# LinXueyuanStdio/LaTeX_OCR

Hardware: AMD Instinct MI355X
Metric: formula-images/sec training step (batch 64, 128x512) (higher is better)
Workload: dtype bf16; 1 GPU; configs[2]: full encoder+attention+decoder training step, batch 64/GPU, 128x512, vocab 500, T=101 (lengths U{30..100}), Adam; global_batch=64, parallelism=dp1

## Files before the change

### include/lxo.h

```cpp
#ifndef LXO_H
#define LXO_H
#include <stddef.h>
#include <stdint.h>
#ifdef __cplusplus
extern "C" {
#endif
#pragma GCC visibility push(default)

#define LXO_F32 0
#define LXO_BF16 1

const char* lxo_last_error(void);
#define LXO_ABI_VERSION 6
int lxo_version(void);
int lxo_shape_size(void);


int lxo_gemm_nt(int dt, int a_f32, int c_f32, int small, const void* A, const void* Bp, void* C,
                int M, int N, int K, int lda, int ldb, int ldc, const float* bias, int act,
                float alpha, int accumulate, void* stream);

int lxo_gemm_tn(int dt, int a_f32, int b_f32, const void* A, const void* B, float* C,
                int M, int I, int J, int lda, int ldb, int ldc, int nsplit, int atomic, void* stream);

int lxo_gemm_slab(int dt, const void* A, const void* Bp, float* slab, int M, int N, int K, int lda, int ldb, int ldc,
                  long long slab_stride, void* stream);

int lxo_conv3x3(int dt, const void* in, const void* wpk, const float* bias, void* out, int B, int H, int W,
                int Cin, int Ho, int Wo, int Cout, int pad, int relu, void* stream);

int lxo_conv3x3_ex(int dt, const void* in, const void* wpk, const float* bias, void* out, int B, int H, int W,
                   int Cin, int Ho, int Wo, int Cout, int pad, int relu, const float* addend, int addend_rows,
                   void* out_pre, const void* relu_ref, float* colsum, void* stream);

int lxo_conv3x3_wgrad(int dt, const void* in, const void* dout, float* dw, int B, int H, int W,
                      int Cin, int Ho, int Wo, int Cout, int pad, void* stream);

int lxo_attention_fwd(int dt, const void* att_img, const void* img, const float* att_h, const float* beta,
                      float* alpha, float* part, float* ctx, int ldctx, int nv, int R, int E, int C, int beam,
                      void* stream);

int lxo_timing_enable(int on);
int lxo_timing_count(void);
int lxo_timing_get(int i, const char** family, const char** name, double* work, float* ms);


typedef struct lxo_shape {
    int B, H, W, T, V;
    int C, E, U, O, D;
    int dtype;
    int beam;
    int max_steps;
    float keep_prob;
    int dropout_seed;
    float div_gamma, div_prob;
    int div_seed;
    int encoder_cnn;
    int no_positional;
    int step_kernels;
    int encoder_rnn;
    int deterministic;
    int live_B;
} lxo_shape;

int lxo_param_num(void);
const char* lxo_param_name(int id);
const char* lxo_param_name_for(const lxo_shape* s, int id);
long long lxo_param_total(const lxo_shape* s);
int lxo_param_info(const lxo_shape* s, int id, long long* offset, long long* count);

size_t lxo_wpack_bytes(const lxo_shape* s);
size_t lxo_workspace_bytes(const lxo_shape* s);
int lxo_ws_region(const lxo_shape* s, const char* name, size_t* offset, size_t* bytes);
#define LXO_I32 2
#define LXO_U8 3
int lxo_ws_region_dtype(const lxo_shape* s, const char* name);

int lxo_pack_weights(const lxo_shape* s, const float* params, void* wpack, void* stream);

int lxo_encoder_fwd(const lxo_shape* s, const float* params, const void* wpack, void* ws,
                    const uint8_t* img, void* stream);
int lxo_encoder_bwd(const lxo_shape* s, const float* params, const void* wpack, void* ws,
                    const uint8_t* img, float* grads, int last_layer, int first_layer, void* stream);
int lxo_encoder_bwd_ready(const lxo_shape* s, const float* params, const void* wpack, void* ws, const uint8_t* img, float* grads,
                          int last_layer, int first_layer, void* const* ready_events, void* stream);
int lxo_train_bwd(const lxo_shape* s, const float* params, const void* wpack, void* ws, const int32_t* formula, const uint8_t* img,
                  float* grads, void* const* ready_events, void* stream);

int lxo_set_side_stream(void* stream);
int lxo_set_encoder_side_stream(void* stream);

int lxo_decoder_train_fwd(const lxo_shape* s, const float* params, const void* wpack, void* ws,
                          const int32_t* formula, void* stream);
int lxo_decoder_train_fwd_live(const lxo_shape* s, const float* params, const void* wpack, void* ws,
                               const int32_t* formula, const int32_t* lengths, void* stream);
int lxo_ce_loss_fwd_bwd(const lxo_shape* s, void* ws, const int32_t* formula,
                        const int32_t* lengths, float inv_ntok, void* stream);
int lxo_ce_loss_fwd_bwd_dev(const lxo_shape* s, void* ws, const int32_t* formula,
                            const int32_t* lengths, const float* ntok_dev, void* stream);
int lxo_ce_loss_weighted(const lxo_shape* s, void* ws, const int32_t* formula, const int32_t* lengths,
                         const float* w_tok, const float* w_row, float inv_norm, const float* norm_dev, void* stream);
int lxo_ce_loss_smoothed(const lxo_shape* s, void* ws, const int32_t* formula, const int32_t* lengths, float eps,
                         const float* w_tok, const float* w_row, float inv_norm, const float* norm_dev, void* stream);
int lxo_mrt_weights(const float* seq_logp, const float* cost, const int32_t* group_off, int G, int rows, float alpha,
                    float* w_out, float* q_out, float* risk_out, void* stream);
#define LXO_EDIT_MAX_REF 1024
int lxo_edit_distance(const int32_t* hyp, int hyp_block, long long hyp_block_stride, long long hyp_row_stride, long long hyp_tok_stride, int T,
                      const int32_t* hyp_len, const int32_t* ref, int G, int ref_ld, const int32_t* ref_len, const int32_t* ref_of, int per_ref,
                      int pairs, int id_end, int32_t* dist_out, float* cost_out, void* stream);
#define LXO_TEXT_STATS  12
#define LXO_TEXT_CORPUS 14
int lxo_text_stats(const int32_t* hyp, int hyp_block, long long hyp_block_stride, long long hyp_row_stride, long long hyp_tok_stride, int T,
                   const int32_t* hyp_len, const int32_t* ref, int G, int ref_ld, const int32_t* ref_len, const int32_t* ref_of, int per_ref,
                   int pairs, int id_end, int32_t* stats_out, long long* corpus_io, int accumulate, void* stream);
int lxo_mrt_candidates(const int32_t* ids, int B, int max_steps, int n, int steps, const int32_t* ref, int Tr, const int32_t* ref_len,
                       int id_end, int id_pad, int include_reference, int32_t* cand, int32_t* cand_len, float* cost, int32_t* group_off,
                       int32_t* row_image, void* stream);
#define LXO_CONSENSUS_MAX_N 64
int lxo_consensus(const int32_t* ids, long long image_stride, long long draw_stride, long long tok_stride, int B, int n, int T, int id_end,
                  const float* weights, int normalize, int32_t* dist_out, float* risk_out, int32_t* best_out, void* stream);
#define LXO_BLEU_COUNTS 10
int lxo_sentence_bleu(const int32_t* hyp, int hyp_block, long long hyp_block_stride, long long hyp_row_stride, long long hyp_tok_stride, int T,
                      const int32_t* hyp_len, const int32_t* ref, int G, int ref_ld, const int32_t* ref_len, const int32_t* ref_of, int per_ref,
                      int pairs, int id_end, int32_t* counts_out, float* bleu_out, float* cost_out, void* stream);
int lxo_consensus_bleu(const int32_t* ids, long long image_stride, long long draw_stride, long long tok_stride, int B, int n, int T, int id_end,
                       const float* weights, int32_t* match_out, float* cost_out, float* risk_out, int32_t* best_out, void* stream);
#define LXO_COST_EDIT 0
#define LXO_COST_BLEU 1
int lxo_mrt_candidates_cost(const int32_t* ids, int B, int max_steps, int n, int steps, const int32_t* ref, int Tr, const int32_t* ref_len,
                            int id_end, int id_pad, int include_reference, int32_t* cand, int32_t* cand_len, float* cost, int32_t* group_off,
                            int32_t* row_image, int cost_kind, void* stream);
int lxo_score_tokens(const lxo_shape* s, void* ws, const int32_t* formula, const int32_t* lengths,
                     float* logp_out, int32_t* top1_out, float* seq_out, void* stream);
int lxo_score_alternatives(const lxo_shape* s, void* ws, const int32_t* formula, const int32_t* lengths, int k,
                           const uint32_t* allow, int allow_ld, int32_t* ids_out, float* logp_out,
                           int32_t* rank_out, float* entropy_out, void* stream);
int lxo_decoder_train_bwd(const lxo_shape* s, const float* params, const void* wpack, void* ws,
                          const int32_t* formula, float* grads, void* stream);
int lxo_decoder_train_bwd_part(const lxo_shape* s, const float* params, const void* wpack, void* ws,
                               const int32_t* formula, float* grads, int parts, void* stream);

#define LXO_XDEC_BLOCK_BYTES (4096 + (384 << 10))
#define LXO_XDEC_ERR_WORD 512
int lxo_chain_guard(const lxo_shape* s, void* ws, const float* grads, float* scale_io, int have_scale, uint32_t* status_out, void* stream);

#define LXO_GNORM_FLOATS (2 + 1024)
int lxo_global_norm_scale(long long n, const float* grads, float clip, float* scale_out, void* stream);
int lxo_adam_step(long long n, float* params, const float* grads, float* m, float* v,
                  float lr_t, float beta1, float beta2, float eps, const float* scale_dev, void* stream);

int lxo_optimizer_step(int method, long long n, float* params, const float* grads, float* slot, float lr,
                       const float* scale_dev, void* stream);

int lxo_greedy_decode(const lxo_shape* s, const float* params, const void* wpack, void* ws,
                      int id_end, int max_iter, int32_t* ids_out, int* steps_out, void* stream);
int lxo_greedy_decode_attn(const lxo_shape* s, const float* params, const void* wpack, void* ws,
                           int id_end, int max_iter, int32_t* ids_out, float* alpha_out, int* steps_out, void* stream);
int lxo_greedy_decode_scores(const lxo_shape* s, const float* params, const void* wpack, void* ws, int id_end, int max_iter,
                             int32_t* ids_out, float* logp_out, float* alpha_out, int* steps_out, void* stream);
int lxo_greedy_decode_prefix(const lxo_shape* s, const float* params, const void* wpack, void* ws, int id_end, int max_iter,
                             const int32_t* prefix, int prefix_ld, const int32_t* prefix_len,
                             int32_t* ids_out, float* logp_out, float* alpha_out, int* steps_out, void* stream);
int lxo_greedy_decode_constrained(const lxo_shape* s, const float* params, const void* wpack, void* ws, int id_end, int max_iter,
                                  const uint32_t* allow, int allow_ld,
                                  const int32_t* prefix, int prefix_ld, const int32_t* prefix_len,
                                  int32_t* ids_out, float* logp_out, float* alpha_out, int* steps_out, void* stream);
typedef struct lxo_sample_opts { float temperature; int top_k; float top_p; unsigned seed; } lxo_sample_opts;
int lxo_sample_decode(const lxo_shape* s, const float* params, const void* wpack, void* ws, int id_end, int max_iter,
                      const lxo_sample_opts* opts, const uint32_t* allow, int allow_ld,
                      const int32_t* prefix, int prefix_ld, const int32_t* prefix_len,
                      int32_t* ids_out, float* logp_out, float* logq_out, float* alpha_out, int* steps_out, void* stream);
int lxo_sample_tokens(const float* logits, int ld, int rows, int n, int V, int time, const lxo_sample_opts* opts,
                      const uint32_t* allow, int allow_ld, int32_t* ids_out, float* logp_out, float* logq_out, void* stream);
int lxo_decode_begin(const lxo_shape* s, const float* params, const void* wpack, void* ws, void* stream);
int lxo_decode_step(const lxo_shape* s, const float* params, const void* wpack, void* ws, int id_end, int time,
                    int32_t* ids_out, int32_t* parents_out, int32_t* finished_host, int* unfinished_host, void* stream);
// ... 54 lines not shown
```

### latex_ocr_amd/_abi.py

```python
import ctypes
import os

c_int, c_ll, c_size, c_float, c_void = ctypes.c_int, ctypes.c_longlong, ctypes.c_size_t, ctypes.c_float, ctypes.c_void_p
P = ctypes.POINTER

LXO_F32, LXO_BF16 = 0, 1
LXO_GNORM_FLOATS = 2 + 1024
LIB_PATH = os.environ.get("LXO_LIB_PATH") or os.path.join(os.path.dirname(os.path.abspath(__file__)), "liblxo.so")


ABI_VERSION = 6
LXO_COMM_ID_BYTES = 128
LXO_I32, LXO_U8 = 2, 3
LXO_XDEC_BLOCK_BYTES, LXO_XDEC_ERR_WORD = 4096 + (384 << 10), 512
LXO_EDIT_MAX_REF = 1024
LXO_CONSENSUS_MAX_N = 64
LXO_TEXT_STATS, LXO_TEXT_CORPUS = 12, 14
LXO_BLEU_COUNTS = 10
LXO_COST_EDIT, LXO_COST_BLEU = 0, 1


class LxoShape(ctypes.Structure):
    _fields_ = [(n, c_int) for n in ("B", "H", "W", "T", "V", "C", "E", "U", "O", "D", "dtype", "beam", "max_steps")] + \
               [("keep_prob", c_float), ("dropout_seed", c_int), ("div_gamma", c_float), ("div_prob", c_float), ("div_seed", c_int),
                ("encoder_cnn", c_int), ("no_positional", c_int), ("step_kernels", c_int), ("encoder_rnn", c_int), ("deterministic", c_int), ("live_B", c_int)]


class LxoSampleOpts(ctypes.Structure):
    _fields_ = [("temperature", c_float), ("top_k", c_int), ("top_p", c_float), ("seed", ctypes.c_uint)]


class LxoGrammar(ctypes.Structure):
    _fields_ = [("cls", c_void), ("n_kinds", c_int), ("max_depth", c_int), ("budget", c_int)]


LXO_GRAMMAR_MAX_DEPTH = 32


def bind(lib):
    S = P(LxoShape)
    sig = {
        "lxo_last_error": (ctypes.c_char_p, []),
        "lxo_version": (c_int, []),
        "lxo_shape_size": (c_int, []),
        "lxo_ws_region_dtype": (c_int, [S, ctypes.c_char_p]),
        "lxo_gemm_nt": (c_int, [c_int] * 4 + [c_void] * 3 + [c_int] * 6 + [c_void, c_int, c_float, c_int, c_void]),
        "lxo_gemm_tn": (c_int, [c_int] * 3 + [c_void] * 3 + [c_int] * 8 + [c_void]),
        "lxo_conv3x3": (c_int, [c_int, c_void, c_void, c_void, c_void] + [c_int] * 9 + [c_void]),
        "lxo_conv3x3_ex": (c_int, [c_int, c_void, c_void, c_void, c_void] + [c_int] * 9 + [c_void, c_int, c_void, c_void, c_void, c_void]),
        "lxo_conv3x3_wgrad": (c_int, [c_int, c_void, c_void, c_void] + [c_int] * 8 + [c_void]),
        "lxo_gemm_slab": (c_int, [c_int, c_void, c_void, c_void] + [c_int] * 6 + [c_ll, c_void]),
        "lxo_attention_fwd": (c_int, [c_int] + [c_void] * 7 + [c_int] * 6 + [c_void]),
        "lxo_timing_enable": (c_int, [c_int]),
        "lxo_timing_count": (c_int, []),
        "lxo_timing_get": (c_int, [c_int, P(ctypes.c_char_p), P(ctypes.c_char_p), P(ctypes.c_double), P(c_float)]),
        "lxo_param_num": (c_int, []),
        "lxo_param_name": (ctypes.c_char_p, [c_int]),
        "lxo_param_name_for": (ctypes.c_char_p, [S, c_int]),
        "lxo_param_total": (c_ll, [S]),
        "lxo_param_info": (c_int, [S, c_int, P(c_ll), P(c_ll)]),
        "lxo_wpack_bytes": (c_size, [S]),
        "lxo_workspace_bytes": (c_size, [S]),
        "lxo_ws_region": (c_int, [S, ctypes.c_char_p, P(c_size), P(c_size)]),
        "lxo_pack_weights": (c_int, [S, c_void, c_void, c_void]),
        "lxo_encoder_fwd": (c_int, [S, c_void, c_void, c_void, c_void, c_void]),
        "lxo_encoder_bwd": (c_int, [S, c_void, c_void, c_void, c_void, c_void, c_int, c_int, c_void]),
        "lxo_encoder_bwd_ready": (c_int, [S, c_void, c_void, c_void, c_void, c_void, c_int, c_int, c_void, c_void]),
        "lxo_train_bwd": (c_int, [S, c_void, c_void, c_void, c_void, c_void, c_void, c_void, c_void]),
        "lxo_set_encoder_side_stream": (c_int, [c_void]),
        "lxo_set_side_stream": (c_int, [c_void]),
        "lxo_decoder_train_fwd": (c_int, [S, c_void, c_void, c_void, c_void, c_void]),
        "lxo_decoder_train_fwd_live": (c_int, [S, c_void, c_void, c_void, c_void, c_void, c_void]),
        "lxo_ce_loss_fwd_bwd": (c_int, [S, c_void, c_void, c_void, c_float, c_void]),
        "lxo_ce_loss_fwd_bwd_dev": (c_int, [S, c_void, c_void, c_void, c_void, c_void]),
        "lxo_ce_loss_weighted": (c_int, [S, c_void, c_void, c_void, c_void, c_void, c_float, c_void, c_void]),
        "lxo_ce_loss_smoothed": (c_int, [S, c_void, c_void, c_void, c_float, c_void, c_void, c_float, c_void, c_void]),
        "lxo_mrt_weights": (c_int, [c_void, c_void, c_void, c_int, c_int, c_float, c_void, c_void, c_void, c_void]),
        "lxo_edit_distance": (c_int, [c_void, c_int, c_ll, c_ll, c_ll, c_int, c_void, c_void, c_int, c_int, c_void, c_void, c_int, c_int, c_int, c_void, c_void, c_void]),
        "lxo_text_stats": (c_int, [c_void, c_int, c_ll, c_ll, c_ll, c_int, c_void, c_void, c_int, c_int, c_void, c_void, c_int, c_int, c_int, c_void, c_void, c_int, c_void]),
        "lxo_mrt_candidates": (c_int, [c_void, c_int, c_int, c_int, c_int, c_void, c_int, c_void, c_int, c_int, c_int, c_void, c_void, c_void, c_void, c_void, c_void]),
        "lxo_sentence_bleu": (c_int, [c_void, c_int, c_ll, c_ll, c_ll, c_int, c_void, c_void, c_int, c_int, c_void, c_void, c_int, c_int, c_int, c_void, c_void, c_void, c_void]),
        "lxo_mrt_candidates_cost": (c_int, [c_void, c_int, c_int, c_int, c_int, c_void, c_int, c_void, c_int, c_int, c_int, c_void, c_void, c_void, c_void, c_void, c_int, c_void]),
        "lxo_consensus_bleu": (c_int, [c_void, c_ll, c_ll, c_ll, c_int, c_int, c_int, c_int, c_void, c_void, c_void, c_void, c_void, c_void]),
        "lxo_consensus": (c_int, [c_void, c_ll, c_ll, c_ll, c_int, c_int, c_int, c_int, c_void, c_int, c_void, c_void, c_void, c_void]),
        "lxo_decoder_train_bwd_part": (c_int, [S, c_void, c_void, c_void, c_void, c_void, c_int, c_void]),
        "lxo_decoder_train_bwd": (c_int, [S, c_void, c_void, c_void, c_void, c_void, c_void]),
        "lxo_global_norm_scale": (c_int, [c_ll, c_void, c_float, c_void, c_void]),
        "lxo_adam_step": (c_int, [c_ll, c_void, c_void, c_void, c_void, c_float, c_float, c_float, c_float, c_void, c_void]),
        "lxo_optimizer_step": (c_int, [c_int, c_ll, c_void, c_void, c_void, c_float, c_void, c_void]),
        "lxo_greedy_decode": (c_int, [S, c_void, c_void, c_void, c_int, c_int, c_void, P(c_int), c_void]),
        "lxo_greedy_decode_attn": (c_int, [S, c_void, c_void, c_void, c_int, c_int, c_void, c_void, P(c_int), c_void]),
        "lxo_decode_begin": (c_int, [S, c_void, c_void, c_void, c_void]),
        "lxo_decode_step": (c_int, [S, c_void, c_void, c_void, c_int, c_int, c_void, c_void, c_void, P(c_int), c_void]),
        "lxo_beam_decode": (c_int, [S, c_void, c_void, c_void, c_int, c_int, c_void, c_void, P(c_int), c_void]),
        "lxo_beam_decode_attn": (c_int, [S, c_void, c_void, c_void, c_int, c_int, c_void, c_void, c_void, P(c_int), c_void]),
        "lxo_greedy_decode_scores": (c_int, [S, c_void, c_void, c_void, c_int, c_int, c_void, c_void, c_void, P(c_int), c_void]),
        "lxo_beam_decode_scores": (c_int, [S, c_void, c_void, c_void, c_int, c_int, c_void, c_void, c_void, c_void, P(c_int), c_void]),
        "lxo_score_tokens": (c_int, [S, c_void, c_void, c_void, c_void, c_void, c_void, c_void]),
        "lxo_score_alternatives": (c_int, [S, c_void, c_void, c_void, c_int, c_void, c_int, c_void, c_void, c_void, c_void, c_void]),
        "lxo_greedy_decode_prefix": (c_int, [S, c_void, c_void, c_void, c_int, c_int, c_void, c_int, c_void, c_void, c_void, c_void, P(c_int), c_void]),
        "lxo_beam_decode_prefix": (c_int, [S, c_void, c_void, c_void, c_int, c_int, c_void, c_int, c_void, c_void, c_void, c_void, c_void, P(c_int), c_void]),
        "lxo_greedy_decode_constrained": (c_int, [S, c_void, c_void, c_void, c_int, c_int, c_void, c_int, c_void, c_int, c_void, c_void, c_void, c_void, P(c_int), c_void]),
        "lxo_beam_decode_constrained": (c_int, [S, c_void, c_void, c_void, c_int, c_int, c_void, c_int, c_void, c_int, c_void, c_void, c_void, c_void, c_void, P(c_int), c_void]),
        "lxo_sample_decode": (c_int, [S, c_void, c_void, c_void, c_int, c_int, P(LxoSampleOpts), c_void, c_int, c_void, c_int, c_void, c_void, c_void, c_void, c_void, P(c_int), c_void]),
        "lxo_sample_tokens": (c_int, [c_void, c_int, c_int, c_int, c_int, c_int, P(LxoSampleOpts), c_void, c_int, c_void, c_void, c_void, c_void]),
        "lxo_grammar_scratch_bytes": (c_size, [c_int, c_int]),
        "lxo_greedy_decode_grammar": (c_int, [S, c_void, c_void, c_void, c_int, c_int, c_void, c_int, c_void, c_int, c_void, P(LxoGrammar), c_void, c_void, c_void, c_void, c_void, P(c_int), c_void]),
        "lxo_beam_decode_grammar": (c_int, [S, c_void, c_void, c_void, c_int, c_int, c_void, c_int, c_void, c_int, c_void, P(LxoGrammar), c_void, c_void, c_void, c_void, c_void, c_void, P(c_int), c_void]),
        "lxo_sample_decode_grammar": (c_int, [S, c_void, c_void, c_void, c_int, c_int, P(LxoSampleOpts), c_void, c_int, c_void, c_int, c_void, P(LxoGrammar), c_void, c_void, c_void, c_void, c_void, c_void, P(c_int), c_void]),
        "lxo_grammar_step": (c_int, [P(LxoGrammar), c_int, c_int, c_int, c_int, c_void, c_void, c_void, c_int, c_int, c_void, c_int, c_void, c_void, c_void, c_void]),
        "lxo_chain_guard": (c_int, [S, c_void, c_void, c_void, c_int, c_void, c_void]),
        "lxo_decode_state_get": (c_int, [S, c_void, c_int, c_void, c_void, c_void, c_void]),
        "lxo_decode_state_set": (c_int, [S, c_void, c_int, c_void, c_void, c_void, c_void, c_void]),
        "lxo_decode_cell_step": (c_int, [S, c_void, c_void, c_void, c_int, c_int, c_void]),
        "lxo_comm_unique_id": (c_int, [c_void]),
        "lxo_comm_init": (c_int, [c_void, c_int, c_int, P(c_void)]),
        "lxo_comm_info": (c_int, [c_void, P(c_int), P(c_int)]),
        "lxo_allreduce_bucket": (c_int, [c_void, c_void, c_ll, c_int, c_void, c_void]),
        "lxo_comm_destroy": (c_int, [c_void]),
        "lxo_comm_last_error": (ctypes.c_char_p, []),
    }
    missing = []
    for name, (res, args) in sig.items():
        try:
            fn = getattr(lib, name)
        except AttributeError:
            missing.append(name)
            continue
        fn.restype, fn.argtypes = res, args
    lib._lxo_missing = missing
    if not missing:
        if lib.lxo_version() != ABI_VERSION or lib.lxo_shape_size() != ctypes.sizeof(LxoShape):
            raise RuntimeError("liblxo ABI mismatch: library version %d / lxo_shape %d bytes, binding version %d / %d bytes"
                               % (lib.lxo_version(), lib.lxo_shape_size(), ABI_VERSION, ctypes.sizeof(LxoShape)))
    return lib


ENTRY_POINTS = ["lxo_last_error", "lxo_version", "lxo_shape_size", "lxo_ws_region_dtype", "lxo_timing_enable", "lxo_timing_count", "lxo_timing_get", "lxo_gemm_nt", "lxo_gemm_tn", "lxo_conv3x3", "lxo_conv3x3_ex", "lxo_conv3x3_wgrad", "lxo_gemm_slab", "lxo_attention_fwd", "lxo_param_num", "lxo_param_name", "lxo_param_name_for",
                "lxo_param_total", "lxo_param_info", "lxo_wpack_bytes", "lxo_workspace_bytes", "lxo_ws_region",
                "lxo_pack_weights", "lxo_encoder_fwd", "lxo_encoder_bwd", "lxo_encoder_bwd_ready", "lxo_train_bwd", "lxo_set_side_stream", "lxo_set_encoder_side_stream", "lxo_decoder_train_fwd", "lxo_decoder_train_fwd_live",
                "lxo_ce_loss_fwd_bwd", "lxo_ce_loss_fwd_bwd_dev", "lxo_ce_loss_weighted", "lxo_ce_loss_smoothed", "lxo_mrt_weights", "lxo_edit_distance", "lxo_text_stats", "lxo_mrt_candidates", "lxo_consensus", "lxo_sentence_bleu", "lxo_consensus_bleu", "lxo_mrt_candidates_cost", "lxo_decoder_train_bwd", "lxo_decoder_train_bwd_part", "lxo_global_norm_scale", "lxo_adam_step", "lxo_optimizer_step",
                "lxo_greedy_decode", "lxo_greedy_decode_attn", "lxo_beam_decode", "lxo_beam_decode_attn", "lxo_greedy_decode_scores", "lxo_beam_decode_scores", "lxo_score_tokens", "lxo_score_alternatives", "lxo_greedy_decode_prefix", "lxo_beam_decode_prefix", "lxo_greedy_decode_constrained", "lxo_beam_decode_constrained", "lxo_sample_decode", "lxo_sample_tokens",
                "lxo_grammar_scratch_bytes", "lxo_greedy_decode_grammar", "lxo_beam_decode_grammar", "lxo_sample_decode_grammar", "lxo_grammar_step", "lxo_decode_begin", "lxo_decode_step",
                "lxo_chain_guard", "lxo_decode_state_get", "lxo_decode_state_set", "lxo_decode_cell_step",
                "lxo_comm_unique_id", "lxo_comm_init", "lxo_comm_info", "lxo_allreduce_bucket", "lxo_comm_destroy", "lxo_comm_last_error"]

_lib = None


def load():
    global _lib
    if _lib is None:
        if not os.path.exists(LIB_PATH):
            raise RuntimeError(
                "latex_ocr_amd: %s is missing. Build it with `python -c 'import __graft_entry__ as g; g.build()'` "
                "(hipcc --offload-arch=gfx950). There is no CPU fallback." % LIB_PATH)
        try:
            import torch
        except ImportError:
            pass
        _lib = bind(ctypes.CDLL(LIB_PATH))
        if _lib._lxo_missing:
            raise RuntimeError("liblxo.so lacks entry points: %s" % _lib._lxo_missing)
    return _lib


def check(lib, rc, what=""):
    if rc != 0:
        raise RuntimeError("%s failed: rc=%d %s" % (what, rc, lib.lxo_last_error().decode()))
```

### latex_ocr_amd/csrc/api.hip

```cpp
#include "lxo.h"
#include "gemm.h"
#include "impl.h"
#include <stdio.h>
#include <string.h>

static thread_local char g_err[256] = "";
static int fail(int code, const char* what) {
    snprintf(g_err, sizeof(g_err), "%s (code %d)", what, code);
    return code < 0 ? code : -code;
}
#define CHECK_LAUNCH(expr, what) do { int rc_ = (expr); if (rc_ != 0) return fail(rc_, what); } while (0)

extern "C" const char* lxo_last_error(void) { return g_err; }
extern "C" int lxo_version(void) { return LXO_ABI_VERSION; }
extern "C" int lxo_shape_size(void) { return (int)sizeof(lxo_shape); }

extern "C" int lxo_gemm_nt(int dt, int a_f32, int c_f32, int small, const void* A, const void* Bp, void* C,
                           int M, int N, int K, int lda, int ldb, int ldc, const float* bias, int act,
                           float alpha, int accumulate, void* stream) {
    GemmNT p; memset(&p, 0, sizeof(p));
    p.A = A; p.Bp = Bp; p.C = C; p.M = M; p.N = N; p.K = K; p.lda = lda; p.ldb = ldb; p.ldc = ldc;
    p.bias = bias; p.act = act; p.alpha = alpha; p.accumulate = accumulate; p.addend_rows = 1;
    CHECK_LAUNCH(lxo_launch_gemm_nt(dt, a_f32, c_f32, small, p, (hipStream_t)stream), "lxo_gemm_nt");
    return 0;
}

extern "C" int lxo_gemm_tn(int dt, int a_f32, int b_f32, const void* A, const void* B, float* C,
                           int M, int I, int J, int lda, int ldb, int ldc, int nsplit, int atomic, void* stream) {
    GemmTN p; memset(&p, 0, sizeof(p));
    p.A = A; p.B = B; p.C = C; p.M = M; p.I = I; p.J = J; p.lda = lda; p.ldb = ldb; p.ldc = ldc;
    p.nsplit = nsplit; p.nbatch = 1; p.atomic = atomic;
    CHECK_LAUNCH(lxo_launch_gemm_tn(dt, a_f32, b_f32, p, (hipStream_t)stream), "lxo_gemm_tn");
    return 0;
}

#define MAKE_PLAN(P, s) if (!(s)) return fail(-1, "null shape"); Plan P(*(s)); \
    { char m_[200]; int v_ = P.validate(m_, sizeof(m_)); if (v_) { snprintf(g_err, sizeof(g_err), "%s", m_); return v_; } }

extern "C" int lxo_param_num(void) { return P_COUNT; }
extern "C" const char* lxo_param_name_for(const lxo_shape* s, int id) { return lxo_param_name_mode(id, s ? s->encoder_cnn : 0); }
extern "C" long long lxo_param_total(const lxo_shape* s) { if (!s) return -1; Plan P(*s); return P.ptotal; }
extern "C" int lxo_param_info(const lxo_shape* s, int id, long long* offset, long long* count) {
    if (!s || id < 0 || id >= P_COUNT) return fail(-1, "lxo_param_info");
    Plan P(*s);
    if (offset) *offset = P.poff[id];
    if (count) *count = P.pcount[id];
    return 0;
}
extern "C" size_t lxo_wpack_bytes(const lxo_shape* s) { if (!s) return 0; Plan P(*s); return P.ktotal; }
extern "C" size_t lxo_workspace_bytes(const lxo_shape* s) { if (!s) return 0; Plan P(*s); return P.wtotal; }
extern "C" int lxo_ws_region(const lxo_shape* s, const char* name, size_t* offset, size_t* bytes) {
    if (!s || !name) return fail(-1, "lxo_ws_region");
    Plan P(*s);
    for (int i = 0; i < W_COUNT; ++i)
        if (strcmp(name, lxo_ws_name(i)) == 0) {
            if (offset) *offset = P.woff[i];
            if (bytes) *bytes = P.wbytes[i];
            return 0;
        }
    return fail(-1, "unknown workspace region");
}
extern "C" int lxo_ws_region_dtype(const lxo_shape* s, const char* name) {
    if (!s || !name) return fail(-1, "lxo_ws_region_dtype");
    const bool bf = s->dtype == LXO_BF16;
    static const char* const kCompute[] = {"p1", "y2", "p2", "y3", "y4", "p4", "y5", "p5", "y6", "img", "att_img", "emb_in", "dlogits",
                                           "d_att_img", "g0", "g1", "g2", "cols", "dec_emb", "dec_txe", "rxt"};
    static const char* const kBf16[] = {"recb", "gb", "dzb", "rhb", "rdzb", "att_exp", "datth_b"};
    static const char* const kI32[] = {"dec_ids", "dec_flags", "beam_par"};
    static const char* const kU8[] = {"m2", "m4", "m5"};
    for (const char* n : kCompute) if (strcmp(name, n) == 0) return bf ? LXO_BF16 : LXO_F32;
    for (const char* n : kBf16) if (strcmp(name, n) == 0) return LXO_BF16;
    for (const char* n : kI32) if (strcmp(name, n) == 0) return LXO_I32;
    for (const char* n : kU8) if (strcmp(name, n) == 0) return LXO_U8;
    if (strcmp(name, "d_img") == 0) { Plan P(*s); return P.dimg_masked() ? LXO_BF16 : LXO_F32; }
    for (int i = 0; i < W_COUNT; ++i) if (strcmp(name, lxo_ws_name(i)) == 0) return LXO_F32;
    return fail(-1, "unknown workspace region");
}
extern "C" int lxo_pack_weights(const lxo_shape* s, const float* params, void* wpack, void* stream) {
    MAKE_PLAN(P, s);
    CHECK_LAUNCH(lxo_impl_pack_weights(P, params, wpack, (hipStream_t)stream), "lxo_pack_weights");
    return 0;
}
extern "C" int lxo_encoder_fwd(const lxo_shape* s, const float* params, const void* wpack, void* ws,
                               const uint8_t* img, void* stream) {
    MAKE_PLAN(P, s);
    CHECK_LAUNCH(lxo_impl_encoder_fwd(P, params, wpack, ws, img, (hipStream_t)stream), "lxo_encoder_fwd");
    return 0;
}
extern "C" int lxo_encoder_bwd(const lxo_shape* s, const float* params, const void* wpack, void* ws,
                               const uint8_t* img, float* grads, int last_layer, int first_layer, void* stream) {
    MAKE_PLAN(P, s);
    if (last_layer > 6 || first_layer < 1 || last_layer < first_layer) return fail(-1, "lxo_encoder_bwd: layer range");
    CHECK_LAUNCH(lxo_impl_encoder_bwd(P, params, wpack, ws, img, grads, last_layer, first_layer, (hipStream_t)stream), "lxo_encoder_bwd");
    return 0;
}
extern "C" int lxo_encoder_bwd_ready(const lxo_shape* s, const float* params, const void* wpack, void* ws, const uint8_t* img, float* grads,
                                     int last_layer, int first_layer, void* const* ready_events, void* stream) {
    MAKE_PLAN(P, s);
    if (last_layer > 6 || first_layer < 1 || last_layer < first_layer) return fail(-1, "lxo_encoder_bwd_ready: layer range");
    if (!ready_events) return fail(-1, "lxo_encoder_bwd_ready: null event table");
    CHECK_LAUNCH(lxo_impl_encoder_bwd(P, params, wpack, ws, img, grads, last_layer, first_layer, (hipStream_t)stream, ready_events), "lxo_encoder_bwd_ready");
    return 0;
}

#include "head_kernels.h"
extern "C" int lxo_decoder_train_fwd(const lxo_shape* s, const float* params, const void* wpack, void* ws,
                                     const int32_t* formula, void* stream) {
    MAKE_PLAN(P, s);
    if (s->T <= 0) return fail(-1, "T must be positive");
    CHECK_LAUNCH(lxo_impl_decoder_train_fwd(P, params, wpack, ws, formula, (hipStream_t)stream), "lxo_decoder_train_fwd");
    return 0;
}
extern "C" int lxo_decoder_train_fwd_live(const lxo_shape* s, const float* params, const void* wpack, void* ws,
                                          const int32_t* formula, const int32_t* lengths, void* stream) {
    MAKE_PLAN(P, s);
    if (s->T <= 0) return fail(-1, "T must be positive");
    CHECK_LAUNCH(lxo_impl_decoder_train_fwd(P, params, wpack, ws, formula, (hipStream_t)stream, lengths), "lxo_decoder_train_fwd_live");
    return 0;
}
extern "C" int lxo_ce_loss_fwd_bwd(const lxo_shape* s, void* ws, const int32_t* formula, const int32_t* lengths,
                                   float inv_ntok, void* stream) {
    MAKE_PLAN(P, s);
    CHECK_LAUNCH(lxo_impl_ce_loss(P, ws, formula, lengths, inv_ntok, nullptr, (hipStream_t)stream), "lxo_ce_loss_fwd_bwd");
    return 0;
}
extern "C" int lxo_ce_loss_fwd_bwd_dev(const lxo_shape* s, void* ws, const int32_t* formula, const int32_t* lengths,
                                       const float* ntok_dev, void* stream) {
    MAKE_PLAN(P, s);
    if (!ntok_dev) return fail(-1, "lxo_ce_loss_fwd_bwd_dev: null token count");
    CHECK_LAUNCH(lxo_impl_ce_loss(P, ws, formula, lengths, 0.f, ntok_dev, (hipStream_t)stream), "lxo_ce_loss_fwd_bwd_dev");
    return 0;
}
extern "C" int lxo_ce_loss_weighted(const lxo_shape* s, void* ws, const int32_t* formula, const int32_t* lengths, const float* w_tok, const float* w_row,
                                    float inv_norm, const float* norm_dev, void* stream) {
    MAKE_PLAN(P, s);
    if (!w_tok && !w_row) return fail(-1, "lxo_ce_loss_weighted: w_tok and w_row are both NULL (the unweighted loss is lxo_ce_loss_fwd_bwd)");
    CHECK_LAUNCH(lxo_impl_ce_loss(P, ws, formula, lengths, inv_norm, norm_dev, (hipStream_t)stream, w_tok, w_row), "lxo_ce_loss_weighted");
    return 0;
}
extern "C" int lxo_ce_loss_smoothed(const lxo_shape* s, void* ws, const int32_t* formula, const int32_t* lengths, float eps, const float* w_tok,
                                    const float* w_row, float inv_norm, const float* norm_dev, void* stream) {
    MAKE_PLAN(P, s);
    if (!ws || !formula || !lengths) return fail(-1, "lxo_ce_loss_smoothed: null ws, formula or lengths");
    if (!(eps - eps == 0.f) || !(eps >= 0.f && eps < 1.f)) return fail(-1, "lxo_ce_loss_smoothed: eps is not a finite number in [0, 1)");
    CHECK_LAUNCH(lxo_impl_ce_loss(P, ws, formula, lengths, inv_norm, norm_dev, (hipStream_t)stream, w_tok, w_row, &eps), "lxo_ce_loss_smoothed");
    return 0;
}
extern "C" int lxo_mrt_weights(const float* seq_logp, const float* cost, const int32_t* group_off, int G, int rows, float alpha,
                               float* w_out, float* q_out, float* risk_out, void* stream) {
    if (!w_out || !seq_logp || !cost || !group_off) return fail(-1, "lxo_mrt_weights: null w_out, seq_logp, cost or group_off");
    if (G < 0 || rows < 0) return fail(-1, "lxo_mrt_weights: G < 0 or rows < 0");
    if (!(alpha - alpha == 0.f)) return fail(-1, "lxo_mrt_weights: alpha is not finite");
    CHECK_LAUNCH(lxo_k_mrt_weights(seq_logp, cost, group_off, G, rows, alpha, w_out, q_out, risk_out, (hipStream_t)stream), "lxo_mrt_weights");
    return 0;
}
#include "seqcost.h"
static_assert(LXO_EDIT_MAX_REF == kEditMaxRef, "include/lxo.h and csrc/seqcost.h disagree on the reference limit");
extern "C" int lxo_edit_distance(const int32_t* hyp, int hyp_block, long long hyp_block_stride, long long hyp_row_stride, long long hyp_tok_stride, int T,
                                 const int32_t* hyp_len, const int32_t* ref, int G, int ref_ld, const int32_t* ref_len, const int32_t* ref_of,
                                 int per_ref, int pairs, int id_end, int32_t* dist_out, float* cost_out, void* stream) {
    if (!hyp || !ref || !dist_out) return fail(-1, "lxo_edit_distance: null hyp, ref or dist_out");
    if (pairs < 0 || T < 0 || G < 0 || hyp_block_stride < 0 || hyp_row_stride < 0 || hyp_tok_stride < 0)
        return fail(-1, "lxo_edit_distance: a negative count or stride");
    if (hyp_block < 1 || per_ref < 1 || (pairs > 0 && G < 1)) return fail(-1, "lxo_edit_distance: hyp_block < 1, per_ref < 1 or no reference row");
    if (ref_ld < 1 || ref_ld > LXO_EDIT_MAX_REF) return fail(-1, "lxo_edit_distance: ref_ld outside 1 .. LXO_EDIT_MAX_REF (a reference longer than the kernel's column limit)");
    const EditArgs a = {hyp, hyp_len, ref, ref_len, ref_of, nullptr, dist_out, cost_out, hyp_block_stride, hyp_row_stride, hyp_tok_stride,
                        hyp_block, T, G, ref_ld, per_ref, pairs, id_end};
    CHECK_LAUNCH(lxo_k_edit_distance(a, (hipStream_t)stream), "lxo_edit_distance");
    return 0;
}
static_assert(LXO_TEXT_STATS == kTextStats && LXO_TEXT_CORPUS == kTextCorpus, "include/lxo.h and csrc/seqcost.h disagree on the text-metric rows");
extern "C" int lxo_text_stats(const int32_t* hyp, int hyp_block, long long hyp_block_stride, long long hyp_row_stride, long long hyp_tok_stride, int T,
                              const int32_t* hyp_len, const int32_t* ref, int G, int ref_ld, const int32_t* ref_len, const int32_t* ref_of, int per_ref,
                              int pairs, int id_end, int32_t* stats_out, long long* corpus_io, int accumulate, void* stream) {
    if (!hyp || !ref) return fail(-1, "lxo_text_stats: null hyp or ref");
    if (!stats_out && !corpus_io) return fail(-1, "lxo_text_stats: stats_out and corpus_io are both NULL");
    if (pairs < 0 || T < 0 || G < 0 || hyp_block_stride < 0 || hyp_row_stride < 0 || hyp_tok_stride < 0)
        return fail(-1, "lxo_text_stats: a negative count or stride");
    if (hyp_block < 1 || per_ref < 1 || (pairs > 0 && G < 1)) return fail(-1, "lxo_text_stats: hyp_block < 1, per_ref < 1 or no reference row");
    if (T > LXO_EDIT_MAX_REF) return fail(-1, "lxo_text_stats: T outside 0 .. LXO_EDIT_MAX_REF (a hypothesis wider than the kernel's staging limit)");
    if (ref_ld < 1 || ref_ld > LXO_EDIT_MAX_REF) return fail(-1, "lxo_text_stats: ref_ld outside 1 .. LXO_EDIT_MAX_REF (a reference longer than the kernel's column limit)");
    if (accumulate != 0 && accumulate != 1) return fail(-1, "lxo_text_stats: accumulate must be 0 or 1");
    const TextArgs a = {hyp, hyp_len, ref, ref_len, ref_of, stats_out, corpus_io, hyp_block_stride, hyp_row_stride, hyp_tok_stride,
                        hyp_block, T, G, ref_ld, per_ref, pairs, id_end, accumulate};
    CHECK_LAUNCH(lxo_k_text_stats(a, (hipStream_t)stream), "lxo_text_stats");
// ... 443 lines not shown
```

### latex_ocr_amd/csrc/conv_wgrad.hip

```cpp
#include "gemm.h"
#include "api_util.h"
#include "lxo_debug.h"

namespace {

constexpr int WTH = 2, WTW = 64, WPW = WTW + 2, WPH = WTH + 2, WPROWS = WPH * WPW;
constexpr int WTHREADS = 512;
constexpr int WPATCH = 5 * WTHREADS * 16;
constexpr int WDY = WTH * WTW * 256;
constexpr int WSTAGE = WPATCH + WDY;
constexpr int WCI = 64, WCO = 128;

typedef __attribute__((address_space(1))) const void* gptr_t;
typedef __attribute__((address_space(3))) void* lptr_t;
typedef __attribute__((ext_vector_type(4))) short v4s_t;
typedef __attribute__((address_space(3))) v4s_t* ltr_t;
LXO_DEV void glds16(const void* g, void* l) {
    __builtin_amdgcn_global_load_lds((gptr_t)(uintptr_t)g, (lptr_t)(uintptr_t)l, 16, 0, 0);
}
LXO_DEV u32x2 tr_read(const char* p) {
    return __builtin_bit_cast(u32x2, __builtin_amdgcn_ds_read_tr16_b64_v4i16((ltr_t)(uintptr_t)p));
}

}
// ... 45 lines not shown
    const unsigned drel = (unsigned)(((tid >> 4) * Cout + dgch) * 2);
    const int dxq = (co0 + dgch) < Cout ? (tid >> 4) : 0x7FFF0000;
    int tx_i = pb_beg % tiles_x, ty_i = (pb_beg / tiles_x) % tiles_y, b_i = pb_beg / (tiles_x * tiles_y);
    auto issue = [&](int stage) {
        const int oy0 = ty_i * WTH, ox0 = tx_i * WTW;
        const unsigned sx = (unsigned)((((b_i * p.H + oy0) * p.W + ox0) * p.Cin + ci0) * 2);
        const int loy = max(0, p.pad - oy0), lox = max(0, p.pad - ox0);
        const int ny = min(WPH, p.H + p.pad - oy0) - loy, nx = min(WPW, p.W + p.pad - ox0) - lox;
        const unsigned lo = __builtin_amdgcn_readfirstlane(((unsigned)loy << 16) | (unsigned)lox);
        const unsigned lim = __builtin_amdgcn_readfirstlane(((unsigned)(ny - 1) << 16) | (unsigned)(nx - 1));
#pragma unroll
        for (int j = 0; j < 5; ++j) {
            if (j == 4 && wave != 0) break;
            const u16x2_t t = __builtin_bit_cast(u16x2_t, ppk[j]) - __builtin_bit_cast(u16x2_t, lo);
            const u16x2_t m = __builtin_elementwise_min(t, __builtin_bit_cast(u16x2_t, lim));
            const bool ok = __builtin_bit_cast(unsigned, m) == __builtin_bit_cast(unsigned, t) && (j < 4 || tid < 64);
            const unsigned voff = ok ? prel[j] : LXO_BLDS_OOB;
            LXO_BLDS16(voff, rx, sx, lxo_wgrad_lds, m0b, stage * WSTAGE + (wave * 64 + 512 * j) * 16);
        }
        const unsigned sd = (unsigned)((((b_i * p.Ho + oy0) * p.Wo + ox0) * Cout + co0) * 2);
#pragma unroll
        for (int j = 0; j < 4; ++j) {
            const int hx = (oy0 + (j >> 1) < p.Ho) ? p.Wo - ox0 - 32 * (j & 1) : 0;
            const unsigned voff = dxq < hx ? drel : LXO_BLDS_OOB;
            const unsigned sdj = __builtin_amdgcn_readfirstlane(sd + (unsigned)((((j >> 1) * p.Wo + 32 * (j & 1)) * Cout) * 2));
            LXO_BLDS16(voff, rdy, sdj, lxo_wgrad_lds, m0b, stage * WSTAGE + WPATCH + (wave * 64 + 512 * j) * 16);
        }
        if (++tx_i == tiles_x) { tx_i = 0; if (++ty_i == tiles_y) { ty_i = 0; ++b_i; } }
    };

    f32x16 acc[9];
#pragma unroll
    for (int t = 0; t < 9; ++t)
#pragma unroll
        for (int e = 0; e < 16; ++e) acc[t][e] = 0.f;

    const int h = lane >> 5, g = (lane >> 4) & 1, qj = (lane & 15) >> 2, qc = lane & 3;
    const int a_ch = wci * 32 + 16 * g + 4 * qc;
    const int a_chunk = a_ch >> 3, a_sub = (a_ch & 7) * 2;
    const int b_ch = wco * 32 + 16 * g + 4 * qc;
    const int b_chunk = b_ch >> 3, b_sub = (b_ch & 7) * 2;
    const int bl = 8 * h + qj;
    int poff[8];
#pragma unroll
    for (int k = 0; k < 8; ++k) poff[k] = bl * 128 + ((a_chunk ^ ((k + (bl >> 1)) & 7)) << 4) + a_sub;
    const int doff_a = WPATCH + bl * 256 + ((b_chunk ^ (bl & 15)) << 4) + b_sub;
    const int doff_b = WPATCH + (bl + 4) * 256 + ((b_chunk ^ ((bl + 4) & 15)) << 4) + b_sub;

#define WSTAMP(i) do { if (p.dbg && tid == 0 && (i) < 64) p.dbg[(long long)blockIdx.x * 64 + (i)] = __builtin_readcyclecounter(); } while (0)
    WSTAMP(0);
    issue(0);
    for (int pb = pb_beg; pb < pb_end; ++pb) {
        const int stage = (pb - pb_beg) & 1;
        WSTAMP(1 + 3 * (pb - pb_beg));
        __builtin_amdgcn_s_waitcnt(0x0F70);
        WSTAMP(2 + 3 * (pb - pb_beg));
        __builtin_amdgcn_s_barrier();
        WSTAMP(3 + 3 * (pb - pb_beg));
#ifndef LXO_WG_DIAG
#define LXO_WG_DIAG 0
#endif
        const char* sb = lxo_wgrad_lds + stage * WSTAGE;
        const char* pk[8];
#pragma unroll
        for (int k = 0; k < 8; ++k) pk[k] = sb + poff[k];
        const char* da = sb + doff_a;
        const char* db = sb + doff_b;
        u32x2 ra[2][4], rb[2][4];
        auto read_b = [&](int xg, u32x2 (&b4)[4]) {
#pragma unroll
            for (int ty = 0; ty < 2; ++ty) {
                const int cd = (ty * 64 + xg * 16) * 256;
                b4[2 * ty] = tr_read(da + cd);
                b4[2 * ty + 1] = tr_read(db + cd);
            }
        };
        auto read_a = [&](int s, u32x2 (&r)[4]) {
            const int cc = (s & 3) * WPW + (s >> 2) * 16;
            r[0] = tr_read(pk[(cc >> 1) & 7] + cc * 128);
            r[1] = tr_read(pk[((cc + 4) >> 1) & 7] + (cc + 4) * 128);
            r[2] = tr_read(pk[((cc + 2) >> 1) & 7] + (cc + 2) * 128);
            r[3] = tr_read(pk[((cc + 6) >> 1) & 7] + (cc + 6) * 128);
        };
        read_b(0, rb[0]);
        read_a(0, ra[0]);
        __builtin_amdgcn_sched_barrier(0);
        if (pb + 1 < pb_end && !((LXO_WG_DIAG & 1) && pb > pb_beg)) issue(stage ^ 1);
        __builtin_amdgcn_sched_barrier(0);
#pragma unroll
        for (int s = 0; s < 16; ++s) {
            const int xg = s >> 2, row = s & 3, cur = s & 1, bcur = xg & 1;
            if (s == 0) __builtin_amdgcn_s_setprio(3);
            else if (s == 4) __builtin_amdgcn_s_setprio(2);
            else if (s == 8) __builtin_amdgcn_s_setprio(1);
            else if (s == 12) __builtin_amdgcn_s_setprio(0);
            if (!(LXO_WG_DIAG & 2)) {
                if (s + 1 < 16) read_a(s + 1, ra[cur ^ 1]);
                if (row == 1 && xg + 1 < 4) read_b(xg + 1, rb[bcur ^ 1]);
            } else if (s == 0) { read_a(1, ra[1]); read_b(1, rb[1]); }
            __builtin_amdgcn_sched_barrier(0);
            const u32x2* r = ra[cur];
            const u32x4 a0 = {r[0][0], r[0][1], r[1][0], r[1][1]};
            const u32x4 a2 = {r[2][0], r[2][1], r[3][0], r[3][1]};
            const u32x4 b0 = {rb[bcur][0][0], rb[bcur][0][1], rb[bcur][1][0], rb[bcur][1][1]};
            const u32x4 b1 = {rb[bcur][2][0], rb[bcur][2][1], rb[bcur][3][0], rb[bcur][3][1]};
#define WG_MFMA(A, B, T) acc[T] = __builtin_amdgcn_mfma_f32_32x32x16_bf16(__builtin_bit_cast(bf16x8_t, A), __builtin_bit_cast(bf16x8_t, B), acc[T], 0, 0, 0)
            if (row <= 2) WG_MFMA(a0, b0, row * 3 + 0); else WG_MFMA(a0, b1, (row - 1) * 3 + 0);
            __builtin_amdgcn_sched_barrier(0);
            const u32x4 a1 = (LXO_WG_DIAG & 4) ? u32x4{r[0][1], r[1][0], r[1][1], r[3][1]} :
                             u32x4{__builtin_amdgcn_alignbit(r[0][1], r[0][0], 16), __builtin_amdgcn_alignbit(r[1][0], r[0][1], 16),
                                   __builtin_amdgcn_alignbit(r[1][1], r[1][0], 16), __builtin_amdgcn_alignbit(r[3][1], r[1][1], 16)};
            __builtin_amdgcn_sched_barrier(0);
            if (row <= 2) {
                WG_MFMA(a2, b0, row * 3 + 2);
                WG_MFMA(a1, b0, row * 3 + 1);
                if (row >= 1) WG_MFMA(a0, b1, (row - 1) * 3 + 0);
            }
            if (row >= 1) {
                WG_MFMA(a2, b1, (row - 1) * 3 + 2);
                WG_MFMA(a1, b1, (row - 1) * 3 + 1);
            }
#undef WG_MFMA
            __builtin_amdgcn_sched_barrier(0);
        }
    }
    WSTAMP(61);
    if (p.det_slab) {
        float* const sb = p.det_slab + ((long long)split * ntiles + tile) * (9 * WCI * WCO) + (wci * 32 + 4 * (lane >> 5)) * WCO + wco * 32 + (lane & 31);
#pragma unroll
        for (int t = 0; t < 9; ++t)
#pragma unroll
            for (int e = 0; e < 16; ++e) sb[(t * WCI + (e & 3) + 8 * (e >> 2)) * WCO] = acc[t][e];
        return;
    }
    const int co = co0 + wco * 32 + (lane & 31);
    if (co < Cout) {
        const int rot = (int)(blockIdx.x % 9u);
        float* const cbase = p.C + (long long)(ci0 + wci * 32 + 4 * (lane >> 5)) * p.ldc + co;
        auto emit = [&](const f32x16& a, int t) {
#pragma unroll
            for (int e = 0; e < 16; ++e) atomicAdd(cbase + (t * p.Cin + (e & 3) + 8 * (e >> 2)) * p.ldc, a[e]);
        };
#pragma unroll
        for (int t = 0; t < 9; ++t) if (t >= rot) emit(acc[t], t);
#pragma unroll
        for (int t = 0; t < 9; ++t) if (t < rot) emit(acc[t], t);
    }
    WSTAMP(62);
}

__global__ __launch_bounds__(256) void wgrad_slab_reduce_kernel(const float* __restrict__ slab, int nsplit, int ntiles, int tiles_co, int Cin, int Cout,
                                                               float* __restrict__ dw, int ldc) {
    const int tile = blockIdx.y;
    const int i = blockIdx.x * 256 + threadIdx.x;
    if (i >= 9 * WCI * WCO) return;
    const int co = i % WCO, ci = (i / WCO) % WCI, tap = i / (WCO * WCI);
    const int ci0 = (tile / tiles_co) * WCI, co0 = (tile % tiles_co) * WCO;
    float s = 0.f;
    for (int q = 0; q < nsplit; ++q) s += slab[((long long)q * ntiles + tile) * (9 * WCI * WCO) + i];
    if (co0 + co < Cout) dw[(long long)(tap * Cin + ci0 + ci) * ldc + co0 + co] += s;
}

}

static thread_local unsigned long long* g_wgrad_dbg = nullptr;
extern "C" int lxo_wgrad_debug(unsigned long long* buf) { g_wgrad_dbg = buf; return 0; }
int lxo_launch_conv_wgrad(const GemmTN& p, hipStream_t s) {
    if (!p.conv || p.Cin % 64 || p.J % 8) return -2;
    {
        const long long nb = p.M / (p.Ho * p.Wo);
        if (nb * p.H * p.W * p.Cin * 2 + 2LL * (p.W + 1) * p.Cin >= (1LL << 31) || nb * p.Ho * p.Wo * p.J * 2 >= (1LL << 31)) return -2;
    }
    {
        static bool done[64] = {};
        int dev = 0;
        const bool known = hipGetDevice(&dev) == hipSuccess && dev >= 0 && dev < 64;
        if (!known || !done[dev]) {
            HIPRC(hipFuncSetAttribute(reinterpret_cast<const void*>(conv_wgrad_kernel), hipFuncAttributeMaxDynamicSharedMemorySize, 2 * WSTAGE));
            if (known) done[dev] = true;
        }
    }
    const int B = p.M / (p.Ho * p.Wo);
    const int tiles_ci = p.Cin / WCI, tiles_co = cdiv(p.J, WCO);
    const int tiles_x = cdiv(p.Wo, WTW), tiles_y = cdiv(p.Ho, WTH);
    const int nblocks = B * tiles_x * tiles_y;
    const int tiles = tiles_ci * tiles_co;
    int nsplit = cdiv(256, tiles);
    if (nsplit > nblocks) nsplit = nblocks;
    constexpr int min_blk = 8;
    if (nsplit > cdiv(nblocks, min_blk)) nsplit = cdiv(nblocks, min_blk);
    if (nsplit < 1) nsplit = 1;
    const int per_split = cdiv(nblocks, nsplit);
    nsplit = cdiv(nblocks, per_split);
    constexpr float stag_scale = 10.f;
    float stagger = stag_scale / (float)per_split;
    if (stagger > 0.5f) stagger = 0.5f;
    if (nsplit < 2) stagger = 0.f;
    GemmTN q = p;
    q.nbatch = tiles;
    q.dbg = g_wgrad_dbg;
    const int nsplit8 = (nsplit + 7) / 8 * 8;
    if (q.det_slab) {
        const size_t need = (size_t)nsplit * tiles * 9 * WCI * WCO;
        if (need > q.det_floats) return -6;
    }
    hipLaunchKernelGGL(conv_wgrad_kernel, dim3(tiles * nsplit8), dim3(WTHREADS), 2 * WSTAGE, s, q, tiles_co, tiles_x, tiles_y, nblocks, nsplit, stagger);
    if (q.det_slab)
        hipLaunchKernelGGL(wgrad_slab_reduce_kernel, dim3(9 * WCI * WCO / 256, tiles), dim3(256), 0, s, q.det_slab, nsplit, tiles, tiles_co, p.Cin, p.J, p.C, p.ldc);
    return (int)hipGetLastError();
}
```

### latex_ocr_amd/csrc/decoder_kernels.hip

```cpp
#include "decoder_kernels.h"
#include "api_util.h"
#include "drop.h"

namespace {


LXO_DEV void load4(const float* p, float (&v)[4]) {
    f32x4 a = *reinterpret_cast<const f32x4*>(p);
    v[0] = a[0]; v[1] = a[1]; v[2] = a[2]; v[3] = a[3];
}
LXO_DEV void load4(const bf16_t* p, float (&v)[4]) {
    u32x2 a = *reinterpret_cast<const u32x2*>(p);
    v[0] = __uint_as_float(a[0] << 16); v[1] = __uint_as_float(a[0] & 0xffff0000u);
    v[2] = __uint_as_float(a[1] << 16); v[3] = __uint_as_float(a[1] & 0xffff0000u);
}
LXO_DEV void store4(float* p, const float (&v)[4]) { f32x4 a = {v[0], v[1], v[2], v[3]}; *reinterpret_cast<f32x4*>(p) = a; }
LXO_DEV void store4(bf16_t* p, const float (&v)[4]) { u32x2 a = {pack_bf2(v[0], v[1]), pack_bf2(v[2], v[3])}; *reinterpret_cast<u32x2*>(p) = a; }

LXO_DEV float slab_sum(const Slabs& sl, long long row, int col) {
    float v = 0.f;
    const float* q = sl.p + row * sl.ld + col;
    for (int s = 0; s < sl.n; ++s) v += q[(long long)s * sl.stride];
    return v;
}
// ... 902 lines not shown
            const long long pitch = (long long)B * E;
            int t0 = 0;
            for (; t0 + TU <= n; t0 += TU) {
                f32x4 a[TU], d[TU][Q];
#pragma unroll
                for (int tt = 0; tt < TU; ++tt) {
                    a[tt] = *reinterpret_cast<const f32x4*>(ap + (t0 + tt) * pitch);
#pragma unroll
                    for (int c = 0; c < Q; ++c) d[tt][c] = sd[t0 + tt][wave * Q + c];
                }
#pragma unroll
                for (int tt = 0; tt < TU; ++tt) datt_live_step<RW>(x, a[tt], d[tt], acc, db, sumd);
            }
            for (; t0 < n; ++t0) {
                const f32x4 a = *reinterpret_cast<const f32x4*>(ap + t0 * pitch);
                f32x4 d[Q];
#pragma unroll
                for (int c = 0; c < Q; ++c) d[c] = sd[t0][wave * Q + c];
                datt_live_step<RW>(x, a, d, acc, db, sumd);
            }
        }
    }
    if (kon) {
        float bt[4];
        load4(beta + k0, bt);
#pragma unroll
        for (int rr = 0; rr < RW; ++rr)
            if (rbase + rr < R) {
                float o[4];
#pragma unroll
                for (int j = 0; j < 4; ++j) o[j] = (acc[rr][j] * 4.f) * bt[j];
                store4(dout + ((long long)b * R + rbase + rr) * E + k0, o);
            }
#pragma unroll
        for (int j = 0; j < 4; ++j) redb[wave][k0 + j] = sumd - 2.f * db[j];
    }
    __syncthreads();
    if (tid < E) {
        const float s = redb[0][tid] + redb[1][tid] + redb[2][tid] + redb[3][tid];
        if (dbeta_part) dbeta_part[((long long)blockIdx.y * gridDim.x + blockIdx.x) * E + tid] = s;
        else atomicAdd(&dbeta[tid], s);
    }
}

__global__ __launch_bounds__(256) void add_mean_grad_kernel(float* __restrict__ dimg, const float* __restrict__ dmean, int B, int R, int C) {
    const long long total = (long long)B * R * C;
    const float inv = 1.0f / (float)R;
    for (long long i = (long long)blockIdx.x * 256 + threadIdx.x; i < total; i += (long long)gridDim.x * 256) {
        const int c = (int)(i % C);
        const int b = (int)(i / ((long long)R * C));
        dimg[i] += dmean[(long long)b * C + c] * inv;
    }
}

__global__ __launch_bounds__(256) void colsum_kernel(const float* __restrict__ a, int lda, float* __restrict__ out, int M, int N, int rows_per_block) {
    const int n = blockIdx.x * 256 + threadIdx.x;
    const int m0 = blockIdx.y * rows_per_block, m1 = min(M, m0 + rows_per_block);
    if (n >= N) return;
    float s = 0.f;
    for (int m = m0; m < m1; ++m) s += a[(long long)m * lda + n];
    atomicAdd(&out[n], s);
}

__global__ __launch_bounds__(256) void colsum4_kernel(const float* __restrict__ a, int lda, float* __restrict__ out, int M, int N, int rows_per_block) {
    __shared__ f32x4 red[4][64];
    const int cq = threadIdx.x & 63, ry = threadIdx.x >> 6;
    const int n = (blockIdx.x * 64 + cq) * 4;
    const int m0 = blockIdx.y * rows_per_block, m1 = min(M, m0 + rows_per_block);
    const int nl = n < N ? n : 0;
    f32x4 s = {0.f, 0.f, 0.f, 0.f};
    for (int mb = m0 + ry; mb < m1; mb += 32) {
        f32x4 v[8];
#pragma unroll
        for (int u = 0; u < 8; ++u) { const int m = min(mb + 4 * u, m1 - 1); v[u] = *reinterpret_cast<const f32x4*>(a + (long long)m * lda + nl); }
#pragma unroll
        for (int u = 0; u < 8; ++u) if (mb + 4 * u < m1) s += v[u];
    }
    red[ry][cq] = s;
    __syncthreads();
    if (ry == 0 && n < N) {
        const f32x4 t = red[0][cq] + red[1][cq] + red[2][cq] + red[3][cq];
#pragma unroll
        for (int e = 0; e < 4; ++e) atomicAdd(&out[n + e], t[e]);
    }
}


template <typename AT>
__global__ __launch_bounds__(256) void colsum_part_kernel(const AT* __restrict__ a, long long lda, float* __restrict__ part, long long M, int N, int rows_per) {
    const int n = blockIdx.x * 256 + threadIdx.x;
    const long long m0 = (long long)blockIdx.y * rows_per, m1 = m0 + rows_per < M ? m0 + rows_per : M;
    if (n >= N) return;
    float s = 0.f;
    for (long long mb = m0; mb < m1; mb += 8) {
        float v[8];
#pragma unroll
        for (int u = 0; u < 8; ++u) { const long long m = mb + u < m1 ? mb + u : m1 - 1; v[u] = to_f32(a[m * lda + n]); }
#pragma unroll
        for (int u = 0; u < 8; ++u) if (mb + u < m1) s += v[u];
    }
    part[(long long)blockIdx.y * N + n] = s;
}
__global__ __launch_bounds__(256) void det_reduce_kernel(const float* __restrict__ part, int nslot, long long stride, int N, float* __restrict__ out) {
    __shared__ float gs[16][16];
    const int c = threadIdx.x & 15, g = threadIdx.x >> 4;
    const int n = blockIdx.x * 16 + c;
    const int per = (nslot + 15) / 16;
    const int q0 = g * per, q1 = min(nslot, q0 + per);
    float s = 0.f;
    if (n < N) {
        for (int q = q0; q < q1; q += 8) {
            float v[8];
#pragma unroll
            for (int u = 0; u < 8; ++u) v[u] = part[(long long)min(q + u, q1 - 1) * stride + n];
#pragma unroll
            for (int u = 0; u < 8; ++u) if (q + u < q1) s += v[u];
        }
    }
    gs[g][c] = s;
    __syncthreads();
    if (g == 0 && n < N) {
        float tsum = gs[0][c];
#pragma unroll
        for (int k = 1; k < 16; ++k) tsum += gs[k][c];
        out[n] += tsum;
    }
}

__global__ __launch_bounds__(256) void embed_scatter_kernel(const float* __restrict__ demb, const int* __restrict__ formula,
                                                           float* __restrict__ dtable, float* __restrict__ dstart,
                                                           int B, int T, int D, int V) {
    const long long total = (long long)T * B * D;
    for (long long i = (long long)blockIdx.x * 256 + threadIdx.x; i < total; i += (long long)gridDim.x * 256) {
        const int d = (int)(i % D);
        const long long row = i / D;
        const int b = (int)(row % B), t = (int)(row / B);
        const float g = demb[i];
        if (t == 0) atomicAdd(&dstart[d], g);
        else {
            int id = formula[(long long)b * T + t - 1];
            id = id < 0 ? 0 : (id >= V ? V - 1 : id);
            atomicAdd(&dtable[(long long)id * D + d], g);
        }
    }
}

__global__ __launch_bounds__(256) void embed_scatter_rows_kernel(const float* __restrict__ demb, const int* __restrict__ formula,
                                                                float* __restrict__ dtable, float* __restrict__ dstart,
                                                                int B, int T, int D, int V, int det) {
    constexpr int CH = 2048;
    __shared__ int list[CH];
    __shared__ float part[256];
    __shared__ int cnt;
    __shared__ int wcnt[4];
    const int id = blockIdx.x;
    const int tid = threadIdx.x;
    const int rpw = 256 / D, r = tid / D, c = tid - r * D;
    float sum = 0.f;
    const int total = T * B;
    const int per = (total + (int)gridDim.y - 1) / (int)gridDim.y;
    const int s0 = blockIdx.y * per, s1 = min(total, s0 + per);
    for (int base = s0; base < s1; base += CH) {
        if (tid == 0) cnt = 0;
        __syncthreads();
        if (det) {
            for (int jb = base; jb < min(s1, base + CH); jb += 256) {
                const int j = jb + tid;
                int row = -1;
                if (j < min(s1, base + CH)) {
                    const int b = j / T, tt = j - b * T;
                    if (id == V) { if (j < B) row = j; }
                    else if (tt + 1 < T) { int tok = formula[j]; tok = tok < 0 ? 0 : (tok >= V ? V - 1 : tok); if (tok == id) row = (tt + 1) * B + b; }
                }
                const unsigned long long m = __ballot(row >= 0);
                const int lane = tid & 63, wv = tid >> 6;
                if (lane == 0) wcnt[wv] = __builtin_popcountll(m);
                __syncthreads();
                int off = cnt;
                for (int w = 0; w < wv; ++w) off += wcnt[w];
                if (row >= 0) list[off + __builtin_popcountll(m & ((1ull << lane) - 1ull))] = row;
                __syncthreads();
                if (tid == 0) cnt += wcnt[0] + wcnt[1] + wcnt[2] + wcnt[3];
                __syncthreads();
            }
        } else
        for (int j = base + tid; j < min(s1, base + CH); j += 256) {
            const int b = j / T, tt = j - b * T;
            if (id == V) { if (j < B) list[atomicAdd(&cnt, 1)] = j; continue; }
            if (tt + 1 >= T) continue;
            int tok = formula[j]; tok = tok < 0 ? 0 : (tok >= V ? V - 1 : tok);
            if (tok == id) list[atomicAdd(&cnt, 1)] = (tt + 1) * B + b;
        }
        __syncthreads();
        const int n = cnt;
        if (r < rpw) {
            for (int k = r; k < n; k += 4 * rpw) {
                float v[4];
#pragma unroll
                for (int u = 0; u < 4; ++u) { const int kk = min(k + u * rpw, n - 1); v[u] = demb[(long long)list[kk] * D + c]; }
#pragma unroll
                for (int u = 0; u < 4; ++u) if (k + u * rpw < n) sum += v[u];
            }
        }
        __syncthreads();
    }
    part[tid] = (r < rpw) ? sum : 0.f;
    __syncthreads();
    if (tid < D) {
        float t = 0.f;
        for (int q = 0; q < rpw; ++q) t += part[q * D + tid];
        float* dst = id == V ? dstart : dtable + (long long)id * D;
        if (t != 0.f) atomicAdd(&dst[tid], t);
    }
}

__global__ __launch_bounds__(256) void init_bwd_kernel(const float* __restrict__ dcc, Slabs dxh,
                                                      const float* __restrict__ c0, const float* __restrict__ rec0, int ldr,
                                                      float* __restrict__ dpre, int B, int U, int O) {
    const int W = 2 * U + O;
    const int total = B * W;
    for (int i = blockIdx.x * 256 + threadIdx.x; i < total; i += gridDim.x * 256) {
        const int b = i / W, k = i - b * W;
        float d, s;
        if (k < U) { d = dcc[(long long)b * U + k]; s = c0[(long long)b * U + k]; }
        else if (k < 2 * U) { d = slab_sum(dxh, b, O + (k - U)); s = rec0[(long long)b * ldr + O + (k - U)]; }
        else { d = slab_sum(dxh, b, k - 2 * U); s = rec0[(long long)b * ldr + (k - 2 * U)]; }
        dpre[i] = d * (1.f - s * s);
    }
}

__global__ __launch_bounds__(256) void beam_gather_kernel(const float* __restrict__ rec, int ldr, int XH, const float* __restrict__ cs, int U,
                                                         const int* __restrict__ parents, int k, float* __restrict__ tmp_rec, float* __restrict__ tmp_cs, int n) {
    const int W = XH + U;
    const long long total = (long long)n * W;
    for (long long i = (long long)blockIdx.x * 256 + threadIdx.x; i < total; i += (long long)gridDim.x * 256) {
        const int v = (int)(i / W), c = (int)(i - (long long)v * W);
        const int src = (v / k) * k + parents[v];
        if (c < XH) tmp_rec[(long long)v * XH + c] = rec[(long long)src * ldr + c];
        else tmp_cs[(long long)v * U + (c - XH)] = cs[(long long)src * U + (c - XH)];
    }
}
__global__ __launch_bounds__(256) void beam_scatter_kernel(float* __restrict__ rec, int ldr, int XH, float* __restrict__ cs, int U,
                                                          const float* __restrict__ tmp_rec, const float* __restrict__ tmp_cs, int n,
                                                          bf16_t* __restrict__ recb, int ldrb) {
    const int W = XH + U;
    const long long total = (long long)n * W;
    for (long long i = (long long)blockIdx.x * 256 + threadIdx.x; i < total; i += (long long)gridDim.x * 256) {
        const int v = (int)(i / W), c = (int)(i - (long long)v * W);
        if (c < XH) {
            const float x = tmp_rec[(long long)v * XH + c];
            rec[(long long)v * ldr + c] = x;
            if (recb) recb[(long long)v * ldrb + c] = f2bf(x);
        }
        else cs[(long long)v * U + (c - XH)] = tmp_cs[(long long)v * U + (c - XH)];
    }
}
constexpr int BP_KMAX = 16;
__global__ __launch_bounds__(256) void beam_permute_kernel(float* __restrict__ rec, int ldr, int XH, float* __restrict__ cs, int U,
                                                          const int* __restrict__ parents, int k, bf16_t* __restrict__ recb, int ldrb) {
    const int b = blockIdx.x, c = blockIdx.y * 256 + threadIdx.x;
    if (c >= XH + U) return;
    float v[BP_KMAX];
#pragma unroll
    for (int r = 0; r < BP_KMAX; ++r) {
        v[r] = 0.f;
        if (r < k) {
            const int src = b * k + parents[b * k + r];
            v[r] = c < XH ? rec[(long long)src * ldr + c] : cs[(long long)src * U + (c - XH)];
        }
    }
#pragma unroll
    for (int r = 0; r < BP_KMAX; ++r) {
        if (r < k) {
            const int dst = b * k + r;
            if (c < XH) { rec[(long long)dst * ldr + c] = v[r]; if (recb) recb[(long long)dst * ldrb + c] = f2bf(v[r]); }
            else cs[(long long)dst * U + (c - XH)] = v[r];
        }
    }
}
__global__ __launch_bounds__(256) void tile_rows_kernel(const float* __restrict__ src, int lds, float* __restrict__ dst, int ldd, int n, int k, int cols) {
    const long long total = (long long)n * cols;
    for (long long i = (long long)blockIdx.x * 256 + threadIdx.x; i < total; i += (long long)gridDim.x * 256) {
        const int v = (int)(i / cols), c = (int)(i - (long long)v * cols);
        dst[(long long)v * ldd + c] = src[(long long)(v / k) * lds + c];
    }
}

__global__ __launch_bounds__(256) void sumsq_kernel(const float* __restrict__ g, long long n, float* __restrict__ out) {
    __shared__ float red[4];
    float s = 0.f;
    for (long long i = (long long)blockIdx.x * 256 + threadIdx.x; i < n; i += (long long)gridDim.x * 256) s = fmaf(g[i], g[i], s);
    s = wave_sum(s);
    if ((threadIdx.x & 63) == 0) red[threadIdx.x >> 6] = s;
    __syncthreads();
    if (threadIdx.x == 0) out[blockIdx.x] = red[0] + red[1] + red[2] + red[3];
}
__global__ void clip_scale_kernel(const float* __restrict__ sumsq, int nparts, float clip, float* __restrict__ out) {
    float ss = 0.f;
    for (int i = 0; i < nparts; ++i) ss += sumsq[i];
    const float gn = sqrtf(ss);
    out[1] = gn;
    out[0] = clip > 0.f ? clip / fmaxf(gn, clip) : 1.0f;
}
__global__ void chain_guard_kernel(const unsigned* __restrict__ err_fwd, const unsigned* __restrict__ err_bwd, const float* __restrict__ probe,
                                   float* __restrict__ scale, int have_scale, unsigned* __restrict__ status) {
    const unsigned ef = err_fwd ? err_fwd[0] : 0u, eb = err_bwd ? err_bwd[0] : 0u;
    const float pv = probe ? probe[0] : 0.f;
    const bool drop = (ef | eb) != 0u || pv != pv;
    if (status) { status[0] = ef; status[1] = eb; status[2] = drop ? 1u : 0u; }
    scale[0] = drop ? __uint_as_float(0x7fc00000u) : (have_scale ? scale[0] : 1.0f);
}
__global__ void chain_poison_kernel(const unsigned* __restrict__ err_fwd, const unsigned* __restrict__ err_bwd, float* __restrict__ probe) {
    if ((err_fwd && err_fwd[0]) || (err_bwd && err_bwd[0])) probe[0] = __uint_as_float(0x7fc00000u);
}
__global__ __launch_bounds__(256) void adam_kernel(float* __restrict__ p, const float* __restrict__ g, float* __restrict__ m, float* __restrict__ v,
                                                  long long n, float lr_t, float b1, float b2, float eps, const float* __restrict__ scale) {
    const float sc = scale ? scale[0] : 1.0f;
    if (sc != sc) return;
    for (long long i = (long long)blockIdx.x * 256 + threadIdx.x; i < n; i += (long long)gridDim.x * 256) {
        const float gi = g[i] * sc;
        const float mi = b1 * m[i] + (1.f - b1) * gi;
        const float vi = b2 * v[i] + (1.f - b2) * gi * gi;
        m[i] = mi; v[i] = vi;
        p[i] -= lr_t * mi / (sqrtf(vi) + eps);
    }
}

__global__ __launch_bounds__(256) void simple_opt_kernel(float* __restrict__ p, const float* __restrict__ g, float* __restrict__ slot,
                                                        long long n, float lr, int mode, const float* __restrict__ scale) {
    const float sc = scale ? scale[0] : 1.0f;
    if (sc != sc) return;
    for (long long i = (long long)blockIdx.x * 256 + threadIdx.x; i < n; i += (long long)gridDim.x * 256) {
        const float gi = g[i] * sc;
        if (mode == 1) p[i] -= lr * gi;
        else if (mode == 2) { const float a = slot[i] + gi * gi; slot[i] = a; p[i] -= lr * gi / sqrtf(a); }
        else { const float ms = 0.9f * slot[i] + 0.1f * gi * gi; slot[i] = ms; p[i] -= lr * gi / sqrtf(ms + 1e-10f); }
    }
}

inline int grid1(long long items, int per_block = 256, int cap = 2048) {
    long long g = (items + per_block - 1) / per_block;
    return (int)(g < 1 ? 1 : (g > cap ? cap : g));
}
}

#define LAUNCH(kern, grid, ...) hipLaunchKernelGGL(kern, dim3(grid), dim3(256), 0, st, __VA_ARGS__)
#define BYCT(dt, kern, grid, ...) do { if ((dt) == LXO_BF16) LAUNCH((kern<bf16_t>), grid, __VA_ARGS__); else LAUNCH((kern<float>), grid, __VA_ARGS__); } while (0)
#define DONE return (int)hipGetLastError()

int lxo_k_rowmean(int dt, const void* img, float* mean, int B, int R, int C, hipStream_t st) {
    if (C % 64) return -2;
    if (dt == LXO_BF16) LAUNCH((rowmean_kernel<bf16_t>), dim3(C / 64, B), (const bf16_t*)img, mean, R, C);
    else LAUNCH((rowmean_kernel<float>), dim3(C / 64, B), (const float*)img, mean, R, C);
    DONE;
// ... 206 lines not shown
```

### latex_ocr_amd/csrc/gemm.h

```cpp
#pragma once
#include "lxo_common.h"

struct GemmNT {
    const void* A; const void* Bp; void* C;
    int M, N, K;
    int lda, ldb, ldc;
    int conv, H, W, Cin, Ho, Wo, pad;
    const float* bias;
    const float* addend; int addend_rows;
    int act;
    const void* relu_ref; int ldr;
    void* out_pre;
    int accumulate;
    float* colsum;
    float* colsum_part; size_t colsum_part_floats;
    float alpha;
    unsigned long long* dbg;
    void* pool_out; unsigned char* pool_mask; int pool_h, pool_w;
    int diag;
};

struct GemmTN {
    const void* A; const void* B; float* C;
    int M, I, J;
    int lda, ldb, ldc;
    int conv, H, W, Cin, Ho, Wo, pad;
    int nsplit, nbatch;
    long long strideA, strideB, strideC;
    int atomic;
    unsigned long long* dbg;
    float* det_slab; size_t det_floats;
};

int lxo_launch_gemm_nt(int dt, int a_f32, int c_f32, int small, const GemmNT& p, hipStream_t s);
int lxo_launch_gemm_tn(int dt, int a_f32, int b_f32, const GemmTN& p, hipStream_t s);

int lxo_launch_gemm_slab(int dt, const GemmNT& p, float* slab, long long slab_stride, hipStream_t s);

int lxo_launch_conv_igemm(const GemmNT& p, hipStream_t s);

int lxo_launch_gemm_nt_dma(const GemmNT& p, int c_f32, hipStream_t s);

int lxo_launch_gemm_tn_tr(const GemmTN& p, hipStream_t s);

int lxo_launch_conv_wgrad(const GemmTN& p, hipStream_t s);
```

### latex_ocr_amd/csrc/gemm_tn_tr.hip

```cpp
#include "gemm.h"
#include "api_util.h"

namespace {

constexpr int TBR = 64;
constexpr int TTILE = TBR * 256;
constexpr int TSTAGE = 2 * TTILE;

typedef __attribute__((ext_vector_type(4))) short v4s_t;
typedef __attribute__((address_space(3))) v4s_t* ltr_t;
LXO_DEV u32x2 tr_read(const char* p) {
    return __builtin_bit_cast(u32x2, __builtin_amdgcn_ds_read_tr16_b64_v4i16((ltr_t)(uintptr_t)p));
}

}

HIP_DYNAMIC_SHARED(char, lxo_tntr_lds)

namespace {

__global__ __launch_bounds__(256) void gemm_tn_tr_kernel(GemmTN p) {
    const int tid = threadIdx.x, lane = tid & 63, wave = tid >> 6;
    const int wi = wave >> 1, wj = wave & 1;
    const int tj_n = (p.J + 127) / 128, ti_n = (p.I + 127) / 128, tiles = tj_n * ti_n;
    const int units = tiles * p.nsplit, per_xcd = (units + 7) / 8;
    const int unit = (int)(blockIdx.x & 7) * per_xcd + (int)(blockIdx.x >> 3);
    if ((int)(blockIdx.x >> 3) >= per_xcd || unit >= units) return;
    const int split = unit / tiles, tile = unit - split * tiles;
    const int i0 = (tile / tj_n) * 128, j0 = (tile % tj_n) * 128;
    const int per = ((p.M + p.nsplit - 1) / p.nsplit + TBR - 1) / TBR * TBR;
    const int mbeg = split * per, mend = min(p.M, mbeg + per);
    float* const slab = p.det_slab ? p.det_slab + ((long long)split * tiles + tile) * (128 * 128) : nullptr;
    if (mbeg >= mend) {
        if (slab) for (int i = tid; i < 128 * 128 / 4; i += 256) reinterpret_cast<f32x4*>(slab)[i] = f32x4{0.f, 0.f, 0.f, 0.f};
        return;
    }
    const bf16_t* __restrict__ A = reinterpret_cast<const bf16_t*>(p.A);
    const bf16_t* __restrict__ B = reinterpret_cast<const bf16_t*>(p.B);

    const int dch = tid & 15, drow = tid >> 4;
    const unsigned m0b = __builtin_amdgcn_readfirstlane((unsigned)(uintptr_t)lxo_tntr_lds);
    const lxo_rsrc_t ra = lxo_make_rsrc(A, (unsigned)((long long)mend * p.lda * 2));
    const lxo_rsrc_t rb = lxo_make_rsrc(B, (unsigned)((long long)mend * p.ldb * 2));
    unsigned voa[4], vob[4];
#pragma unroll
    for (int j = 0; j < 4; ++j) {
        const int r = drow + 16 * j;
        const int gch = (dch ^ (r & 15)) << 3;
        voa[j] = i0 + gch < p.I ? (unsigned)((r * p.lda + i0 + gch) * 2) : LXO_BLDS_OOB;
        vob[j] = j0 + gch < p.J ? (unsigned)((r * p.ldb + j0 + gch) * 2) : LXO_BLDS_OOB;
    }
    const int wave_u = __builtin_amdgcn_readfirstlane(wave);
    auto issue = [&](int m0, int stage) {
        const unsigned sa = __builtin_amdgcn_readfirstlane((unsigned)(m0 * p.lda * 2)), sb = __builtin_amdgcn_readfirstlane((unsigned)(m0 * p.ldb * 2));
#pragma unroll
        for (int j = 0; j < 4; ++j) {
            LXO_BLDS16(voa[j], ra, sa, lxo_tntr_lds, m0b, stage * TSTAGE + (wave_u * 64 + 256 * j) * 16);
            LXO_BLDS16(vob[j], rb, sb, lxo_tntr_lds, m0b, stage * TSTAGE + TTILE + (wave_u * 64 + 256 * j) * 16);
        }
    };

    f32x16 acc[2][2];
#pragma unroll
    for (int a = 0; a < 2; ++a)
#pragma unroll
        for (int b = 0; b < 2; ++b)
#pragma unroll
            for (int e = 0; e < 16; ++e) acc[a][b][e] = 0.f;

    const int h = lane >> 5, g = (lane >> 4) & 1, qj = (lane & 15) >> 2, qc = lane & 3;
    const int bl = 8 * h + qj;
    int offa[2][2], offb[2][2];
#pragma unroll
    for (int t = 0; t < 2; ++t) {
        const int ca = wi * 64 + t * 32 + 16 * g + 4 * qc, cb = wj * 64 + t * 32 + 16 * g + 4 * qc;
#pragma unroll
        for (int u = 0; u < 2; ++u) {
            const int r = bl + 4 * u;
            offa[t][u] = r * 256 + (((ca >> 3) ^ (r & 15)) << 4) + (ca & 7) * 2;
            offb[t][u] = TTILE + r * 256 + (((cb >> 3) ^ (r & 15)) << 4) + (cb & 7) * 2;
        }
    }

    issue(mbeg, 0);
    for (int m0 = mbeg, it = 0; m0 < mend; m0 += TBR, ++it) {
        const int stage = it & 1;
        __builtin_amdgcn_s_waitcnt(0x0070);
        __builtin_amdgcn_s_barrier();
        if (m0 + TBR < mend) issue(m0 + TBR, stage ^ 1);
        const char* sb = lxo_tntr_lds + stage * TSTAGE;
#pragma unroll
        for (int ks = 0; ks < TBR / 16; ++ks) {
            const int cd = ks * 16 * 256;
            u32x4 af[2], bf[2];
#pragma unroll
            for (int t = 0; t < 2; ++t) {
                const u32x2 a0 = tr_read(sb + offa[t][0] + cd), a1 = tr_read(sb + offa[t][1] + cd);
                const u32x2 b0 = tr_read(sb + offb[t][0] + cd), b1 = tr_read(sb + offb[t][1] + cd);
                af[t] = u32x4{a0[0], a0[1], a1[0], a1[1]};
                bf[t] = u32x4{b0[0], b0[1], b1[0], b1[1]};
            }
#pragma unroll
            for (int a = 0; a < 2; ++a)
#pragma unroll
                for (int b = 0; b < 2; ++b)
                    acc[a][b] = __builtin_amdgcn_mfma_f32_32x32x16_bf16(__builtin_bit_cast(bf16x8_t, af[a]), __builtin_bit_cast(bf16x8_t, bf[b]), acc[a][b], 0, 0, 0);
        }
    }
    if (slab) {
#pragma unroll
        for (int b = 0; b < 2; ++b)
#pragma unroll
            for (int a = 0; a < 2; ++a)
#pragma unroll
                for (int e = 0; e < 16; ++e)
                    slab[(wi * 64 + a * 32 + (e & 3) + 8 * (e >> 2) + 4 * (lane >> 5)) * 128 + wj * 64 + b * 32 + (lane & 31)] = acc[a][b][e];
        return;
    }
#pragma unroll
    for (int b = 0; b < 2; ++b) {
        const int jj = j0 + wj * 64 + b * 32 + (lane & 31);
#pragma unroll
        for (int a = 0; a < 2; ++a)
#pragma unroll
            for (int e = 0; e < 16; ++e) {
                const int ii = i0 + wi * 64 + a * 32 + (e & 3) + 8 * (e >> 2) + 4 * (lane >> 5);
                if (ii < p.I && jj < p.J) atomicAdd(&p.C[(long long)ii * p.ldc + jj], acc[a][b][e]);
            }
    }
}

__global__ __launch_bounds__(256) void tn_slab_reduce_kernel(const float* __restrict__ slab, int nsplit, int tiles, int tj_n, int I, int J, float* __restrict__ C, int ldc) {
    const int tile = blockIdx.y;
    const int i = blockIdx.x * 256 + threadIdx.x;
    const int r = i >> 7, c = i & 127;
    const int ii = (tile / tj_n) * 128 + r, jj = (tile % tj_n) * 128 + c;
    float s = 0.f;
    for (int q = 0; q < nsplit; ++q) s += slab[((long long)q * tiles + tile) * (128 * 128) + i];
    if (ii < I && jj < J) C[(long long)ii * ldc + jj] += s;
}

}

int lxo_launch_gemm_tn_tr(const GemmTN& p, hipStream_t s) {
    if (p.conv || !p.atomic || p.nbatch != 1 || p.lda % 8 || p.ldb % 8 || (p.I + 7) / 8 * 8 > p.lda || (p.J + 7) / 8 * 8 > p.ldb) return -2;
    if (((uintptr_t)p.A | (uintptr_t)p.B) & 15) return -2;
    if ((long long)p.M * p.lda * 2 >= (1LL << 31) || (long long)p.M * p.ldb * 2 >= (1LL << 31)) return -2;
    {
        static bool done[64] = {};
        int dev = 0;
        const bool known = hipGetDevice(&dev) == hipSuccess && dev >= 0 && dev < 64;
        if (!known || !done[dev]) {
            HIPRC(hipFuncSetAttribute(reinterpret_cast<const void*>(gemm_tn_tr_kernel), hipFuncAttributeMaxDynamicSharedMemorySize, 2 * TSTAGE));
            if (known) done[dev] = true;
        }
    }
    const int tiles = ((p.J + 127) / 128) * ((p.I + 127) / 128);
    const int units = tiles * p.nsplit;
    if (p.det_slab && (size_t)units * 128 * 128 > p.det_floats) return -2;
    dim3 grid(8 * ((units + 7) / 8));
    hipLaunchKernelGGL(gemm_tn_tr_kernel, grid, dim3(256), 2 * TSTAGE, s, p);
    if (p.det_slab)
        hipLaunchKernelGGL(tn_slab_reduce_kernel, dim3(128 * 128 / 256, tiles), dim3(256), 0, s, p.det_slab, p.nsplit, tiles, (p.J + 127) / 128, p.I, p.J, p.C, p.ldc);
    return (int)hipGetLastError();
}
```

### latex_ocr_amd/csrc/model_decoder.hip

```cpp
#include "plan.h"
#include "impl.h"
#include "gemm.h"
#include "head_kernels.h"
#include "grammar.h"
#include "rstep.h"
#include "xdec.h"
#include "dimg.h"
#include "api_util.h"
#include "switches.h"
#include "timing.h"

namespace {
int nt(const Plan& P, bool a_f32, bool c_f32, bool small, const void* A, int lda, const void* Bp, int ldb, void* C, int ldc,
       int M, int N, int K, const float* bias, int act, bool accumulate, hipStream_t st) {
    GemmNT g; memset(&g, 0, sizeof(g));
    g.A = A; g.Bp = Bp; g.C = C; g.M = M; g.N = N; g.K = K; g.lda = lda; g.ldb = ldb; g.ldc = ldc;
    g.bias = bias; g.act = act; g.alpha = 1.f; g.accumulate = accumulate ? 1 : 0; g.addend_rows = 1;
    if (P.s.dtype == LXO_F32) { a_f32 = true; c_f32 = true; }
    return lxo_launch_gemm_nt(P.s.dtype, a_f32, c_f32, small, g, st);
}
int tn(const Plan& P, bool a_f32, bool b_f32, const void* A, int lda, const void* B, int ldb, float* C, int ldc,
       int M, int I, int J, hipStream_t st, DetScratch det = DetScratch{nullptr, 0}) {
    GemmTN g; memset(&g, 0, sizeof(g));
    g.A = A; g.B = B; g.C = C; g.M = M; g.I = I; g.J = J; g.lda = lda; g.ldb = ldb; g.ldc = ldc;
    const int tiles = cdiv(I, 128) * cdiv(J, 128);
    int ns = cdiv(512, tiles);
    const int maxs = M / 64 > 0 ? M / 64 : 1;
    if (ns > maxs) ns = maxs;
    g.nsplit = ns < 1 ? 1 : ns; g.nbatch = 1; g.atomic = 1;
    if (P.bf && P.det()) { if (det.p) { g.det_slab = det.p; g.det_floats = det.floats; } else g.nsplit = 1; }
    if (P.s.dtype == LXO_F32) { a_f32 = true; b_f32 = true; }
    return lxo_launch_gemm_tn(P.s.dtype, a_f32, b_f32, g, st);
}
int slab(const Plan& P, const float* A, int lda, const void* Bp, int ldb, float* out, int M, int N, int K, hipStream_t st) {
    GemmNT g; memset(&g, 0, sizeof(g));
    g.A = A; g.Bp = Bp; g.M = M; g.N = N; g.K = K; g.lda = lda; g.ldb = ldb; g.ldc = N; g.alpha = 1.f; g.addend_rows = 1;
    return lxo_launch_gemm_slab(P.s.dtype, g, out, (long long)M * N, st);
}
Slabs view(const float* p, int K, int M, int N) { Slabs s = {p, K / 128, (long long)M * N, N}; return s; }
const Slabs kNoSlabs = {nullptr, 0, 0, 0};
}

static bool att_alternate() { return lxo_switch(SW_ATT_ALT) != 0; }
static int rs_dense(const Plan& P, const float* A, int lda, const void* W, int ldw, float* out, int ldo, int M, int N, int K,
                    const float* bias, bool tanh_act, bool accumulate, hipStream_t st) {
    RStep a; memset(&a, 0, sizeof(a));
    a.M = M; a.N = N; a.K = K; a.U = P.s.U; a.O = P.s.O; a.zx_row = -1;
    a.A = A; a.lda = lda; a.W = W; a.ldw = ldw; a.out = out; a.ldo = ldo; a.bias = bias; a.accumulate = accumulate ? 1 : 0;
    a.epi = tanh_act ? RS_TANH_O : RS_PLAIN;
    a.dr.inv_keep = 1.f;
    return lxo_launch_rstep(P.s.dtype, 0, a, st);
}

static thread_local hipStream_t g_side = nullptr;
static thread_local hipEvent_t g_ev_fork = nullptr, g_ev_join = nullptr;
int lxo_impl_set_side_stream(hipStream_t s) {
    g_side = s;
    if (s && !g_ev_fork) {
        HIPRC(hipEventCreateWithFlags(&g_ev_fork, hipEventDisableTiming));
        HIPRC(hipEventCreateWithFlags(&g_ev_join, hipEventDisableTiming));
    }
    return 0;
}
static int fork_side(hipStream_t st) { HIPRC(hipEventRecord(g_ev_fork, st)); HIPRC(hipStreamWaitEvent(g_side, g_ev_fork, 0)); return 0; }
static int join_side(hipStream_t st) { HIPRC(hipEventRecord(g_ev_join, g_side)); HIPRC(hipStreamWaitEvent(st, g_ev_join, 0)); return 0; }

static bool rstep_k_ok(int K, bool bf) {
    if (K % 128) return false;
    const int kq = K / 4;
    auto pow2_16 = [](int n) { return n >= 1 && n <= 16 && (n & (n - 1)) == 0; };
    if (bf && kq % 64 == 0 && pow2_16(kq / 64)) return true;
    return kq % 32 == 0 && pow2_16(kq / 32);
}
struct StepPath {
    enum Kernels { SplitK, Fused };
    Kernels shape, loop;
    bool dual, mirrors, try_chain;
};
static StepPath step_path(const Plan& P, bool training) {
    StepPath p;
    p.shape = P.s.step_kernels == 1 ? StepPath::SplitK : StepPath::Fused;
    const int ks[7] = {P.XH, P.s.U, P.HC, P.s.O, P.s.E, 4 * P.s.U, P.s.C};
    for (int k : ks) if (!rstep_k_ok(k, P.bf) || !rstep_k_ok(k, false)) p.shape = StepPath::SplitK;
    p.dual = training && g_side != nullptr && P.s.B >= 2 && (P.s.B % 2) == 0;
    p.loop = p.dual ? StepPath::SplitK : p.shape;
    p.mirrors = P.bf && p.loop == StepPath::Fused;
    p.try_chain = p.mirrors && P.s.step_kernels == 0;
    return p;
}
static int attn_bwd_chunks(const Plan& P, int nr) { return P.det() ? 1 : P.attn_chunks(nr); }

enum { kChainFwd = 0, kChainBwd = 1 };
static unsigned* chain_block(const Plan& P, void* ws, int which) { return P.ws<unsigned>(ws, W_XSYNC) + which * kXDecBlockWords; }
static unsigned* chain_err(const Plan& P, void* ws, int which) { return P.bf ? chain_block(P, ws, which) + kXDecErrWord : nullptr; }

struct InitProj { size_t woff; int n; ParamId bias, weight; float* x; int ldx; };
struct InitProjs { InitProj p[3]; const InitProj* begin() const { return p; } const InitProj* end() const { return p + 3; } };
static InitProjs init_projs(const Plan& P, float* c, int ldc, float* h, int ldh, float* o, int ldo) {
    const size_t blk = (size_t)P.s.U * P.s.C * P.esz;
    return {{{0, P.s.U, P_BC0, P_WC0, c, ldc}, {blk, P.s.U, P_BH0, P_WH0, h, ldh}, {2 * blk, P.s.O, P_BO0, P_WO0, o, ldo}}};
}

static int attention_prepare(const Plan& P, const StepPath& sp, const float* prm, const void* wp, void* ws, int beam, hipStream_t st) {
    const int B = P.s.B, C = P.s.C, E = P.s.E, U = P.s.U, O = P.s.O;
    RC(nt(P, false, false, false, P.ws<void>(ws, W_IMG), C, P.pk(wp, K_ATT_IMG_T), C, P.ws<void>(ws, W_ATT_IMG), E,
          B * P.R, E, C, nullptr, 0, false, st));
    RC(lxo_k_rowmean(P.s.dtype, P.ws<void>(ws, W_IMG), P.ws<float>(ws, W_MEAN), B, P.R, C, st));
    float* rec0 = P.ws<float>(ws, W_REC);
    const char* wt = (const char*)P.pk(wp, K_INIT_T);
    float* mean = P.ws<float>(ws, W_MEAN);
    const InitProjs state = init_projs(P, P.ws<float>(ws, W_CS), U, rec0 + O, P.REC, rec0, P.REC);
    float* tmp = P.ws<float>(ws, W_BEAM_TMP);
    const InitProjs out = beam <= 1 ? state : init_projs(P, tmp, U, tmp + (size_t)B * U, U, tmp + (size_t)2 * B * U, O);
    for (const InitProj& p : out) {
        if (beam <= 1 && sp.shape == StepPath::Fused) RC(rs_dense(P, mean, C, wt + p.woff, C, p.x, p.ldx, B, p.n, C, prm + P.poff[p.bias], true, false, st));
        else RC(nt(P, true, true, true, mean, C, wt + p.woff, C, p.x, p.ldx, B, p.n, C, prm + P.poff[p.bias], 2, false, st));
    }
    for (int i = 0; i < 3 && beam > 1; ++i)
        RC(lxo_k_tile_rows(out.p[i].x, out.p[i].ldx, state.p[i].x, state.p[i].ldx, B * beam, beam, out.p[i].n, st));
    return 0;
}

struct Step {
    const float *zx, *rec_prev, *cs_prev; float *rec_cur, *cs_cur; const bf16_t* recb_prev; bf16_t* recb_cur;
    float *gates, *atth, *alpha;
    const float* dolog; float *g, *dhc, *de, *datth, *dz; bf16_t *gb, *dzb;
};

static int cell_step(const Plan& P, const float* prm, const void* wp, void* ws, int r0, int nr, int beam, const Step& s, Drop dr, hipStream_t st) {
    const int C = P.s.C, E = P.s.E, U = P.s.U, O = P.s.O;
    const size_t r = (size_t)r0;
    float* s1 = P.ws<float>(ws, W_S_K1) + r * (P.XH / 128) * 4 * U;
    float* s2 = P.ws<float>(ws, W_S_K2) + r * (U / 128) * E;
    float* s4 = P.ws<float>(ws, W_S_K4) + r * (P.HC / 128) * O;
    const char* att_img = (const char*)P.ws<void>(ws, W_ATT_IMG) + (r / beam) * P.R * E * P.esz;
    const char* img = (const char*)P.ws<void>(ws, W_IMG) + (r / beam) * P.R * C * P.esz;
    float* part = P.ws<float>(ws, W_APART) + r * 32 * (C + 2);
    RC(slab(P, s.rec_prev, P.REC, P.pk(wp, K_LSTM_RT), P.ldRT, s1, nr, 4 * U, P.XH, st));
    RC(lxo_k_lstm_fwd(s.zx, view(s1, P.XH, nr, 4 * U), s.cs_prev, s.gates, s.cs_cur, s.rec_cur + O, s.rec_cur + P.OFF_HT, P.REC, dr, nr, U, st));
    RC(slab(P, s.rec_cur + P.OFF_HT, P.REC, P.pk(wp, K_ATT_H_T), P.ldAHT, s2, nr, E, U, st));
    RC(lxo_k_attn_fwd(P.s.dtype, att_img, img, nullptr, view(s2, U, nr, E), s.atth,
                      prm + P.poff[P_BETA], s.alpha, part, s.rec_cur + P.OFF_CTX, P.REC, nullptr, 0, nr, P.R, P.Rp, E, C, beam,
                      P.attn_chunks(nr), 0, st));
    RC(slab(P, s.rec_cur + P.OFF_HT, P.REC, P.pk(wp, K_OW_T), P.ldOWT, s4, nr, O, P.HC, st));
    RC(lxo_k_tanh_finalize(view(s4, P.HC, nr, O), s.rec_cur, P.REC, dr, nr, O, st));
    return 0;
}

static int cell_step_fused(const Plan& P, const float* prm, const void* wp, void* ws, int nr, int beam, const Step& s, Drop dr, hipStream_t st,
                           const int* zx_idx = nullptr, int zx_row = -1, const int* a_par = nullptr) {
    const int C = P.s.C, E = P.s.E, U = P.s.U, O = P.s.O;
    const bool bf = P.bf;
    const char* att_img = (const char*)P.ws<void>(ws, W_ATT_IMG);
    const char* img = (const char*)P.ws<void>(ws, W_IMG);
    float* part = P.ws<float>(ws, W_APART);
    RStep a; memset(&a, 0, sizeof(a));
    a.M = nr; a.U = U; a.O = O; a.dr = dr; a.zx_row = -1;
    RStep k1 = a;
    k1.A = bf ? (const void*)s.recb_prev : (const void*)s.rec_prev; k1.lda = bf ? P.RECB : P.REC;
    k1.W = P.pk(wp, K_LSTM_RT); k1.ldw = P.ldRT; k1.N = 4 * U; k1.K = P.XH; k1.epi = RS_LSTM_FWD;
    k1.zx = s.zx; k1.c_prev = s.cs_prev; k1.gates = s.gates; k1.c_out = s.cs_cur;
    k1.zx_idx = zx_idx; k1.zx_vocab = P.s.V; k1.zx_row = zx_row;
    k1.a_par = a_par; k1.a_k = beam;
    k1.out = s.rec_cur + O; k1.out2 = s.rec_cur + P.OFF_HT; k1.ldo = P.REC;
    if (bf) { k1.outb = s.recb_cur + O; k1.out2b = s.recb_cur + P.OFF_HT; k1.ldob = P.RECB; }
    RC(lxo_launch_rstep(P.s.dtype, bf, k1, st));
    RStep k2 = a;
    k2.A = bf ? (const void*)(s.recb_cur + P.OFF_HT) : (const void*)(s.rec_cur + P.OFF_HT); k2.lda = bf ? P.RECB : P.REC;
    k2.W = P.pk(wp, K_ATT_H_T); k2.ldw = P.ldAHT; k2.N = E; k2.K = U; k2.epi = RS_PLAIN;
    k2.out = s.atth; k2.ldo = E;
    RC(lxo_launch_rstep(P.s.dtype, bf, k2, st));
    {
    LxoTimed tm("attn_fwd", "part+combine", (double)nr * P.R * (E + C) * P.esz, st);
    RC(lxo_k_attn_fwd(P.s.dtype, att_img, img, s.atth, kNoSlabs, nullptr,
                      prm + P.poff[P_BETA], s.alpha, part, s.rec_cur + P.OFF_CTX, P.REC, bf ? s.recb_cur + P.OFF_CTX : nullptr, P.RECB, nr, P.R, P.Rp, E, C, beam,
                      P.attn_chunks(nr), att_alternate() ? (dr.t & 1) : 0, st,
                      (!s.gates && P.att_exp()) ? P.ws<void>(ws, W_ATT_EXP) : nullptr));
    }
    RStep k4 = a;
    k4.A = bf ? (const void*)(s.recb_cur + P.OFF_HT) : (const void*)(s.rec_cur + P.OFF_HT); k4.lda = bf ? P.RECB : P.REC;
    k4.W = P.pk(wp, K_OW_T); k4.ldw = P.ldOWT; k4.N = O; k4.K = P.HC; k4.epi = RS_TANH_O;
    k4.out = s.rec_cur; k4.ldo = P.REC;
// ... 7 lines not shown
}
template <class X>
static void xdec_common(X& x, const Plan& P, const float* prm, const void* wp, void* ws) {
    x.Wrt = (const bf16_t*)P.pk(wp, K_LSTM_RT); x.ldrt = P.ldRT;
    x.Wah = (const bf16_t*)P.pk(wp, K_ATT_H_T); x.ldah = P.ldAHT;
    x.Wow = (const bf16_t*)P.pk(wp, K_OW_T); x.ldow = P.ldOWT;
    x.beta = prm + P.poff[P_BETA];
    x.img = P.ws<bf16_t>(ws, W_IMG);
    x.att_exp = P.att_exp() ? P.ws<bf16_t>(ws, W_ATT_EXP) : nullptr;
    x.rec = P.ws<float>(ws, W_REC); x.recb = P.ws<bf16_t>(ws, W_RECB); x.cs = P.ws<float>(ws, W_CS);
    x.part = P.ws<float>(ws, W_APART); x.sync = chain_block(P, ws, kChainFwd);
    x.B = P.s.B; x.R = P.R; x.REC = P.REC; x.RECB = P.RECB;
}

struct Train {
    const Plan& P; const float* prm; const void* wp; void* ws; hipStream_t st;
    StepPath sp;
    float *zx, *rec, *cs, *gates, *atth, *alpha; bf16_t* recb;
    float *dolog, *g, *dhc, *de, *datth, *dz, *dcc, *dxh; bf16_t *gb, *dzb;
    Step step(int t, int r0 = 0) const {
        const int B = P.s.B, U = P.s.U, O = P.s.O, E = P.s.E;
        const size_t p = (size_t)t * B + r0, c = p + B;
        Step s;
        s.zx = zx + p * 4 * U; s.rec_prev = rec + p * P.REC; s.cs_prev = cs + p * U; s.rec_cur = rec + c * P.REC; s.cs_cur = cs + c * U;
        s.recb_prev = recb ? recb + p * P.RECB : nullptr; s.recb_cur = recb ? recb + c * P.RECB : nullptr;
        s.gates = gates + p * 4 * U; s.atth = atth + p * E; s.alpha = alpha + p * P.Rp;
        s.dolog = dolog + p * O; s.g = g + p * O; s.dhc = dhc + p * P.HC; s.de = de + p * P.Rp; s.datth = datth + p * E; s.dz = dz + p * 4 * U;
        s.gb = gb ? gb + p * P.GBP : nullptr; s.dzb = dzb ? dzb + p * P.DZBP : nullptr;
        return s;
    }
};
static Train train_of(const Plan& P, const float* prm, const void* wp, void* ws, hipStream_t st) {
    Train w = {P, prm, wp, ws, st, step_path(P, true),
               P.ws<float>(ws, W_ZX), P.ws<float>(ws, W_REC), P.ws<float>(ws, W_CS), P.ws<float>(ws, W_GATES), P.ws<float>(ws, W_ATTH),
               P.ws<float>(ws, W_ALPHA), P.bf ? P.ws<bf16_t>(ws, W_RECB) : nullptr,
               P.ws<float>(ws, W_DOLOG), P.ws<float>(ws, W_G), P.ws<float>(ws, W_DHC), P.ws<float>(ws, W_DE), P.ws<float>(ws, W_DATTH),
               P.ws<float>(ws, W_DZ), P.ws<float>(ws, W_DCC), P.ws<float>(ws, W_DXH),
               P.bf ? P.ws<bf16_t>(ws, W_GB) : nullptr, P.bf ? P.ws<bf16_t>(ws, W_DZB) : nullptr};
    return w;
}

static int fwd_setup(const Train& w, const int* formula) {
    const Plan& P = w.P; void* ws = w.ws; hipStream_t st = w.st;
    const int B = P.s.B, T = P.s.T, U = P.s.U, D = P.s.D, V = P.s.V;
    RC(attention_prepare(P, w.sp, w.prm, w.wp, ws, 1, st));
    if (P.att_exp()) RC(lxo_k_att_exp(P.ws<void>(ws, W_ATT_IMG), P.ws<void>(ws, W_ATT_EXP), (long long)B * P.R * P.s.E, st));
    RC(lxo_k_embed_gather(P.s.dtype, w.prm + P.poff[P_EMB], w.prm + P.poff[P_START], formula, P.ws<void>(ws, W_EMB_IN), B, T, D, P.Dp, V, st));
    return nt(P, false, true, false, P.ws<void>(ws, W_EMB_IN), P.Dp, P.pk(w.wp, K_LSTM_XT), P.Dp, w.zx, 4 * U, T * B, 4 * U, P.Dp,
              w.prm + P.poff[P_LSTM_B], 0, false, st);
}
static int fwd_chain(const Train& w, const int* lengths, bool* ran) {
    const Plan& P = w.P; void* ws = w.ws;
    RC(mirror_oh(P, ws, 0, P.s.B, w.st));
    XDecFwd x; memset(&x, 0, sizeof(x));
    xdec_common(x, P, w.prm, w.wp, ws);
    x.att_img = P.ws<bf16_t>(ws, W_ATT_IMG);
    x.zx = w.zx; x.gates = w.gates; x.atth = w.atth; x.alpha = w.alpha;
    x.T = P.s.T; x.Rp = P.Rp;
    x.dr = P.drop(0, 0);
    x.lengths = lengths;
    LxoTimed tm("xdec_fwd", "chain", (double)P.s.T * P.s.B * P.R * (P.s.E + P.s.C) * P.esz, w.st);
    const int rc = lxo_launch_xdec_fwd(x, P.s.U, P.s.O, P.s.C, P.s.E, w.st);
    if (rc == 0) *ran = true;
    else if (rc != -2) return rc < 0 ? rc : -rc;
    return 0;
}
static int fwd_fused_loop(const Train& w) {
    const Plan& P = w.P;
    RC(mirror_oh(P, w.ws, 0, P.s.B, w.st));
    for (int t = 0; t < P.s.T; ++t) RC(cell_step_fused(P, w.prm, w.wp, w.ws, P.s.B, 1, w.step(t), P.drop(t, 0), w.st));
    return 0;
}
static int fwd_splitk_loop(const Train& w) {
    const Plan& P = w.P;
    const int nh = w.sp.dual ? 2 : 1, hb = P.s.B / nh;
    if (w.sp.dual) RC(fork_side(w.st));
    for (int t = 0; t < P.s.T; ++t)
        for (int h = 0; h < nh; ++h)
            RC(cell_step(P, w.prm, w.wp, w.ws, h * hb, hb, 1, w.step(t, h * hb), P.drop(t, h * hb), h ? g_side : w.st));
    if (w.sp.dual) RC(join_side(w.st));
    return 0;
}
static int fwd_logits(const Train& w) {
    const Plan& P = w.P;
    const bool m = w.sp.mirrors;
    return nt(P, !m, true, false, m ? (const void*)w.step(0).recb_cur : (const void*)w.step(0).rec_cur, m ? P.RECB : P.REC, P.pk(w.wp, K_YWO_T), P.s.O,
              P.ws<float>(w.ws, W_LOGITS), P.Vp, P.s.T * P.s.B, P.s.V, P.s.O, nullptr, 0, false, w.st);
}

int lxo_impl_decoder_train_fwd(const Plan& P, const float* prm, const void* wp, void* ws, const int* formula, hipStream_t st, const int* lengths) {
    const Train w = train_of(P, prm, wp, ws, st);
    RC(fwd_setup(w, formula));
    bool chain = false;
    if (w.sp.try_chain) RC(fwd_chain(w, lengths, &chain));
    if (P.bf && !chain) HIPRC(hipMemsetAsync(chain_block(P, ws, kChainFwd), 0, kXDecSyncBytes, st));
    if (w.sp.loop == StepPath::SplitK) RC(fwd_splitk_loop(w));
    else if (!chain) RC(fwd_fused_loop(w));
    return fwd_logits(w);
}

int lxo_impl_ce_loss(const Plan& P, void* ws, const int* formula, const int* lengths, float inv_ntok, const float* ntok_dev, hipStream_t st,
                     const float* w_tok, const float* w_row, const float* smooth_eps) {
    HIPRC(hipMemsetAsync(P.ws<float>(ws, W_LOSS), 0, 64, st));
    const CeWeights wt = {w_tok, w_row};
    const CeSmooth sm = {smooth_eps ? *smooth_eps : 0.f, smooth_eps ? *smooth_eps / (float)P.s.V : 0.f};
    RC(lxo_k_ce_loss(P.s.dtype, P.ws<float>(ws, W_LOGITS), formula, lengths, P.ws<void>(ws, W_DLOGITS), P.ws<float>(ws, W_LOSS),
                     inv_ntok, ntok_dev, chain_err(P, ws, kChainFwd), P.s.B, P.s.T, P.s.V, P.Vp,
                     DetScratch{P.ws<float>(ws, W_DET), P.wbytes[W_DET] / 4}, st,
                     (w_tok || w_row) ? &wt : nullptr, smooth_eps ? &sm : nullptr));
    return 0;
}

int lxo_impl_score_tokens(const Plan& P, void* ws, const int* formula, const int* lengths, float* logp_out, int* top1_out, float* seq_out, hipStream_t st) {
    return lxo_k_score(P.s.dtype, P.ws<float>(ws, W_LOGITS), formula, lengths, logp_out, top1_out, seq_out,
                       chain_err(P, ws, kChainFwd), P.s.B, P.s.T, P.s.V, P.Vp, st);
}

int lxo_impl_score_alternatives(const Plan& P, void* ws, const int* formula, const int* lengths, int k, const DecAllow* allow, int* ids_out, float* logp_out,
                                int* rank_out, float* ent_out, hipStream_t st) {
    return lxo_k_score_alt(P.s.dtype, P.ws<float>(ws, W_LOGITS), formula, lengths, k, allow, ids_out, logp_out, rank_out, ent_out,
                           chain_err(P, ws, kChainFwd), P.s.B, P.s.T, P.s.V, P.Vp, st);
}

hipStream_t lxo_impl_encoder_side_stream();
static thread_local hipEvent_t g_dbw_fork = nullptr, g_dbw_fork2 = nullptr, g_dbw_join = nullptr, g_dbw_init = nullptr;
struct BwdStreams {
    hipStream_t main, side;
    hipStream_t deferred() const { return side ? side : main; }
    int fork() const {
        if (!side) return 0;
        if (!g_dbw_fork) for (hipEvent_t* e : {&g_dbw_fork, &g_dbw_fork2, &g_dbw_join, &g_dbw_init}) HIPRC(hipEventCreateWithFlags(e, hipEventDisableTiming));
        HIPRC(hipEventRecord(g_dbw_fork, main));
        HIPRC(hipStreamWaitEvent(side, g_dbw_fork, 0));
        return 0;
    }
    int dmean_ready() const { if (side) HIPRC(hipEventRecord(g_dbw_init, side)); return 0; }
    int wait_dmean() const { if (side) HIPRC(hipStreamWaitEvent(main, g_dbw_init, 0)); return 0; }
    int datt_img_ready() const { if (side) HIPRC(hipEventRecord(g_dbw_fork2, main)); return 0; }
    int wait_datt_img() const { if (side) HIPRC(hipStreamWaitEvent(side, g_dbw_fork2, 0)); return 0; }
    int join(bool defer) const {
        if (!side || defer) return 0;
        HIPRC(hipEventRecord(g_dbw_join, side));
        HIPRC(hipStreamWaitEvent(main, g_dbw_join, 0));
        return 0;
    }
    int record_ready(void* ready) const {
        if (!ready) return 0;
        if (side) { HIPRC(hipEventRecord(g_dbw_fork, main)); HIPRC(hipStreamWaitEvent(side, g_dbw_fork, 0)); }
        HIPRC(hipEventRecord((hipEvent_t)ready, deferred()));
        return 0;
    }
};

static int bwd_logits(const Train& w, float* grads) {
    const Plan& P = w.P; hipStream_t st = w.st;
    const int B = P.s.B, TB = P.s.T * B, O = P.s.O, V = P.s.V;
    const void* dlog = P.ws<void>(w.ws, W_DLOGITS);
    RC(nt(P, false, true, false, dlog, P.Vp, P.pk(w.wp, K_YWO), P.Vp, w.dolog, O, TB, O, P.Vp, nullptr, 0, false, st));
    if (w.sp.mirrors) RC(tn(P, false, false, w.step(0).recb_cur, P.RECB, dlog, P.Vp, grads + P.poff[P_YWO], V, TB, O, V, st, P.det_scratch(w.ws)));
    else RC(tn(P, true, false, w.step(0).rec_cur, P.REC, dlog, P.Vp, grads + P.poff[P_YWO], V, TB, O, V, st));
    if (P.bf) RC(lxo_k_chain_poison(chain_err(P, w.ws, kChainFwd), nullptr, grads + P.ptotal - 1, st));
    return 0;
}
static int bwd_zero_acc(const Train& w) {
    HIPRC(hipMemsetAsync(w.dcc, 0, (size_t)w.P.s.B * w.P.s.U * 4, w.st));
    HIPRC(hipMemsetAsync(w.datth, 0, (size_t)w.P.s.T * w.P.s.B * w.P.s.E * 4, w.st));
    return 0;
}
static int bwd_last_g(const Train& w) {
    const Plan& P = w.P;
    const Step l = w.step(P.s.T - 1);
    return lxo_k_tanh_bwd(l.dolog, P.s.O, kNoSlabs, l.rec_cur, P.REC, l.g, P.s.O, l.gb, P.GBP, P.drop(P.s.T - 1, 0), 0, P.s.B, P.s.O, w.st);
}
static int bwd_chain(const Train& w, bool* ran) {
    const Plan& P = w.P; void* ws = w.ws; const void* wp = w.wp;
    XDecBwd x; memset(&x, 0, sizeof(x));
    x.Wow = (const bf16_t*)P.pk(wp, K_OW); x.ldow = P.ldOW;
    x.Wah = (const bf16_t*)P.pk(wp, K_ATT_H); x.ldah = P.ldAH;
    x.Wk = (const bf16_t*)P.pk(wp, K_LSTM) + (size_t)P.s.D * P.ldK; x.ldk = P.ldK;
    x.beta = w.prm + P.poff[P_BETA];
    x.att_img = P.ws<bf16_t>(ws, W_ATT_IMG); x.img = P.ws<bf16_t>(ws, W_IMG);
    x.att_exp = P.att_exp() ? P.ws<bf16_t>(ws, W_ATT_EXP) : nullptr;
    x.rec = w.rec; x.REC = P.REC; x.cs = w.cs; x.gates = w.gates; x.atth = w.atth; x.alpha = w.alpha; x.Rp = P.Rp;
    x.dolog = w.dolog; x.gall = w.g; x.gb = w.gb; x.GBP = P.GBP; x.dhc = w.dhc; x.de = w.de; x.datth = w.datth; x.datthb = P.ws<bf16_t>(ws, W_DATTHB);
    x.dz = w.dz; x.dzb = w.dzb; x.DZBP = P.DZBP; x.carry_h = P.ws<float>(ws, W_CARRYH); x.dcc = w.dcc; x.dxh = w.dxh;
    x.part = P.ws<float>(ws, W_APART);
    x.sync = chain_block(P, ws, kChainBwd);
    x.T = P.s.T; x.B = P.s.B; x.R = P.R;
    x.dr = P.drop(0, 0);
    LxoTimed tm("xdec_bwd", "chain", (double)P.s.T * P.s.B * P.R * (P.s.E + P.s.C) * P.esz, w.st);
    const int rc = lxo_launch_xdec_bwd(x, P.s.U, P.s.O, P.s.C, P.s.E, w.st);
    if (rc == 0) *ran = true;
    else if (rc != -2) return rc < 0 ? rc : -rc;
    else { RC(bwd_zero_acc(w)); HIPRC(hipMemsetAsync(x.sync, 0, kXDecSyncBytes, w.st)); }
    return 0;
}
static int bwd_fused_loop(const Train& w) {
    const Plan& P = w.P; void* ws = w.ws; const void* wp = w.wp; hipStream_t st = w.st;
    const int B = P.s.B, T = P.s.T, C = P.s.C, E = P.s.E, U = P.s.U, O = P.s.O;
    const bool bf = P.bf;
    float* carry_h = P.ws<float>(ws, W_CARRYH);
    const int nchb = attn_bwd_chunks(P, B);
    RStep a; memset(&a, 0, sizeof(a));
    a.U = U; a.O = O; a.zx_row = -1; a.M = B;
    for (int t = T - 1; t >= 0; --t) {
        const Step s = w.step(t);
        RStep b1 = a;
        b1.A = bf ? (const void*)s.gb : (const void*)s.g; b1.lda = bf ? P.GBP : O;
        b1.W = P.pk(wp, K_OW); b1.ldw = P.ldOW; b1.N = P.HC; b1.K = O; b1.epi = RS_PLAIN;
        b1.out = s.dhc; b1.ldo = P.HC;
        RC(lxo_launch_rstep(P.s.dtype, bf, b1, st));
        const Slabs dc1 = {s.dhc, 1, 0, P.HC};
        {
        LxoTimed tm("attn_bwd", "part", (double)B * P.R * (E + C) * P.esz, st);
        RC(lxo_k_attn_bwd(P.s.dtype, P.ws<void>(ws, W_ATT_IMG), P.att_exp() ? P.ws<void>(ws, W_ATT_EXP) : nullptr, P.ws<void>(ws, W_IMG), s.atth, w.prm + P.poff[P_BETA],
                          s.alpha, dc1, U, nullptr, P.HC, s.rec_cur + P.OFF_CTX, P.REC,
                          s.de, s.datth, B, P.R, P.Rp, E, C, nchb, att_alternate() ? (t & 1) : 0, st));
        }
        RStep b3 = a;
        b3.A = s.datth; b3.lda = E;
        b3.W = P.pk(wp, K_ATT_H); b3.ldw = P.ldAH; b3.N = U; b3.K = E; b3.epi = RS_LSTM_BWD;
        b3.dhm = s.dhc; b3.lddhm = P.HC; b3.carry_h = carry_h; b3.carry_rows = (t == T - 1) ? 0 : B;
        b3.gates_in = s.gates; b3.c_prev = s.cs_prev; b3.c_cur = s.cs_cur;
        b3.dcc = w.dcc; b3.out = s.dz; b3.outb = s.dzb; b3.ldob = P.DZBP; b3.dr = P.drop(t, 0);
        RC(lxo_launch_rstep(P.s.dtype, 0, b3, st));
        RStep b4 = a;
        b4.A = bf ? (const void*)s.dzb : (const void*)s.dz; b4.lda = bf ? P.DZBP : 4 * U;
        b4.W = (const char*)P.pk(wp, K_LSTM) + (size_t)P.s.D * P.ldK * P.esz; b4.ldw = P.ldK; b4.N = P.XH; b4.K = 4 * U; b4.epi = RS_CARRY;
        if (t == 0) { b4.first = 1; b4.out = w.dxh; b4.ldo = P.XH; }
        else {
            const Step q = w.step(t - 1);
            b4.out = q.g; b4.outb = q.gb; b4.ldob = P.GBP; b4.out2 = carry_h;
            b4.dolog = q.dolog; b4.o_prev = s.rec_prev; b4.ldoprev = P.REC;
            b4.dr = P.drop(t - 1, 0);
        }
        RC(lxo_launch_rstep(P.s.dtype, bf, b4, st));
    }
    return 0;
}
static int bwd_splitk_loop(const Train& w) {
    const Plan& P = w.P; void* ws = w.ws; const void* wp = w.wp;
    const int T = P.s.T, C = P.s.C, E = P.s.E, U = P.s.U, O = P.s.O;
    const int nh = w.sp.dual ? 2 : 1, hb = P.s.B / nh;
    const int nchb = attn_bwd_chunks(P, hb);
    auto sb4_of = [&](size_t r0) { return P.ws<float>(ws, W_S_B4) + r0 * (4 * U / 128) * P.XH; };
    if (w.sp.dual) RC(fork_side(w.st));
    for (int t = T - 1; t >= 0; --t) {
        for (int h = 0; h < nh; ++h) {
            const int crows = (t == T - 1) ? 0 : hb;
            hipStream_t sh = h ? g_side : w.st;
            const size_t r0 = (size_t)h * hb;
            const Step s = w.step(t, (int)r0);
            float* sb1 = P.ws<float>(ws, W_S_B1) + r0 * (O / 128) * P.HC;
            float* sb3 = P.ws<float>(ws, W_S_B3) + r0 * (E / 128) * U;
            float* sb4 = sb4_of(r0);
            const char* att_img = (const char*)P.ws<void>(ws, W_ATT_IMG) + r0 * P.R * E * P.esz;
            const char* img = (const char*)P.ws<void>(ws, W_IMG) + r0 * P.R * C * P.esz;
            const Slabs carry = (crows <= 0) ? kNoSlabs : view(sb4, 4 * U, crows, P.XH);
            const Drop dr = P.drop(t, (int)r0);
            RC(lxo_k_tanh_bwd(s.dolog, O, carry, s.rec_cur, P.REC, s.g, O, nullptr, 0, dr, crows, hb, O, sh));
            RC(slab(P, s.g, O, P.pk(wp, K_OW), P.ldOW, sb1, hb, P.HC, O, sh));
            RC(lxo_k_attn_bwd(P.s.dtype, att_img, P.att_exp() ? (const char*)P.ws<void>(ws, W_ATT_EXP) + r0 * P.R * E * P.esz : nullptr, img, s.atth, w.prm + P.poff[P_BETA],
                              s.alpha, view(sb1, O, hb, P.HC), U, s.dhc + U, P.HC, s.rec_cur + P.OFF_CTX, P.REC,
                              s.de, s.datth, hb, P.R, P.Rp, E, C, nchb, 0, sh));
            RC(slab(P, s.datth, E, P.pk(wp, K_ATT_H), P.ldAH, sb3, hb, U, E, sh));
            RC(lxo_k_lstm_bwd(s.gates, s.cs_prev, s.cs_cur, view(sb1, O, hb, P.HC), view(sb3, E, hb, U), carry, O, w.dcc + r0 * U, s.dz, dr, crows, hb, U, sh));
            RC(slab(P, s.dz, 4 * U, (const char*)P.pk(wp, K_LSTM) + (size_t)P.s.D * P.ldK * P.esz, P.ldK, sb4, hb, P.XH, 4 * U, sh));
        }
    }
    if (w.sp.dual) RC(join_side(w.st));
    for (int h = 0; h < nh; ++h) {
        const size_t r0 = (size_t)h * hb;
        RC(lxo_k_slab_reduce(view(sb4_of(r0), 4 * U, hb, P.XH), w.dxh + r0 * P.XH, P.XH, hb, P.XH, w.st));
    }
    return 0;
}
static int bwd_init_states(const Train& w, float* grads, const BwdStreams& s, DetScratch det_s) {
    const Plan& P = w.P; void* ws = w.ws;
    const int B = P.s.B, C = P.s.C, U = P.s.U, O = P.s.O, W3 = 2 * U + O;
    hipStream_t sd = s.deferred();
    float* dpre = P.ws<float>(ws, W_DPRE0); float* mean = P.ws<float>(ws, W_MEAN); float* dmean = P.ws<float>(ws, W_DMEAN);
    { const Slabs one = {w.dxh, 1, 0, P.XH}; RC(lxo_k_init_bwd(w.dcc, one, w.cs, w.rec, P.REC, dpre, B, U, O, sd)); }
    const char* wi = (const char*)P.pk(w.wp, K_INIT);
    const InitProjs pr = init_projs(P, dpre, W3, dpre + U, W3, dpre + 2 * U, W3);
    for (const InitProj& p : pr) {
        const bool acc = &p != pr.p;
        if (w.sp.shape == StepPath::Fused) RC(rs_dense(P, p.x, W3, wi + p.woff, p.n, dmean, C, B, C, p.n, nullptr, false, acc, sd));
        else RC(nt(P, true, true, true, p.x, W3, wi + p.woff, p.n, dmean, C, B, C, p.n, nullptr, 0, acc, sd));
    }
    RC(s.dmean_ready());
    for (const InitProj& p : pr) RC(tn(P, true, true, mean, C, p.x, W3, grads + P.poff[p.weight], p.n, B, C, p.n, sd));
    for (const InitProj& p : pr) RC(lxo_k_colsum(p.x, W3, grads + P.poff[p.bias], B, p.n, det_s, sd));
    return 0;
}
static int bwd_weight_grads(const Train& w, float* grads, bool bwd_chain_ran, const BwdStreams& s, DetScratch det_s) {
    const Plan& P = w.P; void* ws = w.ws; hipStream_t st = w.st, sd = s.deferred();
    const int TB = P.s.T * P.s.B, E = P.s.E, U = P.s.U, O = P.s.O, D = P.s.D;
    auto gw = [&](int pid) { return grads + P.poff[pid]; };
    const bool m = w.sp.mirrors, f = !m;
    const Step s0 = w.step(0);
    const void* rec = m ? (const void*)w.recb : (const void*)w.rec; const int ldr = m ? P.RECB : P.REC;
    const void* hc = m ? (const void*)(s0.recb_cur + P.OFF_HT) : (const void*)(s0.rec_cur + P.OFF_HT);
    const void* g = m ? (const void*)w.gb : (const void*)w.g; const int ldg = m ? P.GBP : O;
    const void* dz = m ? (const void*)w.dzb : (const void*)w.dz; const int ldz = m ? P.DZBP : 4 * U;
    hipStream_t sx = m ? sd : st;
    const DetScratch dx = m ? det_s : DetScratch{nullptr, 0};
    RC(tn(P, f, f, hc, ldr, g, ldg, gw(P_OWH), O, TB, P.HC, O, sx, dx));
    if (bwd_chain_ran) RC(tn(P, f, false, hc, ldr, P.ws<bf16_t>(ws, W_DATTHB), E, gw(P_ATT_H), E, TB, U, E, sx, dx));
    else RC(tn(P, f, true, hc, ldr, w.datth, E, gw(P_ATT_H), E, TB, U, E, sx));
    RC(tn(P, false, f, P.ws<void>(ws, W_EMB_IN), P.Dp, dz, ldz, gw(P_LSTM_K), 4 * U, TB, D, 4 * U, sx, dx));
    RC(tn(P, f, f, rec, ldr, dz, ldz, gw(P_LSTM_K) + (size_t)D * 4 * U, 4 * U, TB, P.XH, 4 * U, sx, dx));
    return lxo_k_colsum(w.dz, 4 * U, gw(P_LSTM_B), TB, 4 * U, det_s, sd);
}
static int bwd_embedding(const Train& w, const int* formula, float* grads, const BwdStreams& s) {
    const Plan& P = w.P; hipStream_t sd = s.deferred();
    const int B = P.s.B, T = P.s.T, TB = T * B, U = P.s.U, D = P.s.D;
    float* demb = P.ws<float>(w.ws, W_DEMB);
    if (w.sp.loop == StepPath::Fused) {
        RStep e; memset(&e, 0, sizeof(e));
        e.M = TB; e.N = D; e.K = 4 * U; e.U = U; e.O = P.s.O; e.zx_row = -1; e.epi = RS_PLAIN; e.dr.inv_keep = 1.f;
        e.A = P.bf ? (const void*)w.dzb : (const void*)w.dz; e.lda = P.bf ? P.DZBP : 4 * U;
        e.W = P.pk(w.wp, K_LSTM); e.ldw = P.ldK; e.out = demb; e.ldo = D;
        RC(lxo_launch_rstep(P.s.dtype, P.bf, e, sd));
    } else
        RC(nt(P, true, true, true, w.dz, 4 * U, P.pk(w.wp, K_LSTM), P.ldK, demb, D, TB, D, 4 * U, nullptr, 0, false, w.st));
    return lxo_k_embed_scatter(demb, formula, grads + P.poff[P_EMB], grads + P.poff[P_START], B, T, D, P.s.V, P.det() ? 1 : 0, sd);
}
static int bwd_datt_img(const Train& w, float* grads) {
    const Plan& P = w.P;
    return lxo_k_datt_img(P.s.dtype, P.ws<void>(w.ws, W_ATT_IMG), w.atth, w.prm + P.poff[P_BETA], w.de, P.ws<void>(w.ws, W_DATTIMG), grads + P.poff[P_BETA],
                          P.s.T, P.s.B, P.R, P.Rp, P.s.E, P.wbytes[W_ATTH_EXP] ? P.ws<float>(w.ws, W_ATTH_EXP) : nullptr, P.det_scratch(w.ws), w.st);
}
static int bwd_dimg_masked(const Train& w, float* grads, const BwdStreams& s) {
    const Plan& P = w.P; void* ws = w.ws;
    const int B = P.s.B;
    const DetScratch det = P.det_scratch(ws);
    RC(bwd_datt_img(w, grads));
    RC(s.datt_img_ready());
    RC(s.wait_dmean());
    DimgArgs a; memset(&a, 0, sizeof(a));
    a.alpha = w.alpha; a.ld_alpha = (long long)B * P.Rp; a.Rp = P.Rp;
    a.dctx = w.dhc + P.s.U; a.ld_dctx = (long long)B * P.HC; a.HC = P.HC;
    a.datt = P.ws<bf16_t>(ws, W_DATTIMG); a.W = (const bf16_t*)P.pk(w.wp, K_ATT_IMG); a.ldw = P.s.E;
    a.dmean = P.ws<float>(ws, W_DMEAN); a.T = P.s.T; a.B = B; a.R = P.R; a.C = P.s.C; a.E = P.s.E;
    a.y6 = P.ws<bf16_t>(ws, W_Y6); a.dy6 = P.ws<bf16_t>(ws, W_DIMG); a.db = grads + P.poff[P_CONV6_B];
    if (P.det()) { a.db_part = det.p; a.db_part_floats = det.floats; }
    return lxo_launch_dimg_fused(a, w.st);
}
static int bwd_dimg_plain(const Train& w, float* grads, const BwdStreams& s) {
    const Plan& P = w.P; void* ws = w.ws; hipStream_t st = w.st;
    const int B = P.s.B, C = P.s.C, E = P.s.E;
    float* dimg = P.ws<float>(ws, W_DIMG);
    GemmTN g; memset(&g, 0, sizeof(g));
    g.A = w.alpha; g.B = w.dhc + P.s.U; g.C = dimg; g.M = P.s.T; g.I = P.R; g.J = C;
    g.lda = B * P.Rp; g.ldb = B * P.HC; g.ldc = C;
    g.nsplit = 1; g.nbatch = B; g.strideA = P.Rp; g.strideB = P.HC; g.strideC = (long long)P.R * C; g.atomic = 0;
    RC(lxo_launch_gemm_tn(P.s.dtype, 1, 1, g, st));
    RC(s.wait_dmean());
    RC(lxo_k_add_mean_grad(dimg, P.ws<float>(ws, W_DMEAN), B, P.R, C, st));
    RC(bwd_datt_img(w, grads));
    RC(s.datt_img_ready());
    return nt(P, false, true, false, P.ws<void>(ws, W_DATTIMG), E, P.pk(w.wp, K_ATT_IMG), E, dimg, C, B * P.R, C, E, nullptr, 0, true, st);
}

int lxo_impl_decoder_train_bwd(const Plan& P, const float* prm, const void* wp, void* ws, const int* formula, float* grads,
                               int parts, hipStream_t st, bool defer_join, void* ready) {
    const Train w = train_of(P, prm, wp, ws, st);
    if (parts & 1) RC(bwd_logits(w, grads));
    if (!(parts & 2)) return 0;
    bool chain = false;
    if (!w.sp.try_chain) {
        RC(bwd_zero_acc(w));
        if (P.bf) HIPRC(hipMemsetAsync(chain_block(P, ws, kChainBwd), 0, kXDecSyncBytes, st));
    }
    if (w.sp.loop == StepPath::SplitK) RC(bwd_splitk_loop(w));
    else {
        RC(bwd_last_g(w));
        if (w.sp.try_chain) RC(bwd_chain(w, &chain));
        if (!chain) RC(bwd_fused_loop(w));
    }
    const BwdStreams s = {st, (w.sp.mirrors && !lxo_timer_on()) ? lxo_impl_encoder_side_stream() : nullptr};
    const DetScratch det_s = s.side ? P.det_scratch_side(ws) : P.det_scratch(ws);
    RC(s.fork());
    RC(bwd_init_states(w, grads, s, det_s));
    RC(bwd_weight_grads(w, grads, chain, s, det_s));
    RC(P.dimg_masked() ? bwd_dimg_masked(w, grads, s) : bwd_dimg_plain(w, grads, s));
    RC(bwd_embedding(w, formula, grads, BwdStreams{st, nullptr}));
    RC(s.wait_datt_img());
    RC(tn(P, false, false, P.ws<void>(ws, W_IMG), P.s.C, P.ws<void>(ws, W_DATTIMG), P.s.E, grads + P.poff[P_ATT_IMG], P.s.E, P.s.B * P.R, P.s.C, P.s.E,
          s.deferred(), det_s));
    RC(s.join(defer_join));
    if (chain) RC(lxo_k_chain_poison(nullptr, chain_err(P, ws, kChainBwd), grads + P.ptotal - 1, st));
    return s.record_ready(ready);
}

struct Dec {
    int k, nv;
    bool beam;
    int *flags, *finished;
    int *ids_step, *par_step;
    float *logp, *tmp;
    float *rec, *cs; bf16_t* recb;
    float *logits, *alpha;
    StepPath path;
    bool fused() const { return path.shape == StepPath::Fused; }
};
static Dec dec_of(const Plan& P, void* ws, int k, bool beam) {
    Dec d;
    d.k = k; d.nv = P.s.B * k; d.beam = beam;
    d.flags = P.ws<int>(ws, W_DEC_FLAGS); d.finished = d.flags + 64;
    d.ids_step = P.ws<int>(ws, W_DEC_IDS); d.par_step = P.ws<int>(ws, W_BEAM_PAR);
    d.logp = P.ws<float>(ws, W_BEAM_LP); d.tmp = P.ws<float>(ws, W_BEAM_TMP);
    d.rec = P.ws<float>(ws, W_REC); d.cs = P.ws<float>(ws, W_CS);
    d.logits = P.ws<float>(ws, W_DEC_LOGITS); d.alpha = P.ws<float>(ws, W_ALPHA);
    d.path = step_path(P, false);
    d.recb = d.path.mirrors ? P.ws<bf16_t>(ws, W_RECB) : nullptr;
    return d;
}
static int decode_token_table(const Plan& P, const float* prm, const void* wp, void* ws, hipStream_t st) {
    const int U = P.s.U, D = P.s.D, V = P.s.V;
    RC(lxo_k_embed_table(P.s.dtype, prm + P.poff[P_EMB], prm + P.poff[P_START], P.ws<void>(ws, W_DEC_TXE), V, D, P.Dp, st));
    RC(nt(P, false, true, false, P.ws<void>(ws, W_DEC_TXE), P.Dp, P.pk(wp, K_LSTM_XT), P.Dp, P.ws<float>(ws, W_DEC_TX), 4 * U, V + 1, 4 * U, P.Dp,
          prm + P.poff[P_LSTM_B], 0, false, st));
    return 0;
}
static int decode_common_step(const Plan& P, const float* prm, const void* wp, void* ws, const Dec& d, int time, const int* ids_prev, hipStream_t st, const int* a_par = nullptr) {
    const int U = P.s.U, O = P.s.O, D = P.s.D, V = P.s.V, nv = d.nv;
    const size_t cur = (size_t)((time + 1) & 1) * nv, prev = (size_t)(time & 1) * nv;
    Step s; memset(&s, 0, sizeof(s));
    s.rec_prev = d.rec + prev * P.REC; s.cs_prev = d.cs + prev * U; s.rec_cur = d.rec + cur * P.REC; s.cs_cur = d.cs + cur * U;
    if (d.recb) { s.recb_prev = d.recb + prev * P.RECB; s.recb_cur = d.recb + cur * P.RECB; }
    s.atth = P.ws<float>(ws, W_ATTH); s.alpha = d.alpha;
    if (d.fused()) {
        s.zx = P.ws<float>(ws, W_DEC_TX);
        RC(cell_step_fused(P, prm, wp, ws, nv, d.k, s, Drop{0u, 1.f, 0u, (time + 1) & 1, 0, 0}, st,
                           ids_prev, ids_prev ? -1 : V, ids_prev ? a_par : nullptr));
    } else {
        float* zx = P.ws<float>(ws, W_DEC_ZX);
        RC(lxo_k_embed_rows(P.s.dtype, prm + P.poff[P_EMB], prm + P.poff[P_START], ids_prev, P.ws<void>(ws, W_DEC_EMB), nv, D, P.Dp, V, st));
        RC(nt(P, false, true, false, P.ws<void>(ws, W_DEC_EMB), P.Dp, P.pk(wp, K_LSTM_XT), P.Dp, zx, 4 * U, nv, 4 * U, P.Dp,
              prm + P.poff[P_LSTM_B], 0, false, st));
        s.zx = zx;
        RC(cell_step(P, prm, wp, ws, 0, nv, d.k, s, Drop{0u, 1.f, 0u, 0, 0, 0}, st));
    }
    if (d.fused() && V % 4 == 0) {
        RStep e; memset(&e, 0, sizeof(e));
        e.M = nv; e.N = V; e.K = O; e.U = U; e.O = O; e.zx_row = -1; e.epi = RS_PLAIN; e.dr.inv_keep = 1.f;
        e.A = P.bf ? (const void*)s.recb_cur : (const void*)s.rec_cur;
        e.lda = P.bf ? P.RECB : P.REC;
        e.W = P.pk(wp, K_YWO_T); e.ldw = O; e.out = d.logits; e.ldo = P.Vp;
        const int rc = lxo_launch_rstep(P.s.dtype, P.bf, e, st);
        if (rc != -2) return rc < 0 ? rc : -rc;
    }
    return nt(P, true, true, nv <= 64, s.rec_cur, P.REC, P.pk(wp, K_YWO_T), O, d.logits, P.Vp, nv, V, O, nullptr, 0, false, st);
}

namespace {
struct DecodePoll { int* host; hipEvent_t ev[2]; bool ok; };
thread_local DecodePoll g_poll = {nullptr, {nullptr, nullptr}, false};
int poll_init() {
    if (g_poll.ok) return 0;
    HIPRC(hipHostMalloc((void**)&g_poll.host, 2 * 64 * sizeof(int), 0));
    HIPRC(hipEventCreateWithFlags(&g_poll.ev[0], hipEventDisableTiming));
    HIPRC(hipEventCreateWithFlags(&g_poll.ev[1], hipEventDisableTiming));
    g_poll.ok = true;
    return 0;
}
}
template <typename EnqueueFn>
static int decode_loop(int max_iter, int steps_per_enqueue, int counter_words, int* flags, hipStream_t st, int* steps_out, EnqueueFn enqueue) {
    RC(poll_init());
    if (steps_per_enqueue > counter_words) steps_per_enqueue = counter_words;
    int enq = 0;
    int nchunks = 0;
    int steps = -1;
    auto enqueue_chunk = [&]() -> int {
        const int slot = nchunks & 1;
        int* dflags = flags + slot * 32;
        HIPRC(hipMemsetAsync(dflags, 0, counter_words * sizeof(int), st));
        int n = max_iter + 1 - enq; if (n > steps_per_enqueue) n = steps_per_enqueue;
        RC(enqueue(enq, n, dflags));
        enq += n;
        HIPRC(hipMemcpyAsync(g_poll.host + slot * 64, dflags, counter_words * sizeof(int), hipMemcpyDeviceToHost, st));
        HIPRC(hipEventRecord(g_poll.ev[slot], st));
        g_poll.host[slot * 64 + 32] = n;
        g_poll.host[slot * 64 + 33] = enq - n;
        ++nchunks;
        return 0;
    };
    RC(enqueue_chunk());
    int checked = 0;
    while (steps < 0) {
        if (enq <= max_iter) RC(enqueue_chunk());
        const int slot = checked & 1;
        HIPRC(hipEventSynchronize(g_poll.ev[slot]));
        const int n = g_poll.host[slot * 64 + 32], first = g_poll.host[slot * 64 + 33];
        for (int c = 0; c < n; ++c) {
            if ((g_poll.host[slot * 64 + c] & 0xffff) == 0 || first + c >= max_iter) { steps = first + c + 1; break; }
        }
        ++checked;
        if (steps < 0 && checked == nchunks && enq > max_iter) steps = enq;
    }
    if (nchunks > checked) HIPRC(hipEventSynchronize(g_poll.ev[(nchunks - 1) & 1]));
    if (steps_out) *steps_out = steps;
    return 0;
}
template <typename StepFn>
static int decode_loop_steps(int max_iter, int* flags, hipStream_t st, int* steps_out, StepFn step) {
    return decode_loop(max_iter, 8, 8, flags, st, steps_out, [&](int first, int n, int* unfinished) -> int {
        for (int c = 0; c < n; ++c) RC(step(first + c, unfinished + c));
        return 0;
    });
}

static int decode_check(const Plan& P, int k, int steps_needed, const DecPrefix* prefix, const DecAllow* allow = nullptr) {
    if (P.s.max_steps < steps_needed || k < 1 || k > 16 || k > P.s.V) return -5;
    if (prefix && (!prefix->ids || !prefix->len || prefix->ld < 1)) return -5;
    if (allow && (!allow->bits || (allow->ld != 0 && allow->ld < (P.s.V + 31) / 32))) return -5;
    return 0;
}
static int decode_setup(const Plan& P, const float* prm, const void* wp, void* ws, const Dec& d, bool again, hipStream_t st) {
    RC(attention_prepare(P, d.path, prm, wp, ws, d.k, st));
    if (!again && P.att_exp())
        RC(lxo_k_att_exp(P.ws<void>(ws, W_ATT_IMG), P.ws<void>(ws, W_ATT_EXP), (long long)P.s.B * P.R * P.s.E, st));
    if (d.fused()) RC(mirror_oh(P, ws, 0, d.nv, st));
    HIPRC(hipMemsetAsync(d.flags, 0, 256 + (size_t)d.nv * 4, st));
    if (again) return 0;
    if (d.beam) HIPRC(hipMemsetAsync(d.logp, 0, (size_t)d.nv * 4, st));
    if (d.fused()) RC(decode_token_table(P, prm, wp, ws, st));
    return 0;
}
static int decode_keep_alpha(const Plan& P, const Dec& d, int time, const DecodeOuts& o, hipStream_t st) {
    if (o.alpha) HIPRC(hipMemcpyAsync(o.alpha + (size_t)time * d.nv * P.Rp, d.alpha, (size_t)d.nv * P.Rp * 4, hipMemcpyDeviceToDevice, st));
    return 0;
}
struct DecGram { bool on; GrammarArgs a; DecAllow rows; int* depth; };
static DecGram decode_grammar(const Plan& P, const Dec& d, int id_end, int max_iter, const DecodeOuts& o) {
    DecGram g; memset(&g, 0, sizeof(g));
    if (!o.grammar) return g;
    g.on = true;
    g.a = GrammarArgs{o.grammar->cls, o.grammar->n_kinds, o.grammar->max_depth, o.grammar->budget, o.allow ? o.allow->bits : nullptr,
                      o.allow ? o.allow->ld : 0, o.grammar->scratch, d.nv, d.k, P.s.V, id_end, max_iter};
    g.rows = DecAllow{lxo_k_grammar_sets(g.a), (P.s.V + 31) / 32, 1};
    g.depth = o.grammar->depth;
    return g;
// ... 166 lines not shown
```

### latex_ocr_amd/csrc/plan.hip

```cpp
#include "plan.h"
#include <stdio.h>
#include <string.h>
#include "switches.h"

static const char* kParamNames[P_COUNT] = {
    "Encoder/convolutional_encoder/conv2d/kernel", "Encoder/convolutional_encoder/conv2d/bias",
    "Encoder/convolutional_encoder/conv2d_1/kernel", "Encoder/convolutional_encoder/conv2d_1/bias",
    "Encoder/convolutional_encoder/conv2d_2/kernel", "Encoder/convolutional_encoder/conv2d_2/bias",
    "Encoder/convolutional_encoder/conv2d_3/kernel", "Encoder/convolutional_encoder/conv2d_3/bias",
    "Encoder/convolutional_encoder/conv2d_4/kernel", "Encoder/convolutional_encoder/conv2d_4/bias",
    "Encoder/convolutional_encoder/conv2d_strided/kernel", "Encoder/convolutional_encoder/conv2d_strided/bias",
    "Encoder/convolutional_encoder/conv2d_5/kernel", "Encoder/convolutional_encoder/conv2d_5/bias",
    "Encoder/row_encoder/bidirectional_rnn/fw/lstm_cell/kernel", "Encoder/row_encoder/bidirectional_rnn/fw/lstm_cell/bias",
    "Encoder/row_encoder/bidirectional_rnn/bw/lstm_cell/kernel", "Encoder/row_encoder/bidirectional_rnn/bw/lstm_cell/bias",
    "Decoder/embedding_table", "Decoder/start_token",
    "Decoder/AttentionCell/att_img/kernel",
    "Decoder/AttentionCell/att_mechanism/W_c_0", "Decoder/AttentionCell/att_mechanism/b_c_0",
    "Decoder/AttentionCell/att_mechanism/W_h_0", "Decoder/AttentionCell/att_mechanism/b_h_0",
    "Decoder/AttentionCell/att_mechanism/W_o_0", "Decoder/AttentionCell/att_mechanism/b_o_0",
    "Decoder/AttentionCell/rnn/lstm_cell/kernel", "Decoder/AttentionCell/rnn/lstm_cell/bias",
    "Decoder/AttentionCell/rnn/att_mechanism/dense/kernel", "Decoder/AttentionCell/rnn/att_mechanism/att_beta",
    "Decoder/AttentionCell/rnn/o_W_h", "Decoder/AttentionCell/rnn/o_W_c", "Decoder/AttentionCell/rnn/y_W_o",
};
const char* lxo_param_name(int id) { return (id >= 0 && id < P_COUNT) ? kParamNames[id] : ""; }
const char* lxo_param_name_mode(int id, int encoder_cnn) {
    if (encoder_cnn) {
        switch (id) {
        case P_CONVS_W: return "Encoder/convolutional_encoder/conv2d_5/kernel";
        case P_CONVS_B: return "Encoder/convolutional_encoder/conv2d_5/bias";
        case P_CONV6_W: return "Encoder/convolutional_encoder/conv2d_6/kernel";
        case P_CONV6_B: return "Encoder/convolutional_encoder/conv2d_6/bias";
        default: break;
        }
    }
    return lxo_param_name(id);
}

static const char* kWsNames[W_COUNT] = {
    "p1", "y2", "p2", "y3", "y4", "p4", "y5", "p5", "y6", "img", "pos",
    "att_img", "att_part", "mean", "emb_in", "zx", "rec", "cs", "gates", "att_h", "alpha", "logits",
    "dlogits", "loss", "do_log", "g", "dhc", "de", "datth", "dz", "dxh", "dcc", "d_img", "d_att_img",
    "d_emb", "dpre0", "dmean", "g0", "g1", "g2", "gnorm",
    "s_k1", "s_k2", "s_k4", "s_b1", "s_b3", "s_b4",
    "recb", "gb", "dzb", "carry_h", "dec_tx", "dec_txe",
    "dec_ids", "dec_flags", "dec_emb", "dec_zx", "dec_logits", "beam_lp", "beam_par", "beam_tmp",
    "cols",
    "rxt", "rzx", "rg", "rc", "rh", "rhb", "rdz", "rdzb", "rdh", "rdcc", "rzero",
    "m2", "m4", "m5",
    "att_exp", "xdec_sync", "det_part", "datth_b", "atth_exp",
};
const char* lxo_ws_name(int id) { return (id >= 0 && id < W_COUNT) ? kWsNames[id] : ""; }

static inline int cd2(int n) { return (n + 1) / 2; }
static inline size_t al256(size_t n) { return (n + 255) / 256 * 256; }

Plan::Plan(const lxo_shape& sh, int ) : s(sh) {
    bf = s.dtype == LXO_BF16;
    esz = bf ? 2 : 4;
    const int B = s.B, C = s.C, E = s.E, U = s.U, O = s.O, D = s.D, V = s.V, T = s.T > 0 ? s.T : 1;
    H1 = cd2(s.H); W1 = cd2(s.W);
    H2 = cd2(H1); W2 = cd2(W1);
    cnn = s.encoder_cnn != 0;
    rnn = s.encoder_rnn != 0;
    Be = (s.live_B > 0 && s.live_B < s.B && !rnn) ? s.live_B : s.B;
    Ur = C / 2;
    H4 = cnn ? H2 : cd2(H2);
    W5 = cd2(W2);
    H6 = cnn ? cd2(H2) : H4;
    Hp = H6 - 2; Wp = W5 - 2;
    R = Hp > 0 && Wp > 0 ? Hp * Wp : 0;
    const int ci[6] = {1, 64, 128, 256, 256, C}, co[6] = {64, 128, 256, 256, C, C};
    const int wid[6] = {P_CONV1_W, P_CONV2_W, P_CONV3_W, P_CONV4_W, P_CONV5_W, P_CONV6_W};
    for (int i = 0; i < 6; ++i) { convCin[i] = ci[i]; convCout[i] = co[i]; convW[i] = wid[i]; convB[i] = wid[i] + 1; }
    Vp = (V + 31) / 32 * 32;
    Dp = (D + 63) / 64 * 64;
    Rp = (R + 7) / 8 * 8;
    XH = O + U; HC = U + C; OFF_HT = O + U; OFF_CTX = O + 2 * U; REC = O + 2 * U + C;
    const int WPAD = 128;
    ldRT = XH + WPAD; ldAHT = U + WPAD; ldOWT = HC + WPAD; ldOW = O + WPAD; ldAH = E + WPAD; ldK = 4 * U + WPAD;
    RECB = REC + WPAD; GBP = O + WPAD; DZBP = 4 * U + WPAD;

    long long cnt[P_COUNT];
    for (int i = 0; i < 6; ++i) { cnt[convW[i]] = 9LL * ci[i] * co[i]; cnt[convB[i]] = co[i]; }
    cnt[P_CONVS_W] = cnn ? 8LL * C * C : 0; cnt[P_CONVS_B] = cnn ? C : 0;
    cnt[P_ROWF_K] = cnt[P_ROWB_K] = rnn ? (long long)(C + Ur) * 4 * Ur : 0; cnt[P_ROWF_B] = cnt[P_ROWB_B] = rnn ? 4LL * Ur : 0;
    cnt[P_EMB] = (long long)V * D; cnt[P_START] = D; cnt[P_ATT_IMG] = (long long)C * E;
    cnt[P_WC0] = (long long)C * U; cnt[P_BC0] = U; cnt[P_WH0] = (long long)C * U; cnt[P_BH0] = U;
    cnt[P_WO0] = (long long)C * O; cnt[P_BO0] = O;
    cnt[P_LSTM_K] = (long long)(D + O + U) * 4 * U; cnt[P_LSTM_B] = 4LL * U;
    cnt[P_ATT_H] = (long long)U * E; cnt[P_BETA] = E;
    cnt[P_OWH] = (long long)U * O; cnt[P_OWC] = (long long)C * O; cnt[P_YWO] = (long long)O * V;
    ptotal = 0;
    for (int i = 0; i < P_COUNT; ++i) { poff[i] = ptotal; pcount[i] = cnt[i]; ptotal += cnt[i]; }

    size_t kb[K_COUNT];
    for (int l = 1; l < 6; ++l) {
        kb[K_CONV2_F + l - 1] = (size_t)co[l] * 9 * ci[l] * esz;
        kb[K_CONV2_D + l - 1] = (size_t)ci[l] * 9 * co[l] * esz;
    }
    kb[K_ATT_IMG_T] = (size_t)E * C * esz; kb[K_ATT_IMG] = (size_t)C * E * esz;
    kb[K_INIT_T] = (size_t)(2 * U + O) * C * esz; kb[K_INIT] = (size_t)C * (2 * U + O) * esz;
    kb[K_LSTM_XT] = (size_t)4 * U * Dp * esz; kb[K_LSTM_RT] = (size_t)4 * U * ldRT * esz;
    kb[K_LSTM] = (size_t)(D + O + U) * ldK * esz;
    kb[K_ATT_H_T] = (size_t)E * ldAHT * esz; kb[K_ATT_H] = (size_t)U * ldAH * esz;
    kb[K_OW_T] = (size_t)O * ldOWT * esz; kb[K_OW] = (size_t)HC * ldOW * esz;
    kb[K_YWO_T] = (size_t)V * O * esz; kb[K_YWO] = (size_t)O * Vp * esz;
    kb[K_CONVS_F] = cnn ? (size_t)8 * C * C * esz : 0; kb[K_CONVS_D] = kb[K_CONVS_F];
    for (int d = 0; d < 2; ++d) {
        kb[K_ROWX_T + d] = rnn ? (size_t)4 * Ur * C * esz : 0; kb[K_ROWX + d] = kb[K_ROWX_T + d];
        kb[K_ROWH_T + d] = rnn ? (size_t)4 * Ur * Ur * esz : 0; kb[K_ROWH + d] = kb[K_ROWH_T + d];
    }
    ktotal = 0;
    for (int i = 0; i < K_COUNT; ++i) { koff[i] = ktotal; ktotal += al256(kb[i] + 64); }

    const size_t f4 = 4;
    size_t wb[W_COUNT];
    memset(wb, 0, sizeof(wb));
    const size_t BL = (size_t)B;
    wb[W_P1] = BL * H1 * W1 * 64 * esz;
    wb[W_Y2] = BL * H1 * W1 * 128 * esz;  wb[W_P2] = BL * H2 * W2 * 128 * esz;
    wb[W_Y3] = BL * H2 * W2 * 256 * esz;  wb[W_Y4] = BL * H2 * W2 * 256 * esz;
    wb[W_P4] = cnn ? 0 : BL * H4 * W2 * 256 * esz;
    wb[W_Y5] = BL * H4 * W2 * C * esz;    wb[W_P5] = BL * H6 * W5 * C * esz;
    wb[W_COLS] = cnn ? BL * H6 * W5 * 8 * C * esz : 0;
    wb[W_Y6] = BL * R * C * esz;          wb[W_IMG] = BL * R * C * esz;
    wb[W_POS] = (size_t)R * C * f4;
    if (rnn) {
        const size_t TM = (size_t)B * (Hp > 0 ? Hp : 0) * (Wp > 0 ? Wp : 0), Mr = (size_t)B * (Hp > 0 ? Hp : 0);
        wb[W_RXT] = TM * C * esz;
        wb[W_RZX] = 2 * TM * 4 * Ur * f4;
        wb[W_RG] = 2 * TM * 4 * Ur * f4; wb[W_RC] = 2 * TM * Ur * f4; wb[W_RH] = 2 * TM * Ur * f4;
        wb[W_RHB] = bf ? 2 * TM * Ur * 2 : 0;
        wb[W_RDZ] = 2 * TM * 4 * Ur * f4; wb[W_RDZB] = bf ? 2 * TM * 4 * Ur * 2 : 0;
        wb[W_RDH] = TM * C * f4; wb[W_RDCC] = 2 * Mr * Ur * f4; wb[W_RZERO] = Mr * 4 * Ur * f4;
    }
    wb[W_M2] = bf ? BL * H2 * W2 * 128 : 0;
    wb[W_M4] = (bf && !cnn) ? BL * H4 * W2 * 256 : 0;
    wb[W_M5] = (bf && !cnn) ? BL * H6 * W5 * C : 0;
    wb[W_ATT_EXP] = bf ? BL * R * E * esz : 0;
    wb[W_XSYNC] = bf ? 2 * ((size_t)4096 + (384u << 10)) : 8192;
    wb[W_DET] = 8192;
    if (!bf || s.deterministic) {
        size_t need = BL * (size_t)((R + 15) / 16) * E * f4;
        const size_t floor_ = (size_t)1024 * (4 * U > 2048 ? 4 * U : 2048) * f4;
        wb[W_DET] = need > floor_ ? need : floor_;
        const size_t wg = (size_t)264 * 9 * 64 * 128 * f4;
        if (bf && wb[W_DET] < wg) wb[W_DET] = wg;
        if (bf) wb[W_DET] = 2 * ((wb[W_DET] + 255) / 256 * 256);
    }
    const int nb = s.beam > 1 ? s.beam : 1;
    const size_t BK_ = BL * nb;
    const size_t TB = (size_t)T * B;
    wb[W_DATTHB] = bf ? TB * E * 2 : 0;
    wb[W_ATTH_EXP] = (bf && E <= 256) ? TB * E * f4 : 0;
    wb[W_ATT_IMG] = BL * R * E * esz;
    wb[W_APART] = BK_ * 32 * (C + 16) * f4;
    wb[W_MEAN] = BL * C * f4;
    wb[W_EMB_IN] = TB * Dp * esz;
    wb[W_ZX] = TB * 4 * U * f4;
    wb[W_REC] = (size_t)(T + 1) * B * REC * f4;
    wb[W_CS] = (size_t)(T + 1) * B * U * f4;
    wb[W_GATES] = TB * 4 * U * f4;
    wb[W_ATTH] = TB * E * f4;
    wb[W_ALPHA] = TB * Rp * f4;
    wb[W_LOGITS] = TB * Vp * f4;
    wb[W_DLOGITS] = TB * Vp * esz;
    wb[W_LOSS] = 64;
    wb[W_DOLOG] = TB * O * f4;
    wb[W_G] = TB * O * f4;
    wb[W_DHC] = TB * HC * f4;
    wb[W_DE] = TB * Rp * f4;
    wb[W_DATTH] = TB * E * f4;
    wb[W_DZ] = TB * 4 * U * f4;
    wb[W_DXH] = BL * XH * f4;
    wb[W_DCC] = BL * U * f4;
    wb[W_DIMG] = BL * R * C * f4;
    wb[W_DATTIMG] = BL * R * E * esz;
    wb[W_DEMB] = TB * D * f4;
    wb[W_DPRE0] = BL * (2 * U + O) * f4;
    wb[W_DMEAN] = BL * C * f4;
    size_t gmax = wb[W_Y2];
    const size_t cand[] = {wb[W_P1], wb[W_P2], wb[W_Y3], wb[W_Y4], wb[W_P4], wb[W_Y5], wb[W_P5], wb[W_Y6]};
    for (size_t c : cand) if (c > gmax) gmax = c;
    wb[W_G0] = gmax; wb[W_G1] = gmax; wb[W_G2] = gmax;
    wb[W_GNORM] = 64;
    wb[W_S_K1] = (size_t)(XH / 128) * BK_ * 4 * U * f4;
    wb[W_S_K2] = (size_t)(U / 128) * BK_ * E * f4;
    wb[W_S_K4] = (size_t)(HC / 128) * BK_ * O * f4;
    wb[W_S_B1] = (size_t)(O / 128) * BL * HC * f4;
    wb[W_S_B3] = (size_t)(E / 128) * BL * U * f4;
    wb[W_S_B4] = (size_t)(4 * U / 128) * BL * XH * f4;
    wb[W_RECB] = bf ? (size_t)(T + 1) * B * RECB * 2 : 0;
    wb[W_GB] = bf ? TB * GBP * 2 : 0;
    wb[W_DZB] = bf ? TB * DZBP * 2 : 0;
    wb[W_CARRYH] = BL * U * f4;
    const int ms = s.max_steps > 0 ? s.max_steps : 0;
    if (ms > 0) {
        wb[W_DEC_IDS] = BK_ * ms * 4 + 64;
        wb[W_DEC_FLAGS] = 256 + BK_ * 4;
        wb[W_DEC_EMB] = BK_ * Dp * esz;
        wb[W_DEC_TX] = (size_t)(V + 1) * 4 * U * f4;
        wb[W_DEC_TXE] = (size_t)(V + 1) * Dp * esz;
        wb[W_DEC_ZX] = BK_ * 4 * U * f4;
        wb[W_DEC_LOGITS] = BK_ * Vp * f4;
        wb[W_BEAM_LP] = BK_ * 2 * f4;
        wb[W_BEAM_PAR] = BK_ * ms * 4;
        wb[W_BEAM_TMP] = 3 * (BK_ * REC + BK_ * U) * f4 / 3 + BK_ * 64;
        if (wb[W_BEAM_TMP] < BK_ * Vp * f4) wb[W_BEAM_TMP] = BK_ * Vp * f4;
        const size_t recd = 2 * BK_ * REC * f4, csd = 2 * BK_ * U * f4;
        if (wb[W_REC] < recd) wb[W_REC] = recd;
        if (bf && wb[W_RECB] < 2 * BK_ * RECB * 2) wb[W_RECB] = 2 * BK_ * RECB * 2;
        if (wb[W_CS] < csd) wb[W_CS] = csd;
        if (wb[W_GATES] < BK_ * 4 * U * f4) wb[W_GATES] = BK_ * 4 * U * f4;
        if (wb[W_ATTH] < BK_ * E * f4) wb[W_ATTH] = BK_ * E * f4;
        if (wb[W_ALPHA] < BK_ * Rp * f4) wb[W_ALPHA] = BK_ * Rp * f4;
        if (wb[W_ZX] < BK_ * 4 * U * f4) wb[W_ZX] = BK_ * 4 * U * f4;
    }
    wtotal = 0;
    for (int i = 0; i < W_COUNT; ++i) { wbytes[i] = wb[i]; woff[i] = wtotal; wtotal += al256(wb[i] + 256); }
}

int Plan::attn_chunks(int nv) const {
    constexpr int target = 512;
    int nch = (target + nv - 1) / nv;
    if (nch > 16) nch = 16;
    const int by_rows = R / 32 > 0 ? R / 32 : 1;
    if (nch > by_rows) nch = by_rows;
    const int need = (R + 1023) / 1024;
    if (nch < need) nch = need;
    return nch < 1 ? 1 : nch;
}

int Plan::validate(char* msg, size_t n) const {
#define BAD(cond, text) if (cond) { snprintf(msg, n, "lxo_shape invalid: %s", text); return -10; }
    BAD(s.B <= 0 || s.H <= 0 || s.W <= 0, "B/H/W must be positive");
    BAD(Hp <= 0 || Wp <= 0, "image too small: need ceil(H/8) >= 3 and ceil(W/8) >= 3");
    BAD(s.V < 4, "V < 4");
    BAD(s.C != 512 && s.C != 256 && s.C != 128, "C must be 128/256/512");
    BAD(s.E % 128 || s.U % 128 || s.O % 128 || s.E <= 0 || s.U <= 0 || s.O <= 0, "E, U, O must be positive multiples of 128");
    BAD(s.D % 8 || s.D <= 0, "D must be a positive multiple of 8");
    BAD(s.dtype != LXO_F32 && s.dtype != LXO_BF16, "dtype");
    BAD(s.E > 1024 || s.C > 512, "E <= 1024, C <= 512");
    BAD(R > 16384, "more than 16384 regions");
    BAD(s.encoder_rnn && s.C != 512 && s.C != 256, "encoder_rnn needs C in {256, 512} (C/2 units per direction, multiples of 128)");
#undef BAD
    return 0;
}

bool Plan::att_exp() const {
    return bf && lxo_switch(SW_ATT_EXP) && s.E <= 256 && (long long)s.B * R * s.E % 8 == 0;
}
bool Plan::pool_fused() const {
    return bf && lxo_switch(SW_POOL_FUSED) && lxo_switch(SW_CONV_2WG) && s.C % 128 == 0;
}
Drop Plan::drop(int t, int row0) const {
    Drop d = {0u, 1.f, (unsigned)s.dropout_seed, t, row0, s.B};
    if (s.keep_prob > 0.f && s.keep_prob < 1.f) {
        d.thr = (unsigned)(s.keep_prob * 16777216.0f);
        if (d.thr == 0u) d.thr = 1u;
        d.inv_keep = 1.f / s.keep_prob;
    }
    return d;
}
```

### latex_ocr_amd/csrc/switches.h

```cpp
#pragma once

enum LxoSwitch {
    SW_ATT_ALT, SW_ATT_EXP, SW_BEAM_FAST, SW_BEAM_INDIRECT, SW_RSTEP_MT16, SW_GEMM_NT_DMA, SW_GEMM_TN_TR, SW_WGRAD_HALO,
    SW_POOL_FUSED, SW_CONV1_MFMA, SW_CONV_2WG, SW_CONV_SMALL, SW_XDEC, SW_XDEC_DEC, SW_XDEC_BWD, SW_XDEC_DEC_CHUNK,
    SW_COUNT
};
int lxo_switch(LxoSwitch s);
#ifdef LXO_DIAG
int lxo_conv_diag();
#endif
```

### latex_ocr_amd/csrc/switches.hip

```cpp
#include "switches.h"
#include <stdlib.h>

namespace {
enum Kind { arm, value, live };
struct Row { const char* name; Kind kind; int def; };
const Row kSwitches[SW_COUNT] = {
    {"LXO_ATT_ALT", arm, 1},
    {"LXO_ATT_EXP", arm, 1},
    {"LXO_BEAM_FAST", arm, 1},
    {"LXO_BEAM_INDIRECT", arm, 1},
    {"LXO_RSTEP_MT16", arm, 1},
    {"LXO_GEMM_NT_DMA", arm, 1},
    {"LXO_GEMM_TN_TR", arm, 1},
    {"LXO_WGRAD_HALO", arm, 1},
    {"LXO_POOL_FUSED", arm, 1},
    {"LXO_CONV1_MFMA", arm, 1},
    {"LXO_CONV_2WG", arm, 1},
    {"LXO_CONV_SMALL", value, 256},
    {"LXO_XDEC", arm, 1},
    {"LXO_XDEC_DEC", arm, 1},
    {"LXO_XDEC_BWD", arm, 1},
    {"LXO_XDEC_DEC_CHUNK", live, 0},
};
int read(const Row& r) {
    const char* e = getenv(r.name);
    if (!e) return r.def;
    return r.kind == arm ? e[0] != '0' : atoi(e);
}
struct Cache {
    int v[SW_COUNT];
    Cache() { for (int i = 0; i < SW_COUNT; ++i) v[i] = read(kSwitches[i]); }
};
}

int lxo_switch(LxoSwitch s) {
    static const Cache cache;
    return kSwitches[s].kind == live ? read(kSwitches[s]) : cache.v[s];
}
#ifdef LXO_DIAG
int lxo_conv_diag() {
    static const int diag = [] { const char* e = getenv("LXO_CONV_DIAG"); return e ? atoi(e) : 0; }();
    return diag;
}
#endif
```

Baseline: 9043 img/s.

## Group decoder weight-gradient TN GEMMs into one launch and vectorize slab reductions

Adds a grouped TN GEMM launcher that runs up to eight weight-gradient products (O_W_h, att_h, LSTM kernel halves, and the deferred y_W_o gradient) in a single kernel plus a single slab-reduce kernel. The y_W_o gradient moves off the main stream into the deferred side stream. The slab reductions in both the TN and conv wgrad paths now read float4 with unrolled loads, and the embedding-gradient compaction drops two barriers per chunk and unrolls its gather deeper. This is meant to cut launch count and under-filled grids and to improve reduction bandwidth. In exchange the deterministic scratch grows, and the switch is read from the environment on every call.

```diff
diff --git a/include/lxo.h b/include/lxo.h
--- a/include/lxo.h
+++ b/include/lxo.h
@@ -22,6 +22,9 @@
 
 int lxo_gemm_tn(int dt, int a_f32, int b_f32, const void* A, const void* B, float* C,
                 int M, int I, int J, int lda, int ldb, int ldc, int nsplit, int atomic, void* stream);
+
+int lxo_gemm_tn_group(int n, const void* const* A, const void* const* B, float* const* C, const int* dims, float* slab, size_t slab_floats,
+                      void* stream);
 
 int lxo_gemm_slab(int dt, const void* A, const void* Bp, float* slab, int M, int N, int K, int lda, int ldb, int ldc,
                   long long slab_stride, void* stream);
diff --git a/latex_ocr_amd/_abi.py b/latex_ocr_amd/_abi.py
--- a/latex_ocr_amd/_abi.py
+++ b/latex_ocr_amd/_abi.py
@@ -46,6 +46,7 @@
         "lxo_ws_region_dtype": (c_int, [S, ctypes.c_char_p]),
         "lxo_gemm_nt": (c_int, [c_int] * 4 + [c_void] * 3 + [c_int] * 6 + [c_void, c_int, c_float, c_int, c_void]),
         "lxo_gemm_tn": (c_int, [c_int] * 3 + [c_void] * 3 + [c_int] * 8 + [c_void]),
+        "lxo_gemm_tn_group": (c_int, [c_int, c_void, c_void, c_void, c_void, c_void, c_size, c_void]),
         "lxo_conv3x3": (c_int, [c_int, c_void, c_void, c_void, c_void] + [c_int] * 9 + [c_void]),
         "lxo_conv3x3_ex": (c_int, [c_int, c_void, c_void, c_void, c_void] + [c_int] * 9 + [c_void, c_int, c_void, c_void, c_void, c_void]),
         "lxo_conv3x3_wgrad": (c_int, [c_int, c_void, c_void, c_void] + [c_int] * 8 + [c_void]),
@@ -136,7 +137,7 @@
     return lib
 
 
-ENTRY_POINTS = ["lxo_last_error", "lxo_version", "lxo_shape_size", "lxo_ws_region_dtype", "lxo_timing_enable", "lxo_timing_count", "lxo_timing_get", "lxo_gemm_nt", "lxo_gemm_tn", "lxo_conv3x3", "lxo_conv3x3_ex", "lxo_conv3x3_wgrad", "lxo_gemm_slab", "lxo_attention_fwd", "lxo_param_num", "lxo_param_name", "lxo_param_name_for",
+ENTRY_POINTS = ["lxo_last_error", "lxo_version", "lxo_shape_size", "lxo_ws_region_dtype", "lxo_timing_enable", "lxo_timing_count", "lxo_timing_get", "lxo_gemm_nt", "lxo_gemm_tn", "lxo_gemm_tn_group", "lxo_conv3x3", "lxo_conv3x3_ex", "lxo_conv3x3_wgrad", "lxo_gemm_slab", "lxo_attention_fwd", "lxo_param_num", "lxo_param_name", "lxo_param_name_for",
                 "lxo_param_total", "lxo_param_info", "lxo_wpack_bytes", "lxo_workspace_bytes", "lxo_ws_region",
                 "lxo_pack_weights", "lxo_encoder_fwd", "lxo_encoder_bwd", "lxo_encoder_bwd_ready", "lxo_train_bwd", "lxo_set_side_stream", "lxo_set_encoder_side_stream", "lxo_decoder_train_fwd", "lxo_decoder_train_fwd_live",
                 "lxo_ce_loss_fwd_bwd", "lxo_ce_loss_fwd_bwd_dev", "lxo_ce_loss_weighted", "lxo_ce_loss_smoothed", "lxo_mrt_weights", "lxo_edit_distance", "lxo_text_stats", "lxo_mrt_candidates", "lxo_consensus", "lxo_sentence_bleu", "lxo_consensus_bleu", "lxo_mrt_candidates_cost", "lxo_decoder_train_bwd", "lxo_decoder_train_bwd_part", "lxo_global_norm_scale", "lxo_adam_step", "lxo_optimizer_step",
diff --git a/latex_ocr_amd/csrc/api.hip b/latex_ocr_amd/csrc/api.hip
--- a/latex_ocr_amd/csrc/api.hip
+++ b/latex_ocr_amd/csrc/api.hip
@@ -31,6 +31,19 @@
     p.A = A; p.B = B; p.C = C; p.M = M; p.I = I; p.J = J; p.lda = lda; p.ldb = ldb; p.ldc = ldc;
     p.nsplit = nsplit; p.nbatch = 1; p.atomic = atomic;
     CHECK_LAUNCH(lxo_launch_gemm_tn(dt, a_f32, b_f32, p, (hipStream_t)stream), "lxo_gemm_tn");
+    return 0;
+}
+
+extern "C" int lxo_gemm_tn_group(int n, const void* const* A, const void* const* B, float* const* C, const int* dims, float* slab,
+                                 size_t slab_floats, void* stream) {
+    if (n < 1 || n > kTnGroupMax || !A || !B || !C || !dims) return fail(-2, "lxo_gemm_tn_group: 1 .. 8 products");
+    GemmTN p[kTnGroupMax]; memset(p, 0, sizeof(p));
+    for (int k = 0; k < n; ++k) {
+        const int* d = dims + 7 * k;
+        p[k].A = A[k]; p[k].B = B[k]; p[k].C = C[k]; p[k].M = d[0]; p[k].I = d[1]; p[k].J = d[2]; p[k].lda = d[3]; p[k].ldb = d[4]; p[k].ldc = d[5];
+        p[k].nsplit = d[6]; p[k].nbatch = 1; p[k].atomic = 1;
+    }
+    CHECK_LAUNCH(lxo_launch_gemm_tn_tr_group(p, n, slab, slab_floats, (hipStream_t)stream), "lxo_gemm_tn_group");
     return 0;
 }
 
diff --git a/latex_ocr_amd/csrc/conv_wgrad.hip b/latex_ocr_amd/csrc/conv_wgrad.hip
--- a/latex_ocr_amd/csrc/conv_wgrad.hip
+++ b/latex_ocr_amd/csrc/conv_wgrad.hip
@@ -221,13 +221,25 @@
 __global__ __launch_bounds__(256) void wgrad_slab_reduce_kernel(const float* __restrict__ slab, int nsplit, int ntiles, int tiles_co, int Cin, int Cout,
                                                                float* __restrict__ dw, int ldc) {
     const int tile = blockIdx.y;
-    const int i = blockIdx.x * 256 + threadIdx.x;
+    const int i = (blockIdx.x * 256 + threadIdx.x) * 4;
     if (i >= 9 * WCI * WCO) return;
     const int co = i % WCO, ci = (i / WCO) % WCI, tap = i / (WCO * WCI);
     const int ci0 = (tile / tiles_co) * WCI, co0 = (tile % tiles_co) * WCO;
-    float s = 0.f;
-    for (int q = 0; q < nsplit; ++q) s += slab[((long long)q * ntiles + tile) * (9 * WCI * WCO) + i];
-    if (co0 + co < Cout) dw[(long long)(tap * Cin + ci0 + ci) * ldc + co0 + co] += s;
+    const f32x4* __restrict__ src = reinterpret_cast<const f32x4*>(slab + (long long)tile * (9 * WCI * WCO) + i);
+    const long long stride = (long long)ntiles * (9 * WCI * WCO / 4);
+    f32x4 s = {0.f, 0.f, 0.f, 0.f};
+    int q = 0;
+    for (; q + 16 <= nsplit; q += 16) {
+        f32x4 v[16];
+#pragma unroll
+        for (int u = 0; u < 16; ++u) v[u] = src[(q + u) * stride];
+#pragma unroll
+        for (int u = 0; u < 16; ++u) s += v[u];
+    }
+    for (; q < nsplit; ++q) s += src[q * stride];
+    float* const out = dw + (long long)(tap * Cin + ci0 + ci) * ldc + co0 + co;
+#pragma unroll
+    for (int e = 0; e < 4; ++e) if (co0 + co + e < Cout) out[e] += s[e];
 }
 
 }
@@ -271,10 +283,10 @@
     const int nsplit8 = (nsplit + 7) / 8 * 8;
     if (q.det_slab) {
         const size_t need = (size_t)nsplit * tiles * 9 * WCI * WCO;
-        if (need > q.det_floats) return -6;
+        if (need > q.det_floats || ((uintptr_t)q.det_slab & 15)) return -6;
     }
     hipLaunchKernelGGL(conv_wgrad_kernel, dim3(tiles * nsplit8), dim3(WTHREADS), 2 * WSTAGE, s, q, tiles_co, tiles_x, tiles_y, nblocks, nsplit, stagger);
     if (q.det_slab)
-        hipLaunchKernelGGL(wgrad_slab_reduce_kernel, dim3(9 * WCI * WCO / 256, tiles), dim3(256), 0, s, q.det_slab, nsplit, tiles, tiles_co, p.Cin, p.J, p.C, p.ldc);
+        hipLaunchKernelGGL(wgrad_slab_reduce_kernel, dim3(9 * WCI * WCO / 1024, tiles), dim3(256), 0, s, q.det_slab, nsplit, tiles, tiles_co, p.Cin, p.J, p.C, p.ldc);
     return (int)hipGetLastError();
 }
diff --git a/latex_ocr_amd/csrc/decoder_kernels.hip b/latex_ocr_amd/csrc/decoder_kernels.hip
--- a/latex_ocr_amd/csrc/decoder_kernels.hip
+++ b/latex_ocr_amd/csrc/decoder_kernels.hip
@@ -1078,7 +1078,7 @@
     __shared__ int list[CH];
     __shared__ float part[256];
     __shared__ int cnt;
-    __shared__ int wcnt[4];
+    __shared__ int wcnt[2][4];
     const int id = blockIdx.x;
     const int tid = threadIdx.x;
     const int rpw = 256 / D, r = tid / D, c = tid - r * D;
@@ -1090,7 +1090,8 @@
         if (tid == 0) cnt = 0;
         __syncthreads();
         if (det) {
-            for (int jb = base; jb < min(s1, base + CH); jb += 256) {
+            int have = 0, it = 0;
+            for (int jb = base; jb < min(s1, base + CH); jb += 256, ++it) {
                 const int j = jb + tid;
                 int row = -1;
                 if (j < min(s1, base + CH)) {
@@ -1100,15 +1101,14 @@
                 }
                 const unsigned long long m = __ballot(row >= 0);
                 const int lane = tid & 63, wv = tid >> 6;
-                if (lane == 0) wcnt[wv] = __builtin_popcountll(m);
+                if (lane == 0) wcnt[it & 1][wv] = __builtin_popcountll(m);
                 __syncthreads();
-                int off = cnt;
-                for (int w = 0; w < wv; ++w) off += wcnt[w];
+                const int c0 = wcnt[it & 1][0], c1 = wcnt[it & 1][1], c2 = wcnt[it & 1][2], c3 = wcnt[it & 1][3];
+                const int off = have + (wv > 0 ? c0 : 0) + (wv > 1 ? c1 : 0) + (wv > 2 ? c2 : 0);
                 if (row >= 0) list[off + __builtin_popcountll(m & ((1ull << lane) - 1ull))] = row;
-                __syncthreads();
-                if (tid == 0) cnt += wcnt[0] + wcnt[1] + wcnt[2] + wcnt[3];
-                __syncthreads();
-            }
+                have += c0 + c1 + c2 + c3;
+            }
+            if (tid == 0) cnt = have;
         } else
         for (int j = base + tid; j < min(s1, base + CH); j += 256) {
             const int b = j / T, tt = j - b * T;
@@ -1120,12 +1120,12 @@
         __syncthreads();
         const int n = cnt;
         if (r < rpw) {
-            for (int k = r; k < n; k += 4 * rpw) {
-                float v[4];
-#pragma unroll
-                for (int u = 0; u < 4; ++u) { const int kk = min(k + u * rpw, n - 1); v[u] = demb[(long long)list[kk] * D + c]; }
-#pragma unroll
-                for (int u = 0; u < 4; ++u) if (k + u * rpw < n) sum += v[u];
+            for (int k = r; k < n; k += 16 * rpw) {
+                float v[16];
+#pragma unroll
+                for (int u = 0; u < 16; ++u) { const int kk = min(k + u * rpw, n - 1); v[u] = demb[(long long)list[kk] * D + c]; }
+#pragma unroll
+                for (int u = 0; u < 16; ++u) if (k + u * rpw < n) sum += v[u];
             }
         }
         __syncthreads();
diff --git a/latex_ocr_amd/csrc/gemm.h b/latex_ocr_amd/csrc/gemm.h
--- a/latex_ocr_amd/csrc/gemm.h
+++ b/latex_ocr_amd/csrc/gemm.h
@@ -43,4 +43,16 @@
 
 int lxo_launch_gemm_tn_tr(const GemmTN& p, hipStream_t s);
 
+constexpr int kTnGroupMax = 8;
+int lxo_launch_gemm_tn_tr_group(const GemmTN* probs, int n, float* det_slab, size_t det_floats, hipStream_t s);
+
+inline int lxo_tn_nsplit(int M, int I, int J) {
+    const int tiles = ((I + 127) / 128) * ((J + 127) / 128);
+    if (tiles < 1) return 1;
+    int ns = (512 + tiles - 1) / tiles;
+    const int maxs = M / 64 > 0 ? M / 64 : 1;
+    if (ns > maxs) ns = maxs;
+    return ns < 1 ? 1 : ns;
+}
+
 int lxo_launch_conv_wgrad(const GemmTN& p, hipStream_t s);
diff --git a/latex_ocr_amd/csrc/gemm_tn_tr.hip b/latex_ocr_amd/csrc/gemm_tn_tr.hip
--- a/latex_ocr_amd/csrc/gemm_tn_tr.hip
+++ b/latex_ocr_amd/csrc/gemm_tn_tr.hip
@@ -1,5 +1,6 @@
 #include "gemm.h"
 #include "api_util.h"
+#include <string.h>
 
 namespace {
 
@@ -19,13 +20,13 @@
 
 namespace {
 
-__global__ __launch_bounds__(256) void gemm_tn_tr_kernel(GemmTN p) {
+LXO_DEV void tntr_unit(const GemmTN& p, const unsigned L) {
     const int tid = threadIdx.x, lane = tid & 63, wave = tid >> 6;
     const int wi = wave >> 1, wj = wave & 1;
     const int tj_n = (p.J + 127) / 128, ti_n = (p.I + 127) / 128, tiles = tj_n * ti_n;
     const int units = tiles * p.nsplit, per_xcd = (units + 7) / 8;
-    const int unit = (int)(blockIdx.x & 7) * per_xcd + (int)(blockIdx.x >> 3);
-    if ((int)(blockIdx.x >> 3) >= per_xcd || unit >= units) return;
+    const int unit = (int)(L & 7) * per_xcd + (int)(L >> 3);
+    if ((int)(L >> 3) >= per_xcd || unit >= units) return;
     const int split = unit / tiles, tile = unit - split * tiles;
     const int i0 = (tile / tj_n) * 128, j0 = (tile % tj_n) * 128;
     const int per = ((p.M + p.nsplit - 1) / p.nsplit + TBR - 1) / TBR * TBR;
@@ -130,37 +131,113 @@
     }
 }
 
-__global__ __launch_bounds__(256) void tn_slab_reduce_kernel(const float* __restrict__ slab, int nsplit, int tiles, int tj_n, int I, int J, float* __restrict__ C, int ldc) {
-    const int tile = blockIdx.y;
-    const int i = blockIdx.x * 256 + threadIdx.x;
+struct TnRed { const float* slab; float* C; int nsplit, tiles, tj_n, I, J, ldc; };
+LXO_DEV void tn_slab_reduce_tile(const TnRed& q, const int tile) {
+    const int i = (blockIdx.x * 256 + threadIdx.x) * 4;
     const int r = i >> 7, c = i & 127;
-    const int ii = (tile / tj_n) * 128 + r, jj = (tile % tj_n) * 128 + c;
-    float s = 0.f;
-    for (int q = 0; q < nsplit; ++q) s += slab[((long long)q * tiles + tile) * (128 * 128) + i];
-    if (ii < I && jj < J) C[(long long)ii * ldc + jj] += s;
-}
+    const int ii = (tile / q.tj_n) * 128 + r, jj = (tile % q.tj_n) * 128 + c;
+    const f32x4* __restrict__ src = reinterpret_cast<const f32x4*>(q.slab + (long long)tile * (128 * 128) + i);
+    const long long stride = (long long)q.tiles * (128 * 128 / 4);
+    f32x4 s = {0.f, 0.f, 0.f, 0.f};
+    int k = 0;
+    for (; k + 8 <= q.nsplit; k += 8) {
+        f32x4 v[8];
+#pragma unroll
+        for (int u = 0; u < 8; ++u) v[u] = src[(k + u) * stride];
+#pragma unroll
+        for (int u = 0; u < 8; ++u) s += v[u];
+    }
+    for (; k < q.nsplit; ++k) s += src[k * stride];
+    if (ii < q.I)
+#pragma unroll
+        for (int e = 0; e < 4; ++e) if (jj + e < q.J) q.C[(long long)ii * q.ldc + jj + e] += s[e];
+}
+
+__global__ __launch_bounds__(256) void gemm_tn_tr_kernel(GemmTN p) { tntr_unit(p, blockIdx.x); }
+__global__ __launch_bounds__(256) void tn_slab_reduce_kernel(TnRed q) { tn_slab_reduce_tile(q, blockIdx.y); }
+
+struct TnGroup { GemmTN p[kTnGroupMax]; unsigned first[kTnGroupMax + 1]; };
+struct TnRedGroup { TnRed q[kTnGroupMax]; int tile0[kTnGroupMax + 1]; };
+__global__ __launch_bounds__(256) void gemm_tn_tr_group_kernel(TnGroup g) {
+    int k = 0;
+#pragma unroll
+    for (int j = 1; j < kTnGroupMax; ++j) k += blockIdx.x >= g.first[j] ? 1 : 0;
+    tntr_unit(g.p[k], blockIdx.x - g.first[k]);
+}
+__global__ __launch_bounds__(256) void tn_slab_reduce_group_kernel(TnRedGroup g) {
+    int k = 0;
+#pragma unroll
+    for (int j = 1; j < kTnGroupMax; ++j) k += (int)blockIdx.y >= g.tile0[j] ? 1 : 0;
+    tn_slab_reduce_tile(g.q[k], (int)blockIdx.y - g.tile0[k]);
+}
+
+int tntr_tiles(const GemmTN& p) { return ((p.J + 127) / 128) * ((p.I + 127) / 128); }
+bool tntr_takes(const GemmTN& p) {
+    if (p.conv || !p.atomic || p.nbatch != 1 || p.lda % 8 || p.ldb % 8 || (p.I + 7) / 8 * 8 > p.lda || (p.J + 7) / 8 * 8 > p.ldb) return false;
+    if (((uintptr_t)p.A | (uintptr_t)p.B) & 15) return false;
+    if ((long long)p.M * p.lda * 2 >= (1LL << 31) || (long long)p.M * p.ldb * 2 >= (1LL << 31)) return false;
+    return true;
+}
+int tntr_lds_attr(const void* kernel, bool* done) {
+    int dev = 0;
+    const bool known = hipGetDevice(&dev) == hipSuccess && dev >= 0 && dev < 64;
+    if (!known || !done[dev]) {
+        HIPRC(hipFuncSetAttribute(kernel, hipFuncAttributeMaxDynamicSharedMemorySize, 2 * TSTAGE));
+        if (known) done[dev] = true;
+    }
+    return 0;
+}
+TnRed tntr_red(const GemmTN& p) { return TnRed{p.det_slab, p.C, p.nsplit, tntr_tiles(p), (p.J + 127) / 128, p.I, p.J, p.ldc}; }
 
 }
 
 int lxo_launch_gemm_tn_tr(const GemmTN& p, hipStream_t s) {
-    if (p.conv || !p.atomic || p.nbatch != 1 || p.lda % 8 || p.ldb % 8 || (p.I + 7) / 8 * 8 > p.lda || (p.J + 7) / 8 * 8 > p.ldb) return -2;
-    if (((uintptr_t)p.A | (uintptr_t)p.B) & 15) return -2;
-    if ((long long)p.M * p.lda * 2 >= (1LL << 31) || (long long)p.M * p.ldb * 2 >= (1LL << 31)) return -2;
-    {
-        static bool done[64] = {};
-        int dev = 0;
-        const bool known = hipGetDevice(&dev) == hipSuccess && dev >= 0 && dev < 64;
-        if (!known || !done[dev]) {
-            HIPRC(hipFuncSetAttribute(reinterpret_cast<const void*>(gemm_tn_tr_kernel), hipFuncAttributeMaxDynamicSharedMemorySize, 2 * TSTAGE));
-            if (known) done[dev] = true;
-        }
-    }
-    const int tiles = ((p.J + 127) / 128) * ((p.I + 127) / 128);
+    if (!tntr_takes(p)) return -2;
+    static bool done[64] = {};
+    RC(tntr_lds_attr(reinterpret_cast<const void*>(gemm_tn_tr_kernel), done));
+    const int tiles = tntr_tiles(p);
     const int units = tiles * p.nsplit;
-    if (p.det_slab && (size_t)units * 128 * 128 > p.det_floats) return -2;
+    if (p.det_slab && ((size_t)units * 128 * 128 > p.det_floats || ((uintptr_t)p.det_slab & 15))) return -2;
     dim3 grid(8 * ((units + 7) / 8));
     hipLaunchKernelGGL(gemm_tn_tr_kernel, grid, dim3(256), 2 * TSTAGE, s, p);
-    if (p.det_slab)
-        hipLaunchKernelGGL(tn_slab_reduce_kernel, dim3(128 * 128 / 256, tiles), dim3(256), 0, s, p.det_slab, p.nsplit, tiles, (p.J + 127) / 128, p.I, p.J, p.C, p.ldc);
+    if (p.det_slab) hipLaunchKernelGGL(tn_slab_reduce_kernel, dim3(128 * 128 / 1024, tiles), dim3(256), 0, s, tntr_red(p));
     return (int)hipGetLastError();
 }
+
+int lxo_launch_gemm_tn_tr_group(const GemmTN* probs, int n, float* det_slab, size_t det_floats, hipStream_t s) {
+    if (n < 1 || n > kTnGroupMax || ((uintptr_t)det_slab & 15)) return -2;
+    const size_t unit_floats = 128 * 128;
+    int order[kTnGroupMax], per[kTnGroupMax];
+    for (int k = 0; k < n; ++k) {
+        const GemmTN& p = probs[k];
+        if (p.M <= 0 || p.I <= 0 || p.J <= 0 || p.nsplit < 1 || !tntr_takes(p)) return -2;
+        if (det_slab && (size_t)tntr_tiles(p) * p.nsplit * unit_floats > det_floats) return -2;
+        per[k] = ((p.M + p.nsplit - 1) / p.nsplit + TBR - 1) / TBR * TBR;
+        int at = k;
+        for (; at > 0 && per[order[at - 1]] < per[k]; --at) order[at] = order[at - 1];
+        order[at] = k;
+    }
+    static bool done[64] = {};
+    RC(tntr_lds_attr(reinterpret_cast<const void*>(gemm_tn_tr_group_kernel), done));
+    for (int beg = 0; beg < n;) {
+        TnGroup g; TnRedGroup r;
+        memset(&g, 0, sizeof(g)); memset(&r, 0, sizeof(r));
+        size_t used = 0;
+        unsigned wgs = 0;
+        int m = 0, tiles_all = 0;
+        for (; beg + m < n; ++m) {
+            GemmTN p = probs[order[beg + m]];
+            const int tiles = tntr_tiles(p), units = tiles * p.nsplit;
+            if (det_slab && used + (size_t)units * unit_floats > det_floats) break;
+            p.det_slab = det_slab ? det_slab + used : nullptr; p.det_floats = det_slab ? (size_t)units * unit_floats : 0;
+            g.p[m] = p; g.first[m] = wgs; r.q[m] = tntr_red(p); r.tile0[m] = tiles_all;
+            used += (size_t)units * unit_floats; wgs += 8u * (unsigned)((units + 7) / 8); tiles_all += tiles;
+        }
+        if (m < 1 || (det_slab && used > det_floats)) return -6;
+        for (int j = m; j <= kTnGroupMax; ++j) { g.first[j] = wgs; r.tile0[j] = tiles_all; }
+        hipLaunchKernelGGL(gemm_tn_tr_group_kernel, dim3(wgs), dim3(256), 2 * TSTAGE, s, g);
+        if (det_slab) hipLaunchKernelGGL(tn_slab_reduce_group_kernel, dim3(128 * 128 / 1024, tiles_all), dim3(256), 0, s, r);
+        beg += m;
+    }
+    return (int)hipGetLastError();
+}
diff --git a/latex_ocr_amd/csrc/model_decoder.hip b/latex_ocr_amd/csrc/model_decoder.hip
--- a/latex_ocr_amd/csrc/model_decoder.hip
+++ b/latex_ocr_amd/csrc/model_decoder.hip
@@ -19,15 +19,15 @@
     if (P.s.dtype == LXO_F32) { a_f32 = true; c_f32 = true; }
     return lxo_launch_gemm_nt(P.s.dtype, a_f32, c_f32, small, g, st);
 }
+static GemmTN tn_prob(const void* A, int lda, const void* B, int ldb, float* C, int ldc, int M, int I, int J) {
+    GemmTN g; memset(&g, 0, sizeof(g));
+    g.A = A; g.B = B; g.C = C; g.M = M; g.I = I; g.J = J; g.lda = lda; g.ldb = ldb; g.ldc = ldc;
+    g.nsplit = lxo_tn_nsplit(M, I, J); g.nbatch = 1; g.atomic = 1;
+    return g;
+}
 int tn(const Plan& P, bool a_f32, bool b_f32, const void* A, int lda, const void* B, int ldb, float* C, int ldc,
        int M, int I, int J, hipStream_t st, DetScratch det = DetScratch{nullptr, 0}) {
-    GemmTN g; memset(&g, 0, sizeof(g));
-    g.A = A; g.B = B; g.C = C; g.M = M; g.I = I; g.J = J; g.lda = lda; g.ldb = ldb; g.ldc = ldc;
-    const int tiles = cdiv(I, 128) * cdiv(J, 128);
-    int ns = cdiv(512, tiles);
-    const int maxs = M / 64 > 0 ? M / 64 : 1;
-    if (ns > maxs) ns = maxs;
-    g.nsplit = ns < 1 ? 1 : ns; g.nbatch = 1; g.atomic = 1;
+    GemmTN g = tn_prob(A, lda, B, ldb, C, ldc, M, I, J);
     if (P.bf && P.det()) { if (det.p) { g.det_slab = det.p; g.det_floats = det.floats; } else g.nsplit = 1; }
     if (P.s.dtype == LXO_F32) { a_f32 = true; b_f32 = true; }
     return lxo_launch_gemm_tn(P.s.dtype, a_f32, b_f32, g, st);
@@ -341,13 +341,19 @@
     }
 };
 
-static int bwd_logits(const Train& w, float* grads) {
+static int bwd_dwy(const Train& w, float* grads, hipStream_t st, DetScratch det) {
+    const Plan& P = w.P;
+    const int TB = P.s.T * P.s.B, O = P.s.O, V = P.s.V;
+    const void* dlog = P.ws<void>(w.ws, W_DLOGITS);
+    if (w.sp.mirrors) return tn(P, false, false, w.step(0).recb_cur, P.RECB, dlog, P.Vp, grads + P.poff[P_YWO], V, TB, O, V, st, det);
+    return tn(P, true, false, w.step(0).rec_cur, P.REC, dlog, P.Vp, grads + P.poff[P_YWO], V, TB, O, V, st);
+}
+static int bwd_logits(const Train& w, float* grads, bool dwy) {
     const Plan& P = w.P; hipStream_t st = w.st;
-    const int B = P.s.B, TB = P.s.T * B, O = P.s.O, V = P.s.V;
-    const void* dlog = P.ws<void>(w.ws, W_DLOGITS);
-    RC(nt(P, false, true, false, dlog, P.Vp, P.pk(w.wp, K_YWO), P.Vp, w.dolog, O, TB, O, P.Vp, nullptr, 0, false, st));
-    if (w.sp.mirrors) RC(tn(P, false, false, w.step(0).recb_cur, P.RECB, dlog, P.Vp, grads + P.poff[P_YWO], V, TB, O, V, st, P.det_scratch(w.ws)));
-    else RC(tn(P, true, false, w.step(0).rec_cur, P.REC, dlog, P.Vp, grads + P.poff[P_YWO], V, TB, O, V, st));
+    const int TB = P.s.T * P.s.B, O = P.s.O;
+    RC(nt(P, false, true, false, P.ws<void>(w.ws, W_DLOGITS), P.Vp, P.pk(w.wp, K_YWO), P.Vp, w.dolog, O, TB, O, P.Vp, nullptr, 0, false, st));
+    if (!dwy) return 0;
+    RC(bwd_dwy(w, grads, st, P.det_scratch(w.ws)));
     if (P.bf) RC(lxo_k_chain_poison(chain_err(P, w.ws, kChainFwd), nullptr, grads + P.ptotal - 1, st));
     return 0;
 }
@@ -482,7 +488,7 @@
     for (const InitProj& p : pr) RC(lxo_k_colsum(p.x, W3, grads + P.poff[p.bias], B, p.n, det_s, sd));
     return 0;
 }
-static int bwd_weight_grads(const Train& w, float* grads, bool bwd_chain_ran, const BwdStreams& s, DetScratch det_s) {
+static int bwd_weight_grads(const Train& w, float* grads, bool bwd_chain_ran, bool with_dwy, const BwdStreams& s, DetScratch det_s) {
     const Plan& P = w.P; void* ws = w.ws; hipStream_t st = w.st, sd = s.deferred();
     const int TB = P.s.T * P.s.B, E = P.s.E, U = P.s.U, O = P.s.O, D = P.s.D;
     auto gw = [&](int pid) { return grads + P.poff[pid]; };
@@ -494,11 +500,29 @@
     const void* dz = m ? (const void*)w.dzb : (const void*)w.dz; const int ldz = m ? P.DZBP : 4 * U;
     hipStream_t sx = m ? sd : st;
     const DetScratch dx = m ? det_s : DetScratch{nullptr, 0};
+    bool grouped = false;
+    if (m && bwd_chain_ran && lxo_switch(SW_DW_GROUP) && (P.det() ? dx.p != nullptr : lxo_switch(SW_GEMM_TN_TR) != 0)) {
+        GemmTN q[5];
+        int n = 0;
+        q[n++] = tn_prob(hc, ldr, g, ldg, gw(P_OWH), O, TB, P.HC, O);
+        q[n++] = tn_prob(hc, ldr, P.ws<bf16_t>(ws, W_DATTHB), E, gw(P_ATT_H), E, TB, U, E);
+        q[n++] = tn_prob(P.ws<void>(ws, W_EMB_IN), P.Dp, dz, ldz, gw(P_LSTM_K), 4 * U, TB, D, 4 * U);
+        q[n++] = tn_prob(rec, ldr, dz, ldz, gw(P_LSTM_K) + (size_t)D * 4 * U, 4 * U, TB, P.XH, 4 * U);
+        if (with_dwy) q[n++] = tn_prob(s0.recb_cur, P.RECB, P.ws<void>(ws, W_DLOGITS), P.Vp, gw(P_YWO), P.s.V, TB, O, P.s.V);
+        const int rc = lxo_launch_gemm_tn_tr_group(q, n, P.det() ? dx.p : nullptr, P.det() ? dx.floats : 0, sx);
+        if (rc != 0 && rc != -2) return rc < 0 ? rc : -rc;
+        grouped = rc == 0;
+    }
+    if (!grouped) {
     RC(tn(P, f, f, hc, ldr, g, ldg, gw(P_OWH), O, TB, P.HC, O, sx, dx));
     if (bwd_chain_ran) RC(tn(P, f, false, hc, ldr, P.ws<bf16_t>(ws, W_DATTHB), E, gw(P_ATT_H), E, TB, U, E, sx, dx));
     else RC(tn(P, f, true, hc, ldr, w.datth, E, gw(P_ATT_H), E, TB, U, E, sx));
     RC(tn(P, false, f, P.ws<void>(ws, W_EMB_IN), P.Dp, dz, ldz, gw(P_LSTM_K), 4 * U, TB, D, 4 * U, sx, dx));
     RC(tn(P, f, f, rec, ldr, dz, ldz, gw(P_LSTM_K) + (size_t)D * 4 * U, 4 * U, TB, P.XH, 4 * U, sx, dx));
+    if (with_dwy) RC(bwd_dwy(w, grads, sx, dx));
+    }
+    if (with_dwy && P.bf)
+        RC(lxo_k_chain_poison(chain_err(P, ws, kChainFwd), bwd_chain_ran ? chain_err(P, ws, kChainBwd) : nullptr, grads + P.ptotal - 1, sx));
     return lxo_k_colsum(w.dz, 4 * U, gw(P_LSTM_B), TB, 4 * U, det_s, sd);
 }
 static int bwd_embedding(const Train& w, const int* formula, float* grads, const BwdStreams& s) {
@@ -555,7 +579,8 @@
 int lxo_impl_decoder_train_bwd(const Plan& P, const float* prm, const void* wp, void* ws, const int* formula, float* grads,
                                int parts, hipStream_t st, bool defer_join, void* ready) {
     const Train w = train_of(P, prm, wp, ws, st);
-    if (parts & 1) RC(bwd_logits(w, grads));
+    const bool defer_dwy = parts == 3 && w.sp.mirrors && w.sp.try_chain && lxo_switch(SW_DW_GROUP) != 0;
+    if (parts & 1) RC(bwd_logits(w, grads, !defer_dwy));
     if (!(parts & 2)) return 0;
     bool chain = false;
     if (!w.sp.try_chain) {
@@ -572,14 +597,14 @@
     const DetScratch det_s = s.side ? P.det_scratch_side(ws) : P.det_scratch(ws);
     RC(s.fork());
     RC(bwd_init_states(w, grads, s, det_s));
-    RC(bwd_weight_grads(w, grads, chain, s, det_s));
+    RC(bwd_weight_grads(w, grads, chain, defer_dwy, s, det_s));
     RC(P.dimg_masked() ? bwd_dimg_masked(w, grads, s) : bwd_dimg_plain(w, grads, s));
     RC(bwd_embedding(w, formula, grads, BwdStreams{st, nullptr}));
     RC(s.wait_datt_img());
     RC(tn(P, false, false, P.ws<void>(ws, W_IMG), P.s.C, P.ws<void>(ws, W_DATTIMG), P.s.E, grads + P.poff[P_ATT_IMG], P.s.E, P.s.B * P.R, P.s.C, P.s.E,
           s.deferred(), det_s));
     RC(s.join(defer_join));
-    if (chain) RC(lxo_k_chain_poison(nullptr, chain_err(P, ws, kChainBwd), grads + P.ptotal - 1, st));
+    if (chain && !defer_dwy) RC(lxo_k_chain_poison(nullptr, chain_err(P, ws, kChainBwd), grads + P.ptotal - 1, st));
     return s.record_ready(ready);
 }
 
diff --git a/latex_ocr_amd/csrc/plan.hip b/latex_ocr_amd/csrc/plan.hip
--- a/latex_ocr_amd/csrc/plan.hip
+++ b/latex_ocr_amd/csrc/plan.hip
@@ -1,4 +1,5 @@
 #include "plan.h"
+#include "gemm.h"
 #include <stdio.h>
 #include <string.h>
 #include "switches.h"
@@ -146,6 +147,13 @@
         wb[W_DET] = need > floor_ ? need : floor_;
         const size_t wg = (size_t)264 * 9 * 64 * 128 * f4;
         if (bf && wb[W_DET] < wg) wb[W_DET] = wg;
+        {
+            const int TBi = T * B;
+            const int dims[5][2] = {{HC, O}, {U, E}, {D, 4 * U}, {XH, 4 * U}, {O, V}};
+            size_t units = 0;
+            for (const auto& d : dims) units += (size_t)((d[0] + 127) / 128) * ((d[1] + 127) / 128) * lxo_tn_nsplit(TBi, d[0], d[1]);
+            if (bf && wb[W_DET] < units * 128 * 128 * f4) wb[W_DET] = units * 128 * 128 * f4;
+        }
         if (bf) wb[W_DET] = 2 * ((wb[W_DET] + 255) / 256 * 256);
     }
     const int nb = s.beam > 1 ? s.beam : 1;
diff --git a/latex_ocr_amd/csrc/switches.h b/latex_ocr_amd/csrc/switches.h
--- a/latex_ocr_amd/csrc/switches.h
+++ b/latex_ocr_amd/csrc/switches.h
@@ -3,6 +3,7 @@
 enum LxoSwitch {
     SW_ATT_ALT, SW_ATT_EXP, SW_BEAM_FAST, SW_BEAM_INDIRECT, SW_RSTEP_MT16, SW_GEMM_NT_DMA, SW_GEMM_TN_TR, SW_WGRAD_HALO,
     SW_POOL_FUSED, SW_CONV1_MFMA, SW_CONV_2WG, SW_CONV_SMALL, SW_XDEC, SW_XDEC_DEC, SW_XDEC_BWD, SW_XDEC_DEC_CHUNK,
+    SW_DW_GROUP,
     SW_COUNT
 };
 int lxo_switch(LxoSwitch s);
diff --git a/latex_ocr_amd/csrc/switches.hip b/latex_ocr_amd/csrc/switches.hip
--- a/latex_ocr_amd/csrc/switches.hip
+++ b/latex_ocr_amd/csrc/switches.hip
@@ -21,6 +21,7 @@
     {"LXO_XDEC_DEC", arm, 1},
     {"LXO_XDEC_BWD", arm, 1},
     {"LXO_XDEC_DEC_CHUNK", live, 0},
+    {"LXO_DW_GROUP", live, 1},
 };
 int read(const Row& r) {
     const char* e = getenv(r.name);
```

Measured after the change: 9101 img/s (median of 6 runs). About the same (+0.6%).
